# huzi96/NVFPCC

Hardware: AMD Instinct MI355X
Metric: leaf-blocks/sec NVF train step (32^3, chanstr=8,16,8,8) (higher is better)
Workload: dtype f32; 1 GPU; train_step: decoder mini-batch update, NVFPCC.py:149-223 (fwd mode=train q=1, 3 focal losses + rate terms, bwd, fused Adam); full=False, primed_steps=31, batch_per_gpu=16, global_batch=16, blocks_resident=917, ch=3, chanstr=8,16,8,8, parallelism=dp1

## Files before the change

### include/nvf_hip.h

```cpp
#ifndef NVF_HIP_H
#define NVF_HIP_H

#include <stddef.h>
#include <stdint.h>

#ifdef __cplusplus
extern "C" {
#endif

#define NVF_OK 0
#define NVF_EINVAL (-1)
#define NVF_EWORKSPACE (-2)

#define NVF_ACT_NONE 0
#define NVF_ACT_RELU 1
#define NVF_ACT_SIGMOID 2

int nvf_version(void);

typedef struct NvfStepCtx NvfStepCtx;
size_t nvf_step_ctx_bytes(void);
int nvf_step_ctx_init(NvfStepCtx* ctx);
int nvf_step_ctx_set_direct(NvfStepCtx* ctx, int on);
int nvf_step_ctx_set_wgrad_forms(NvfStepCtx* ctx, int conv2_zsplit, int conv1_wino);
// ... 261 lines not shown
                 int nterm, float thh_acc, float thh_sse, float* out, void* workspace, size_t workspace_bytes,
                 NvfStepCtx* ctx, void* stream);

int nvf_sigmoid_bwd(const float* dp, const float* p, float* dlogit, int64_t n, void* stream);

int nvf_relu_bwd(const float* dy, const float* y, float* out, int64_t n, void* stream);

int nvf_squared_error_map(const float* p, const float* dist, float thh, float* out, int batch, int spatial,
                          void* stream);

int nvf_maxpool2(const float* x, float* y, int batch_channels, int d, int h, int w, void* stream);

int nvf_adam_step(float* p, const float* g, float* m, float* v, int64_t n, float lr, float beta1, float beta2,
                  float eps, int step, void* stream);

typedef struct NvfStepTail {
  float* p;
  const float* g;
  float* m;
  float* v;
  int64_t n;
  const float* coef_dev;
  float coef0_host, coef1_host, beta1, beta2, eps;
  int32_t nnb;
  const float* loss_terms;
  const float* lbits;
  const float* nbits;
  const float* inv_npts_dev;
  float inv_npts_host, nbits_scale;
  const float* counts;
  float* acc;
  int64_t* sched_buf;
  const int64_t* sched_rows;
  uint64_t* sched_cursor;
  uint32_t* done;
  int32_t sched_words, reserved;
} NvfStepTail;
int nvf_step_tail(const NvfStepTail* args, void* stream);

int nvf_finals_flush_tail(NvfStepCtx* ctx, const NvfStepTail* tail, const int64_t* ranges, int nranges, void* stream);
int nvf_wgrad_reduce_finals_tail(const float* const* slabs, float* const* dws, const int* nslabs, const int* jtotals,
                                 int n, const float* const* addends, const NvfAdamFuse* adam, NvfStepCtx* ctx,
                                 const NvfStepTail* tail, const int64_t* ranges, int nranges, void* stream);
int nvf_wgrad_reduce_finals(const float* const* slabs, float* const* dws, const int* nslabs, const int* jtotals, int n,
                            const float* const* addends, NvfStepCtx* ctx, void* stream);
int nvf_adam_coefficients(float lr, float beta1, float beta2, int step, float* coef_host);
int nvf_adam_coefficients_n(float lr, float beta1, float beta2, int step0, int n, float* coef_host);

int nvf_gather_rows(const float* src, const int64_t* idx, float* dst, int rows, int width, void* stream);
int nvf_scatter_add_rows(const float* src, const int64_t* idx, float* dst, int rows, int width, void* stream);

int nvf_gather_rows_multi(const float* const* srcs, float* const* dsts, const int* widths, int n,
                          const int64_t* idx, int rows, void* stream);

int nvf_step_head(const void* table_dev, int nlayers, int q, uint64_t seed, uint64_t step, const uint64_t* step_dev,
                  float* const* pack_dsts, const int* pack_kinds, const int* pack_c0s, const int* pack_c1s,
                  const int* pack_layers, const int* pack_bwd, int npack, const float* const* srcs,
                  float* const* dsts, const int* widths, int n, const int64_t* idx, int rows,
                  const NvfRateJob* rate , void* stream);

typedef struct NvfStemHead {
  const float* emb;
  const float* lat_beta_hat;
  const float* lat_gamma_hat;
  const float* sigma;
  const float* mu;
  const float* beta_hat;
  const float* gamma_hat;
  float* h;
  float* lat;
  float* x_rounded;
  float* bits;
  float* a0;
  float* h0;
  float* y1;
  int32_t lat_row, up0_row, conv0_row;
  int32_t mode, ch, c0, c1, reserved;
} NvfStemHead;
int nvf_step_head_stem(const void* table_dev, int nlayers, int q, uint64_t seed, uint64_t step,
                       const uint64_t* step_dev, float* const* pack_dsts, const int* pack_kinds, const int* pack_c0s,
                       const int* pack_c1s, const int* pack_layers, const int* pack_bwd, int npack,
                       const float* const* srcs, float* const* dsts, const int* widths, int n, const int64_t* idx,
                       int rows, const NvfRateJob* rate , const NvfStemHead* stem, void* stream);

int nvf_uniform(float* out, int64_t n, uint64_t seed, uint64_t stream_id, void* stream);

int nvf_threshold_count(const float* p, float thh, int32_t* counts, int batch, int voxels, void* stream);
int nvf_threshold_compact(const float* p, float thh, const int32_t* offsets, const int32_t* origins,
                          int32_t* coords, int batch, int dim, void* stream);

int nvf_nearest_dist2(const int32_t* pts, const int32_t* blk_off, const int32_t* origins, const int32_t* nb_off,
                      const int32_t* nb_idx, int32_t* d2out, int nblocks, void* stream);

#define NVF_PC_CELLS (128 * 128 * 128)
size_t nvf_pc_workspace_bytes(int n_query, int n_target);
int nvf_pc_nearest(const int32_t* query_sorted, int n_query, const int32_t* target_sorted, const int32_t* cell_start,
                   int n_target, int32_t* nn_idx, int32_t* nn_d2, void* stream);
int nvf_pc_knn_normals(const int32_t* cloud_sorted, const int32_t* cell_start, const int32_t* cloud_xyz, int n, int k,
                       float* normals, int32_t* knn_idx, void* stream);
int nvf_pc_error_sums(const int32_t* query_xyz, int n_query, const int32_t* target_xyz, const int32_t* nn_idx,
                      const float* normals, int normals_of_target, int64_t* sums, double* d2_sum, void* workspace,
                      size_t workspace_bytes, void* stream);

int nvf_occ_hist(const float* p, int batch, int voxels, int shift, int nbits, const uint32_t* prefix,
                 const int32_t* d2, const uint8_t* gt, uint32_t* count, uint64_t* sum_d2, uint32_t* count_gt,
                 uint32_t* bad, void* stream);
int nvf_occ_hist_edges(const float* p, int batch, int voxels, const float* edges, int nedges, const int32_t* d2,
                       const uint8_t* gt, uint32_t* count, uint64_t* sum_d2, uint32_t* count_gt, uint32_t* bad,
                       void* stream);
int nvf_threshold_count_v(const float* p, const float* thh, int32_t* counts, int batch, int voxels, void* stream);
int nvf_threshold_compact_v(const float* p, const float* thh, const int32_t* offsets, const int32_t* origins,
                            int32_t* coords, int batch, int dim, void* stream);

#define NVF_PP_META_INTS 16
#define NVF_PP_OCT_BYTES 37449
int nvf_pp_keys(const int32_t* pts, int npts, int32_t* keys, uint32_t* bitmap6, int32_t* meta, void* stream);
int nvf_pp_tree(const uint32_t* bitmap6, int32_t* origins, uint32_t* rank_tab, uint8_t* octree_bytes, int32_t* nb_off,
                int32_t* meta, void* stream);
int nvf_pp_blocks(const int32_t* sorted_keys, int npts, const uint32_t* rank_tab, int32_t* meta, int32_t* pts,
                  int32_t* blk_off, void* stream);
int nvf_pp_neighbours(const int32_t* origins, const uint32_t* rank_tab, const int32_t* nb_off, int32_t* nb_idx,
                      int nblocks, void* stream);
int nvf_pp_grids(const int32_t* d2, float* dist, float* gt, int64_t n, void* stream);

#define NVF_PP_DEEP_WORK_WORDS 11264
int nvf_pp_keys_deep(const int32_t* pts, int npts, int bits, int64_t* keys, uint32_t* bitmap, int32_t* meta,
                     void* stream);
int nvf_pp_tree_deep(const uint32_t* bitmap, int bits, int npts, int32_t* origins, uint32_t* rank_tab,
                     uint8_t* octree_bytes, int32_t* nb_off, uint32_t* work, int32_t* meta, void* stream);
int nvf_pp_blocks_deep(const int64_t* sorted_keys, int npts, int bits, const uint32_t* rank_tab, int32_t* meta,
                       int32_t* pts, int32_t* blk_off, void* stream);
int nvf_pp_neighbours_deep(const int32_t* origins, int bits, const uint32_t* rank_tab, const int32_t* nb_off,
                           int32_t* nb_idx, int nblocks, void* stream);

#ifdef __cplusplus
}
#endif
#endif
```

### nvfpcc_amd/_lib.py

```python
import ctypes as C
import os

_HERE = os.path.dirname(os.path.abspath(__file__))
LIB_PATH = os.environ.get("NVF_LIB", os.path.join(_HERE, "libnvf_hip.so"))

P = C.c_void_p
I = C.c_int
F = C.c_float
L = C.c_int64
U = C.c_uint64
Z = C.c_size_t

PROTOTYPES = {
    "nvf_version": (I, []),
    "nvf_step_ctx_bytes": (Z, []),
    "nvf_step_ctx_init": (I, [P]),
    "nvf_step_ctx_set_direct": (I, [P, I]),
    "nvf_step_ctx_set_wgrad_forms": (I, [P, I, I]),
    "nvf_pack_conv_weight": (I, [P, I, I, I, P, P, P]),
    "nvf_pack_convT_weight": (I, [P, I, I, I, P, P, P]),
    "nvf_effective_params": (I, [P, P, P, P, I, P, P, P, I, I, U, U, P]),
    "nvf_layer_desc_size": (Z, []),
    "nvf_prepare_weights": (I, [P, I, I, U, U, P, P]),
    "nvf_conv3d_gather": (I, [P, P, P, P, P, P] + [I] * 14 + [P]),
# ... 8 lines not shown
    "nvf_conv3d_k4_wino_fwd": (I, [P, P, P, P, I, I, I, P]),
    "nvf_wgrad_k4_wino": (I, [P, P, P, P, P, Z, I, I, P]),
    "nvf_pack_wino16_k4_floats": (Z, []),
    "nvf_conv3d_k4_wino16_bwd": (I, [P, P, P, P, I, I, I, P, P, P]),
    "nvf_conv3d_k4_wino16_fwd": (I, [P, P, P, P, I, I, I, P]),
    "nvf_wgrad16_k4_wino_partial": (I, [P, P, P, I, I, I, I, P, P]),
    "nvf_pack_convT_mfma_floats": (Z, [I]),
    "nvf_pack_convT_mfma": (I, [P, I, I, P, P]),
    "nvf_convT3d_k5s2_mfma": (I, [P, P, P, P, I, I, I, I, I, I, P]),
    "nvf_pack_s2k5_mfma_floats": (Z, [I, I]),
    "nvf_pack_s2k5_mfma": (I, [P, I, I, P, P]),
    "nvf_conv3d_s2k5_mfma": (I, [P, P, P, P, P, I, I, I, I, I, I, P]),
    "nvf_pack_convT16_mfma_floats": (Z, [I, I]),
    "nvf_pack_convT16_mfma": (I, [P, I, I, P, P]),
    "nvf_convT3d_k5s2_mfma16": (I, [P, P, P, P, I, I, I, I, I, I, I, P]),
    "nvf_pack_g16_mfma_floats": (Z, [I, I, I]),
    "nvf_pack_g16_mfma": (I, [P, I, I, I, P, P]),
    "nvf_conv3d_g16_mfma": (I, [P, P, P, P, P, P] + [I] * 14 + [P]),
    "nvf_pack_mfma_all": (I, [P, P, P, P, P, I, P]),
    "nvf_heads3_fwd": (I, [P, P, P, P, P, P, I, I, P]),
    "nvf_heads3_bwd_data": (I, [P, P, P, P, P, P, I, P]),
    "nvf_heads3_loss_bwd_data": (I, [P, P, P, P, P, P, P, P, P, P, P, P, P, I, P, Z, P, P]),
    "nvf_heads3_loss_bwd_data_bias": (I, [P, P, P, P, P, P, P, P, P, P, P, P, P, I, P, P, Z, P, P]),
    "nvf_heads3_fwd_loss_bwd_data": (I, [P, P, P, P, I, P, P, P, P, P, P, P, P, P, P, P, P, I, P, P, Z, P, P, P]),
    "nvf_heads3_wgrad_partial": (I, [P, P, P, P, P, I, I, P, P]),
    "nvf_stem_fwd": (I, [P] * 10 + [I, I, I, I, P]),
    "nvf_stem_latent_fwd": (I, [P] * 12 + [I, U, U, P] + [P] * 9 + [I, I, I, I, P]),
    "nvf_stem_bwd_workspace": (Z, [I, I]),
    "nvf_stem_bwd_workspace_for": (Z, [I, I, I, I]),
    "nvf_stem_bwd": (I, [P] * 13 + [Z, I, I, I, I, P]),
    "nvf_stem_bwd_partial": (I, [P, P, P, P, P, P, P, P, P, P, P, P, P, P, Z, I, I, I, I, P, P, P, P]),
    "nvf_wgrad_workspace": (Z, [I] * 7),
    "nvf_wgrad": (I, [P, P, P, P, Z] + [I] * 15 + [P]),
    "nvf_wgrad_partial": (I, [P, P, P, P, Z] + [I] * 14 + [P, P]),
    "nvf_wgrad_reduce_multi": (I, [P, P, P, P, I, P]),
    "nvf_wgrad_mfma3_partial": (I, [P, P, P, I, P, P, P]),
    "nvf_wgrad_up1_conv0_partial": (I, [P, P, P, I, P, P]),
    "nvf_wgrad_trunk5_partial": (I, [P, P, P, I, P, P, P]),
    "nvf_wgrad_trunk5_partial_bias": (I, [P, P, P, P, I, P, P, P]),
    "nvf_wgrad_trunk5_heads_partial": (I, [P, P, P, P, P, P, P, I, I, P, P, P, P]),
    "nvf_wgrad_trunk5_heads_sums_partial": (I, [P, P, P, P, P, P, P, I, P, P, P, P, I, P, Z, P, P, I, P, P, P, P]),
    "nvf_wgrad_reduce_finals_tail": (I, [P, P, P, P, I, P, P, P, P, P, I, P]),
    "nvf_wgrad_reduce_finals": (I, [P, P, P, P, I, P, P, P]),
    "nvf_channel_sum_workspace": (Z, [I]),
    "nvf_channel_sum": (I, [P, P, P, Z, I, I, I, I, P]),
    "nvf_multi_channel_sum_workspace": (Z, [I]),
    "nvf_multi_channel_sum": (I, [P, P, P, P, I, I, P, Z, P, P]),
    "nvf_wgrad_reduce_multi_and_sums": (I, [P, P, P, P, I, P, P, P, P, I, I, P, Z, P, P]),
    "nvf_latent_tail_queue": (I, [P, P, P, P, P, P, P, P, P, P, F, I, U, U, P, P, P, P, P, P, P, P, P, P, I, I, I]),
    "nvf_stem_bwd_queue": (I, [P] * 16 + [Z, P, I, I, I, I, P]),
    "nvf_stem_bwd_pending": (I, [P]),
    "nvf_latent_tail_pending": (I, [P]),
    "nvf_latent_tail_cancel": (None, [P]),
    "nvf_finals_begin": (I, [P]),
    "nvf_finals_flush": (I, [P, P]),
    "nvf_finals_cancel": (None, [P]),
    "nvf_gdn_fwd": (I, [P, P, P, P, I, I, I, I, P]),
    "nvf_gdn_bwd_workspace": (Z, [I]),
    "nvf_gdn_bwd": (I, [P, P, P, P, P, P, P, P, Z, I, I, I, I, P]),
    "nvf_latent_fwd": (I, [P] * 12 + [I, I, I, I, U, U, P, P]),
    "nvf_latent_rate": (I, [P] * 12 + [F, I, I, I, I, U, U, P, P]),
    "nvf_weight_rate": (I, [P, I, P, P, P, P, P, P, P, F, I, P]),
    "nvf_weight_rate_batch_workspace": (Z, []),
    "nvf_weight_rate_batch": (I, [P, P, P, I, P, P, P, P, P, P, F, P, Z, P, P]),
    "nvf_reduce_workspace": (Z, []),
    "nvf_focal_loss": (I, [P, P, P, F, F, P, P, P, F, P, Z, L, I, I, P]),
    "nvf_focal_loss_multi": (I, [P, P, P, P, P, P, P, I, P, I, P, Z, P, P]),
    "nvf_metrics": (I, [P, P, P, F, F, P, P, Z, L, I, P, P]),
    "nvf_metrics_workspace": (Z, []),
    "nvf_metrics3": (I, [P, P, P, P, I, F, F, P, P, Z, P, P]),
    "nvf_sigmoid_bwd": (I, [P, P, P, L, P]),
    "nvf_relu_bwd": (I, [P, P, P, L, P]),
    "nvf_squared_error_map": (I, [P, P, F, P, I, I, P]),
    "nvf_maxpool2": (I, [P, P, I, I, I, I, P]),
    "nvf_adam_step": (I, [P, P, P, P, L, F, F, F, F, I, P]),
    "nvf_step_tail": (I, [P, P]),
    "nvf_adam_coefficients": (I, [F, F, F, I, P]),
    "nvf_adam_coefficients_n": (I, [F, F, F, I, I, P]),
    "nvf_gather_rows": (I, [P, P, P, I, I, P]),
    "nvf_scatter_add_rows": (I, [P, P, P, I, I, P]),
    "nvf_gather_rows_multi": (I, [P, P, P, I, P, I, P]),
    "nvf_step_head": (I, [P, I, I, U, U, P, P, P, P, P, P, P, I, P, P, P, I, P, I, P, P]),
    "nvf_step_head_stem": (I, [P, I, I, U, U, P, P, P, P, P, P, P, I, P, P, P, I, P, I, P, P, P]),
    "nvf_weight_rate_batch_final": (I, [P, P, P, P, P, P]),
    "nvf_wgrad_reduce_multi_and_sums_fused": (I, [P, P, P, P, I, P, P, P, P, P, P, I, I, P, Z, P, P]),
    "nvf_finals_flush_tail": (I, [P, P, P, I, P]),
    "nvf_uniform": (I, [P, L, U, U, P]),
    "nvf_nearest_dist2": (I, [P, P, P, P, P, P, I, P]),
    "nvf_threshold_count": (I, [P, F, P, I, I, P]),
    "nvf_threshold_compact": (I, [P, F, P, P, P, I, I, P]),
    "nvf_pc_workspace_bytes": (Z, [I, I]),
    "nvf_pc_nearest": (I, [P, I, P, P, I, P, P, P]),
    "nvf_pc_knn_normals": (I, [P, P, P, I, I, P, P, P]),
    "nvf_pc_error_sums": (I, [P, I, P, P, P, I, P, P, P, Z, P]),
    "nvf_occ_hist": (I, [P, I, I, I, I, P, P, P, P, P, P, P, P]),
    "nvf_occ_hist_edges": (I, [P, I, I, P, I, P, P, P, P, P, P, P]),
    "nvf_threshold_count_v": (I, [P, P, P, I, I, P]),
    "nvf_threshold_compact_v": (I, [P, P, P, P, P, I, I, P]),
    "nvf_pp_keys": (I, [P, I, P, P, P, P]),
    "nvf_pp_tree": (I, [P, P, P, P, P, P, P]),
    "nvf_pp_blocks": (I, [P, I, P, P, P, P, P]),
    "nvf_pp_neighbours": (I, [P, P, P, P, I, P]),
    "nvf_pp_grids": (I, [P, P, P, L, P]),
    "nvf_pp_keys_deep": (I, [P, I, I, P, P, P, P]),
    "nvf_pp_tree_deep": (I, [P, I, I, P, P, P, P, P, P, P]),
    "nvf_pp_blocks_deep": (I, [P, I, I, P, P, P, P, P]),
    "nvf_pp_neighbours_deep": (I, [P, I, P, P, P, I, P]),
}



class NvfStepTail(C.Structure):
    _fields_ = [("p", P), ("g", P), ("m", P), ("v", P), ("n", L), ("coef_dev", P),
                ("coef0_host", F), ("coef1_host", F), ("beta1", F), ("beta2", F), ("eps", F), ("nnb", C.c_int32),
                ("loss_terms", P), ("lbits", P), ("nbits", P), ("inv_npts_dev", P),
                ("inv_npts_host", F), ("nbits_scale", F), ("counts", P), ("acc", P),
                ("sched_buf", P), ("sched_rows", P), ("sched_cursor", P), ("done", P),
                ("sched_words", C.c_int32), ("reserved", C.c_int32)]


class NvfRateJob(C.Structure):
    _fields_ = [("kernel", P * 8), ("dk", P * 8), ("n", C.c_int32 * 8), ("nlayers", C.c_int32), ("reserved", C.c_int32),
                ("sigma", P), ("mu", P), ("part", P), ("g", F), ("reserved2", F)]


class NvfStemHead(C.Structure):
    _fields_ = [(n, P) for n in ("emb", "lat_beta_hat", "lat_gamma_hat", "sigma", "mu", "beta_hat", "gamma_hat", "h", "lat",
                                 "x_rounded", "bits", "a0", "h0", "y1")] + \
               [(n, C.c_int32) for n in ("lat_row", "up0_row", "conv0_row", "mode", "ch", "c0", "c1", "reserved")]


class NvfAdamFuse(C.Structure):
    _fields_ = [("g_base", P), ("p_base", P), ("m_base", P), ("v_base", P), ("n", L), ("coef_dev", P),
                ("coef0_host", F), ("coef1_host", F), ("beta1", F), ("beta2", F), ("eps", F), ("reserved", F),
                ("bad_count", P)]


_lib = None


def lib():
    global _lib
    if _lib is None:
        if not os.path.isfile(LIB_PATH):
            raise RuntimeError(
                f"{LIB_PATH} is missing: the HIP extension has not been built "
                "(python -m nvfpcc_amd.build). There is no CPU fallback for the NVF hot path.")
        h = C.CDLL(LIB_PATH)
        for name, (res, args) in PROTOTYPES.items():
            fn = getattr(h, name)
            fn.restype = res
            fn.argtypes = args
        _lib = h
    return _lib


class NvfError(RuntimeError):
    pass


def check(rc, what):
    if rc != 0:
        kind = {-1: "NVF_EINVAL (rejected argument)", -2: "NVF_EWORKSPACE (workspace too small)"}.get(
            rc, f"hipError_t {rc}")
        raise NvfError(f"{what} failed: {kind}")
```

### nvfpcc_amd/csrc/finals.h

```cpp
#pragma once
#include "nvf_common.h"

static const int kLossMaxWG = 1024;

#define NVF_BETA_BOUND 1.0000072759311445e-03f
#define NVF_GAMMA_BOUND 3.814697265625e-06f

__device__ __forceinline__ int adam_fused_elem(const NvfAdamFuse& a, const float* gp, float gi) {
  const long i = gp - a.g_base;
  if (i < 0 || i >= a.n) return 0;
  if (!(fabsf(gi) <= 3.402823466e38f)) return 1;
  const float step_size = a.coef_dev ? a.coef_dev[0] : a.coef0_host, bc2_sqrt = a.coef_dev ? a.coef_dev[1] : a.coef1_host;
  const float mi = a.m_base[i] * a.beta1 + gi * (1.f - a.beta1);
  const float vi = a.v_base[i] * a.beta2 + (gi * gi) * (1.f - a.beta2);
  a.m_base[i] = mi;
  a.v_base[i] = vi;
  const float denom = sqrtf(vi) / bc2_sqrt + a.eps;
  a.p_base[i] = a.p_base[i] - step_size * (mi / denom);
  return 0;
}
__device__ __forceinline__ NvfAdamFuse adam_fuse_of(const NvfStepTail& t) {
  NvfAdamFuse a{};
  a.g_base = t.g; a.p_base = t.p; a.m_base = t.m; a.v_base = t.v; a.n = t.n; a.coef_dev = t.coef_dev;
  a.coef0_host = t.coef0_host; a.coef1_host = t.coef1_host; a.beta1 = t.beta1; a.beta2 = t.beta2; a.eps = t.eps;
  a.bad_count = t.acc ? t.acc + 6 : nullptr;
  return a;
}

struct FocalMulti {
  const float* p[3];
  const float* gt[3];
  const float* dist[3];
  float* dp[3];
  float alpha[3], beta[3];
  long n[3];
  int nwg[3];
};

struct MultiSumDesc {
  const float* x[12];
  float* out[12];
  int32_t c[12], spatial[12], chan_base[12];
  int32_t ntensors, batch, total_channels, nchunk;
};

struct WeightRateBatch {
  const float* kernel[8];
  float* dk[8];
  int32_t n[8];
  int32_t first_wg[9];
  int32_t nlayers, chunk;
};

__device__ __forceinline__ float focal_elem(float pv, float gv, float dv, bool has_dist, float a1, float a0, float beta,
                                            int chain_sigmoid, float& dp, float g = 1.f) {
#pragma clang fp contract(off)
  const bool occ = gv != 0.f;
  const float F = occ ? pv : 1.f - pv;
  const float at = occ ? a1 : a0;
  float w = 1.f;
  if (has_dist) w = dv + (occ ? beta : 0.f);
  const float Fc = F < 1e-9f ? 1e-9f : F;
  const float om = 1.f - Fc;
  const float lg = logf(Fc);
  float d = 0.f;
  if (F >= 1e-9f) d = -at * w * (-2.f * om * lg + om * om / Fc);
  const float dd = g * (occ ? d : -d);
  dp = chain_sigmoid ? dd * ((1.f - pv) * pv) : dd;
  return -1.f * at * (om * om) * w * lg;
}

__device__ __forceinline__ void focal_multi_final_body(const FocalMulti& m, const float* __restrict__ part,
                                                       float* __restrict__ loss, int nterm, int tid) {
  const int t = tid >> 6, lane = tid & 63;
  if (t >= nterm) return;
  float s = 0.f;
  for (int g = lane; g < m.nwg[t]; g += 64) s += part[t * kLossMaxWG + g];
  s = nvf_wave_sum(s);
  if (lane == 0) loss[t] = s;
}

__device__ __forceinline__ int multi_channel_sum_final_body(const MultiSumDesc& d, const float* __restrict__ part,
                                                            int gch, const NvfAdamFuse* adam = nullptr) {
  if (gch >= d.total_channels) return 0;
  int t = 0;
  while (t + 1 < d.ntensors && gch >= d.chan_base[t + 1]) ++t;
  float s = 0.f;
  for (int g = 0; g < d.nchunk; ++g) s += part[(size_t)g * d.total_channels + gch];
  float* o = d.out[t] + (gch - d.chan_base[t]);
  *o = s;
  return adam ? adam_fused_elem(*adam, o, s) : 0;
}

__device__ __forceinline__ int weight_rate_batch_final_body(const WeightRateBatch& b, const float* __restrict__ part,
                                                            const float* __restrict__ sigma, float* __restrict__ bits,
                                                            float* __restrict__ dsigma, float* __restrict__ dmu,
                                                            const float* __restrict__ g_dev, float g_host, int lane,
                                                            const NvfAdamFuse* adam = nullptr) {
  const float g = g_host * (g_dev ? g_dev[0] : 1.f);
  constexpr int SLOTS = 8;
  const int nwg = b.first_wg[b.nlayers];
  float pb[SLOTS], ps[SLOTS], pm[SLOTS];
#pragma unroll
  for (int i = 0; i < SLOTS; ++i) {
    const int wg = lane + 64 * i;
    const bool ok = wg < nwg;
    pb[i] = ok ? part[3 * wg] : 0.f;
    ps[i] = ok ? part[3 * wg + 1] : 0.f;
// ... 67 lines not shown
__device__ __forceinline__ void metrics_final_body(const float* __restrict__ part, float* __restrict__ out,
                                                   const int32_t* nwg, int nterm, int accumulate, int tid) {
  if (tid >= 6 * nterm) return;
  const int t = tid / 6, k = tid - 6 * t;
  float s = 0.f;
  for (int g0 = 0; g0 < nwg[t]; g0 += 16) {
    float v[16];
#pragma unroll
    for (int i = 0; i < 16; ++i) v[i] = g0 + i < nwg[t] ? part[((size_t)t * kLossMaxWG + g0 + i) * 6 + k] : 0.f;
#pragma unroll
    for (int i = 0; i < 16; ++i) s += v[i];
  }
  out[tid] = accumulate ? out[tid] + s : s;
}

struct FinalsArgs {
  FocalMulti f;
  const float* f_part;
  float* f_loss;
  MultiSumDesc s;
  const float* s_part;
  WeightRateBatch r;
  const float* r_part;
  const float* r_sigma;
  float* r_bits;
  float* r_dsigma;
  float* r_dmu;
  const float* r_gdev;
  float r_ghost;
  StemGdnFinal g;
  const float* m_part;
  float* m_out;
  int32_t m_nwg[3], m_nterm, m_accumulate;
  int32_t f_nterm, has_f, has_s, has_r, has_g, has_m;
  const float* hb_part;
  float* hb_out[3];
  int32_t hb_n[3], has_hb;
};

__device__ __forceinline__ int head_bias_final_body(const FinalsArgs& a, int h, int lane, const NvfAdamFuse* adam = nullptr) {
  float s = 0.f;
  for (int g = lane; g < a.hb_n[h]; g += 64) s += a.hb_part[h * kLossMaxWG + g];
  s = nvf_wave_sum(s);
  if (lane != 0) return 0;
  *a.hb_out[h] = s;
  return adam ? adam_fused_elem(*adam, a.hb_out[h], s) : 0;
}

__host__ __device__ inline int finals_sum_blocks(const FinalsArgs& a) {
  const int n = a.has_s ? (a.s.total_channels + 63) / 64 : 0;
  return n > 0 ? n : (a.has_hb ? 1 : 0);
}

__device__ __forceinline__ void finals_plain_body(const FinalsArgs& a, int sum_blocks, int bid) {
  const int tid = threadIdx.x;
  if (a.has_hb && bid == 2 && tid >= 64 && tid < 256) head_bias_final_body(a, (tid >> 6) - 1, tid & 63);
  if (bid == 2 + sum_blocks) {
    if (a.has_m) metrics_final_body(a.m_part, a.m_out, a.m_nwg, a.m_nterm, a.m_accumulate, tid);
  } else if (bid == 0) {
    if (a.has_f) focal_multi_final_body(a.f, a.f_part, a.f_loss, a.f_nterm, tid);
  } else if (bid == 1) {
    if (a.has_r && tid < 64)
      weight_rate_batch_final_body(a.r, a.r_part, a.r_sigma, a.r_bits, a.r_dsigma, a.r_dmu, a.r_gdev, a.r_ghost, tid);
    if (a.has_g && tid >= 64 && tid < 192) stem_gdn_final_body(a.g, tid - 64, 128);
  } else if (a.has_s && tid < 64) {
    multi_channel_sum_final_body(a.s, a.s_part, (bid - 2) * 64 + tid);
  }
}

struct TailRanges { long lo[16], hi[16]; int n; };

__device__ __forceinline__ void finals_tail_arrive(const NvfStepTail& t, unsigned long long cur, int nblocks) {
  if (!t.sched_rows) return;
  const int tid = threadIdx.x;
  __shared__ int last;
  int64_t next_word = 0;
  if (tid < t.sched_words) next_word = t.sched_rows[cur * (unsigned long long)t.sched_words + tid];
  if (tid == 0) last = atomicAdd(t.done, 1u) == (unsigned)nblocks - 1;
  __syncthreads();
  if (!last) return;
  if (tid < t.sched_words) t.sched_buf[tid] = next_word;
  for (int w = tid + blockDim.x; w < t.sched_words; w += blockDim.x)
    t.sched_buf[w] = t.sched_rows[cur * (unsigned long long)t.sched_words + w];
  if (tid == 0) { t.sched_cursor[0] = cur + 1; t.done[0] = 0u; }
}

__device__ __forceinline__ void finals_tail_body(const FinalsArgs& a, int sum_blocks, const NvfStepTail& t,
                                                 const TailRanges& rg, int bid, int nblocks) {
  const int tid = threadIdx.x, wave = tid >> 6, lane = tid & 63;
  const NvfAdamFuse ad = adam_fuse_of(t);
  const unsigned long long cur = t.sched_rows ? t.sched_cursor[0] : 0ull;
  int bad = 0;
  if (bid == 0) {
    if (a.has_f) focal_multi_final_body(a.f, a.f_part, a.f_loss, a.f_nterm, tid);
    if (a.has_r && wave == 3)
      bad += weight_rate_batch_final_body(a.r, a.r_part, a.r_sigma, a.r_bits, a.r_dsigma, a.r_dmu, a.r_gdev, a.r_ghost,
                                          lane, &ad);
    if (a.has_m) metrics_final_body(a.m_part, a.m_out, a.m_nwg, a.m_nterm, a.m_accumulate, tid);
  } else if (bid == 1) {
    if (a.has_g && tid < 256) bad += stem_gdn_final_body(a.g, tid, 256, &ad);
  } else if (bid < 2 + sum_blocks) {
    if (a.has_s && tid < 64) bad += multi_channel_sum_final_body(a.s, a.s_part, (bid - 2) * 64 + tid, &ad);
    if (a.has_hb && bid == 2 && wave >= 1 && wave <= 3) bad += head_bias_final_body(a, wave - 1, lane, &ad);
  } else {
    for (int r = 0; r < rg.n; ++r)
      for (long i = rg.lo[r] + tid; i < rg.hi[r]; i += blockDim.x) bad += adam_fused_elem(ad, t.g + i, t.g[i]);
  }
  if (t.acc) {
    const unsigned long long any = __ballot(bad != 0);
    float c = (float)bad;
    c = nvf_wave_sum(c);
    if (any && lane == 0) atomicAdd(t.acc + 6, c);
  }
  __syncthreads();
  if (bid == 0 && tid == 0 && t.acc) {
    int bad_terms = 0;
    for (int k = 0; k < 3; ++k) {
      const float x = t.loss_terms[k];
      t.acc[k] += x;
      bad_terms += !(fabsf(x) <= 3.402823466e38f);
    }
    const float bl = t.lbits[0] * (t.inv_npts_dev ? t.inv_npts_dev[0] : t.inv_npts_host);
    float nb = 0.f;
    for (int l = 0; l < t.nnb; ++l) nb += t.nbits[l];
    nb *= t.nbits_scale;
    t.acc[3] += bl;
    t.acc[4] += nb;
    bad_terms += !(fabsf(bl) <= 3.402823466e38f) + !(fabsf(nb) <= 3.402823466e38f);
    t.acc[5] += (float)bad_terms;
    t.acc[7] += 1.f;
    if (t.counts) {
      for (int k = 0; k < 3; ++k) {
        t.acc[8 + 2 * k] += t.counts[6 * k] / t.counts[6 * k + 1];
        t.acc[9 + 2 * k] += t.counts[6 * k + 2] / t.counts[6 * k + 3];
      }
      t.acc[14] += t.counts[4];
      t.acc[15] += t.counts[5];
    }
  }
  finals_tail_arrive(t, cur, nblocks);
}

struct NvfStepCtx;
bool nvf_finals_push_focal(NvfStepCtx* ctx, const FocalMulti& m, const float* part, float* loss, int nterm);
int nvf_finals_run_stem_gdn(NvfStepCtx* ctx, const StemGdnFinal& f, void* stream);
int nvf_finals_run_focal(NvfStepCtx* ctx, const FocalMulti& m, const float* part, float* loss, int nterm, void* stream);
bool nvf_finals_push_sums(NvfStepCtx* ctx, const MultiSumDesc& d, const float* part);
int nvf_finals_run_head_bias(NvfStepCtx* ctx, const float* part, float* const* outs, const int* n, void* stream);
bool nvf_finals_push_metrics(NvfStepCtx* ctx, const float* part, float* out, const int* nwg, int nterm, int accumulate);
bool nvf_finals_push_rate(NvfStepCtx* ctx, const WeightRateBatch& b, const float* part, const float* sigma, float* bits,
                          float* dsigma, float* dmu, const float* g_dev, float g_host);
```

### nvfpcc_amd/csrc/pointwise.hip

```cpp
#include "nvf_common.h"
#include "step_ctx.h"
#include "pack_mfma.h"
#include "latent_tail.h"
#include "stem_fwd.h"

#define NVF_GRID(n, bs) ((unsigned)(((n) + (bs)-1) / (bs)))

extern "C" int nvf_version(void) { return 100; }

__global__ void finalize_partials(const float* __restrict__ part, float* __restrict__ out, int nrow, int ncol,
                                  int accumulate) {
  int j = blockIdx.x * blockDim.x + threadIdx.x;
  if (j >= ncol) return;
  float s = 0.f;
  for (int g = 0; g < nrow; ++g) s += part[(size_t)g * ncol + j];
  out[j] = accumulate ? out[j] + s : s;
}

__global__ void effective_params_kernel(const float* __restrict__ kernel, const float* __restrict__ kernel_init,
                                        const float* __restrict__ u, float* __restrict__ w_eff, int n,
                                        const float* __restrict__ b, const float* __restrict__ b_init,
                                        float* __restrict__ b_eff, int nb, int q, uint64_t seed, uint64_t stream_id) {
  int i = blockIdx.x * blockDim.x + threadIdx.x;
  if (i < n) {
    float k = kernel[i];
    if (q == 1) {
      float uu = u ? u[i] : nvf_uniform01(seed, stream_id, (uint64_t)i);
      k = k + (uu - 0.5f) * 0.0625f;
    } else if (q == 2) {
      k = rintf(k * 16.f) / 16.f;
    }
    w_eff[i] = k + kernel_init[i];
  } else if (i < n + nb) {
    int j = i - n;
    b_eff[j] = b[j] + b_init[j];
  }
}

extern "C" int nvf_effective_params(const float* kernel, const float* kernel_init, const float* u, float* w_eff, int n,
                                    const float* b, const float* b_init, float* b_eff, int nb, int q, uint64_t seed,
                                    uint64_t stream_id, void* stream) {
  if (!kernel || !kernel_init || !w_eff || n <= 0 || nb < 0) return NVF_EINVAL;
  if (nb > 0 && (!b || !b_init || !b_eff)) return NVF_EINVAL;
  effective_params_kernel<<<NVF_GRID(n + nb, 256), 256, 0, nvf_stream(stream)>>>(kernel, kernel_init, u, w_eff, n, b,
                                                                                  b_init, b_eff, nb, q, seed,
                                                                                  stream_id);
  NVF_LAUNCH_CHECK();
  return NVF_OK;
}

struct NvfLayerDesc {
  const float* kernel;
  const float* kernel_init;
  const float* b;
  const float* b_init;
  float* w_fwd;
  float* w_bwd;
  float* b_eff;
  int32_t dim0, dim1, k3;
  int32_t kind;
  int32_t quantised;
  int32_t layer_id;
  int32_t nbias, pad_;
};

__device__ __forceinline__ float effective_weight(const NvfLayerDesc& d, int i, int qq, uint64_t seed, uint64_t sid) {
  float k = d.kernel[i];
  if (qq == 1) k = k + (nvf_uniform01(seed, sid, (uint64_t)i) - 0.5f) * 0.0625f;
  else if (qq == 2) k = rintf(k * 16.f) / 16.f;
  return k + d.kernel_init[i];
}

__device__ __forceinline__ void prepare_weights_body(const NvfLayerDesc* __restrict__ table, int q, uint64_t seed,
                                                     uint64_t step, const uint64_t* __restrict__ step_dev, int layer,
                                                     int bx, int nbx) {
  const NvfLayerDesc d = table[layer];
  const int n = d.dim0 * d.dim1 * d.k3;
  const int qq = d.quantised ? q : 0;
  const uint64_t st = step + (step_dev ? step_dev[0] : 0ull);
  const uint64_t sid = (st << 8) | (uint64_t)d.layer_id;
  for (int i = bx * blockDim.x + threadIdx.x; i < n + d.nbias; i += nbx * blockDim.x) {
    if (i < n) {
      const float w = effective_weight(d, i, qq, seed, sid);
      const int t = i % d.k3, i1 = (i / d.k3) % d.dim1, i0 = i / (d.k3 * d.dim1);
      if (d.kind == 0) {
        if (d.w_fwd) d.w_fwd[(i1 * d.k3 + t) * d.dim0 + i0] = w;
        if (d.w_bwd) d.w_bwd[(i0 * d.k3 + (d.k3 - 1 - t)) * d.dim1 + i1] = w;
      } else {
        if (d.w_fwd) d.w_fwd[(i0 * d.k3 + t) * d.dim1 + i1] = w;
        if (d.w_bwd) d.w_bwd[(i1 * d.k3 + t) * d.dim0 + i0] = w;
      }
    } else {
      const int j = i - n;
      d.b_eff[j] = d.b[j] + d.b_init[j];
    }
  }
}

__global__ void prepare_weights_kernel(const NvfLayerDesc* __restrict__ table, int q, uint64_t seed, uint64_t step,
                                       const uint64_t* __restrict__ step_dev) {
  prepare_weights_body(table, q, seed, step, step_dev, blockIdx.y, blockIdx.x, gridDim.x);
}

extern "C" size_t nvf_layer_desc_size(void) { return sizeof(NvfLayerDesc); }

extern "C" int nvf_prepare_weights(const void* table_dev, int nlayers, int q, uint64_t seed, uint64_t step,
                                   const uint64_t* step_dev, void* stream) {
  if (!table_dev || nlayers <= 0) return NVF_EINVAL;
  prepare_weights_kernel<<<dim3(16, nlayers), 256, 0, nvf_stream(stream)>>>((const NvfLayerDesc*)table_dev, q, seed,
                                                                           step, step_dev);
  NVF_LAUNCH_CHECK();
  return NVF_OK;
}

__global__ void gdn_fwd_kernel(const float* __restrict__ x, const float* __restrict__ beta_hat,
                               const float* __restrict__ gamma_hat, float* __restrict__ y, int batch, int c,
                               int spatial, int inverse) {
  long idx = (long)blockIdx.x * blockDim.x + threadIdx.x;
  long total = (long)batch * c * spatial;
  if (idx >= total) return;
  int s = idx % spatial;
  int ch = (idx / spatial) % c;
  long b = idx / ((long)spatial * c);
  const float* xb = x + b * c * spatial + s;
  float acc = gdn_beta(beta_hat[ch]);
  for (int j = 0; j < c; ++j) {
    float xj = xb[(long)j * spatial];
    acc = fmaf(gdn_gamma(gamma_hat[ch * c + j]), xj * xj, acc);
  }
  float nrm = sqrtf(acc);
  float xv = xb[(long)ch * spatial];
  y[idx] = inverse ? xv * nrm : xv / nrm;
}

extern "C" int nvf_gdn_fwd(const float* x, const float* beta_hat, const float* gamma_hat, float* y, int batch, int c,
                           int spatial, int inverse, void* stream) {
  if (!x || !beta_hat || !gamma_hat || !y || batch <= 0 || c <= 0 || spatial <= 0) return NVF_EINVAL;
  long total = (long)batch * c * spatial;
  gdn_fwd_kernel<<<NVF_GRID(total, 256), 256, 0, nvf_stream(stream)>>>(x, beta_hat, gamma_hat, y, batch, c, spatial,
                                                                       inverse);
  NVF_LAUNCH_CHECK();
  return NVF_OK;
}

static const int kGdnMaxC = 32;
static const int kGdnThreads = 128;
static const int kGdnMaxSlabs = 256;

template <int CG>
__global__ __launch_bounds__(kGdnThreads * CG) void gdn_bwd_kernel(const float* __restrict__ x,
                                                                   const float* __restrict__ beta_hat,
                                                                   const float* __restrict__ gamma_hat,
                                                                   const float* __restrict__ dy, float* __restrict__ dx,
                                                                   float* __restrict__ slabs, int batch, int c,
                                                                   int spatial, int inverse, int vox_per_wg,
                                                                   float* __restrict__ dbeta_hat,
                                                                   float* __restrict__ dgamma_hat) {
  extern __shared__ float sm[];
  constexpr int T = kGdnThreads, LD = T + 1, NT = T * CG, MAXK = kGdnMaxC / CG;
  float* ts = sm;
  float* xs = sm + c * LD;
  float* gam = xs + c * LD;
  float* bet = gam + c * c;
  const int tid = threadIdx.x, vt = tid % T, cg = tid / T;
  const int ncol = c + c * c;
  const long nvox = (long)batch * spatial;
  const long v_lo = (long)blockIdx.x * vox_per_wg;
  long v_hi = v_lo + vox_per_wg;
  if (v_hi > nvox) v_hi = nvox;
  for (int i = tid; i < c * c; i += NT) gam[i] = gdn_gamma(gamma_hat[i]);
  for (int i = tid; i < c; i += NT) bet[i] = gdn_beta(beta_hat[i]);
  float own[(kGdnMaxC + kGdnMaxC * kGdnMaxC + NT - 1) / NT];
#pragma unroll
  for (int i = 0; i < (int)(sizeof(own) / sizeof(float)); ++i) own[i] = 0.f;

  for (long base = v_lo; base < v_hi; base += T) {
    const long v = base + vt;
// ... 147 lines not shown
                               float* dsigma, float* dmu, const float* g_dev, float g_host, int batch, int c,
                               int spatial, int mode,
                               uint64_t seed, uint64_t step, const uint64_t* step_dev, void* stream) {
  if (!x || !sigma || !mu || batch <= 0 || c <= 0 || spatial <= 0) return NVF_EINVAL;
  if (mode != 0 && mode != 1) return NVF_EINVAL;
  latent_rate_kernel<<<1, 1024, 0, nvf_stream(stream)>>>(x, u, block_ids, sigma, mu, x_rounded, bits, dx, dx_addend,
                                                         dsigma, dmu, g_dev, g_host, batch, c, spatial, mode, seed,
                                                         step, step_dev);
  NVF_LAUNCH_CHECK();
  return NVF_OK;
}

__global__ __launch_bounds__(1024) void latent_fwd_kernel(const float* __restrict__ e, const float* __restrict__ w,
                                                          const float* __restrict__ bw,
                                                          const float* __restrict__ beta_hat,
                                                          const float* __restrict__ gamma_hat,
                                                          const int64_t* __restrict__ block_ids,
                                                          const float* __restrict__ sigma, const float* __restrict__ mu,
                                                          float* __restrict__ h_out, float* __restrict__ lat_out,
                                                          float* __restrict__ x_rounded, float* __restrict__ bits,
                                                          int batch, int c, int spatial, int mode, uint64_t seed,
                                                          uint64_t step_in, const uint64_t* __restrict__ step_dev) {
  __shared__ float s_par[160];
  __shared__ float scratch[kTailRateLds / 3];
  latent_fwd_body(e, w, bw, beta_hat, gamma_hat, block_ids, sigma, mu, h_out, lat_out, x_rounded, bits, batch, c, spatial,
                  mode, seed, step_in, step_dev, s_par, scratch, kTailRateLds / 3);
}

extern "C" int nvf_latent_fwd(const float* e, const float* w_fwd, const float* bias, const float* beta_hat,
                              const float* gamma_hat, const int64_t* block_ids, const float* sigma, const float* mu,
                              float* h, float* lat, float* x_rounded, float* bits, int batch, int c, int spatial,
                              int mode, uint64_t seed, uint64_t step, const uint64_t* step_dev, void* stream) {
  if (!e || !w_fwd || !bias || !beta_hat || !gamma_hat || !sigma || !mu || !h || !lat || !x_rounded || !bits)
    return NVF_EINVAL;
  if (batch <= 0 || c <= 0 || c > 8 || spatial <= 0 || (mode != 0 && mode != 1)) return NVF_EINVAL;
  latent_fwd_kernel<<<1, 1024, 0, nvf_stream(stream)>>>(e, w_fwd, bias, beta_hat, gamma_hat, block_ids, sigma, mu, h,
                                                        lat, x_rounded, bits, batch, c, spatial, mode, seed, step,
                                                        step_dev);
  NVF_LAUNCH_CHECK();
  return NVF_OK;
}

__global__ __launch_bounds__(1024) void weight_rate_kernel(const float* __restrict__ kernel, int n,
                                                           const float* __restrict__ sigma,
                                                           const float* __restrict__ mu, float* __restrict__ bits,
                                                           float* __restrict__ dk, float* __restrict__ dsigma,
                                                           float* __restrict__ dmu, const float* __restrict__ g_dev,
                                                           float g_host, int accumulate) {
  __shared__ float red[16];
  const float g = g_host * (g_dev ? g_dev[0] : 1.f);
  const float gsign = g > 0.f ? 1.f : (g < 0.f ? -1.f : 0.f);
  const float sraw = sigma[0], sabs = fabsf(sraw), m = mu[0];
  float sb = 0.f, ss = 0.f, sm_ = 0.f;
  for (int i = threadIdx.x; i < n; i += blockDim.x) {
    float v = rintf(kernel[i] * 16.f) / 16.f;
    RateTerm r = rate_term(v, m, sabs, 0.03125f, gsign);
    sb += r.bits;
    ss += r.dsig;
    sm_ += r.dmu;
    if (dk) dk[i] = accumulate ? dk[i] + g * r.dv : g * r.dv;
  }
  float tb = nvf_block_sum(sb, red);
  float tsg = nvf_block_sum(ss, red);
  float tm = nvf_block_sum(sm_, red);
  if (threadIdx.x == 0) {
    if (bits) bits[0] = tb;
    float sgn = sraw > 0.f ? 1.f : (sraw < 0.f ? -1.f : 0.f);
    if (dsigma) dsigma[0] = accumulate ? dsigma[0] + g * tsg * sgn : g * tsg * sgn;
    if (dmu) dmu[0] = accumulate ? dmu[0] + g * tm : g * tm;
  }
}

extern "C" int nvf_weight_rate(const float* kernel, int n, const float* sigma, const float* mu, float* bits, float* dk,
                               float* dsigma, float* dmu, const float* g_dev, float g_host, int accumulate,
                               void* stream) {
  if (!kernel || !sigma || !mu || n <= 0) return NVF_EINVAL;
  weight_rate_kernel<<<1, 1024, 0, nvf_stream(stream)>>>(kernel, n, sigma, mu, bits, dk, dsigma, dmu, g_dev, g_host,
                                                         accumulate);
  NVF_LAUNCH_CHECK();
  return NVF_OK;
}


__device__ __forceinline__ void weight_rate_partial_body(const WeightRateBatch& b, const float* __restrict__ sigma,
                                                         const float* __restrict__ mu, float* __restrict__ part, float g,
                                                         int wg, int accumulate, float* red, int nthreads = 0) {
  if (nthreads <= 0) nthreads = blockDim.x;
  const float gsign = g > 0.f ? 1.f : (g < 0.f ? -1.f : 0.f);
  const float sabs = fabsf(sigma[0]), m = mu[0];
  int l = 0;
  while (l + 1 < b.nlayers && wg >= b.first_wg[l + 1]) ++l;
  const int lo = (wg - b.first_wg[l]) * b.chunk;
  const int hi = min(lo + b.chunk, b.n[l]);
  const float* k = b.kernel[l];
  float* dk = b.dk[l];
  float sb = 0.f, ss = 0.f, sm_ = 0.f;
  for (int i = lo + threadIdx.x; i < hi && (int)threadIdx.x < nthreads; i += nthreads) {
    float v = rintf(k[i] * 16.f) / 16.f;
    RateTerm r = rate_term(v, m, sabs, 0.03125f, gsign);
    sb += r.bits;
    ss += r.dsig;
    sm_ += r.dmu;
    if (dk) dk[i] = accumulate ? dk[i] + g * r.dv : g * r.dv;
  }
  float tb = nvf_block_sum(sb, red);
  float tsg = nvf_block_sum(ss, red);
  float tm = nvf_block_sum(sm_, red);
  if (threadIdx.x == 0) {
    part[3 * wg] = tb;
    part[3 * wg + 1] = tsg;
    part[3 * wg + 2] = tm;
  }
}

__global__ __launch_bounds__(256) void weight_rate_batch_kernel(WeightRateBatch b, const float* __restrict__ sigma,
                                                                const float* __restrict__ mu,
                                                                float* __restrict__ part,
                                                                const float* __restrict__ g_dev, float g_host) {
  __shared__ float red[16];
  weight_rate_partial_body(b, sigma, mu, part, g_host * (g_dev ? g_dev[0] : 1.f), blockIdx.x, 1, red);
}

static int weight_rate_batch_desc(const float* const* kernels, float* const* dks, const int* ns, int nlayers,
                                  WeightRateBatch& b) {
  if (!kernels || !ns || nlayers <= 0 || nlayers > 8) return NVF_EINVAL;
  long total = 0;
  for (int i = 0; i < nlayers; ++i) {
    if (!kernels[i] || ns[i] <= 0) return NVF_EINVAL;
    b.kernel[i] = kernels[i];
    b.dk[i] = dks ? dks[i] : nullptr;
    b.n[i] = ns[i];
    total += ns[i];
  }
  b.nlayers = nlayers;
  long chunk = (total + 255) / 256;
  if (chunk < 256) chunk = 256;
  b.chunk = (int)chunk;
  int wg = 0;
  for (int i = 0; i < nlayers; ++i) {
    b.first_wg[i] = wg;
    wg += (int)((ns[i] + chunk - 1) / chunk);
  }
  b.first_wg[nlayers] = wg;
  return wg > 512 ? NVF_EINVAL : NVF_OK;
}

__global__ void weight_rate_batch_final(WeightRateBatch b, const float* __restrict__ part,
                                        const float* __restrict__ sigma, float* __restrict__ bits,
                                        float* __restrict__ dsigma, float* __restrict__ dmu,
                                        const float* __restrict__ g_dev, float g_host) {
  weight_rate_batch_final_body(b, part, sigma, bits, dsigma, dmu, g_dev, g_host, threadIdx.x);
}

extern "C" int nvf_weight_rate_batch_final(const NvfRateJob* job, float* bits, float* dsigma, float* dmu,
                                           NvfStepCtx* ctx, void* stream) {
  if (!job || !bits || !job->sigma || !job->mu || !job->part) return NVF_EINVAL;
  WeightRateBatch b{};
  const int rc = weight_rate_batch_desc(job->kernel, job->dk, job->n, job->nlayers, b);
  if (rc != NVF_OK) return rc;
  if (!nvf_finals_push_rate(ctx, b, job->part, job->sigma, bits, dsigma, dmu, nullptr, job->g))
    weight_rate_batch_final<<<1, 64, 0, nvf_stream(stream)>>>(b, job->part, job->sigma, bits, dsigma, dmu, nullptr, job->g);
  NVF_LAUNCH_CHECK();
  return NVF_OK;
}

extern "C" size_t nvf_weight_rate_batch_workspace(void) { return (size_t)3 * 512 * sizeof(float); }

extern "C" int nvf_weight_rate_batch(const float* const* kernels, float* const* dks, const int* ns, int nlayers,
                                     const float* sigma, const float* mu, float* bits, float* dsigma, float* dmu,
                                     const float* g_dev, float g_host, void* workspace, size_t workspace_bytes,
                                     NvfStepCtx* ctx, void* stream) {
  if (!kernels || !ns || nlayers <= 0 || nlayers > 8 || !sigma || !mu || !bits || !workspace) return NVF_EINVAL;
  if (workspace_bytes < nvf_weight_rate_batch_workspace()) return NVF_EWORKSPACE;
  WeightRateBatch b{};
  const int rc = weight_rate_batch_desc(kernels, dks, ns, nlayers, b);
  if (rc != NVF_OK) return rc;
  const int wg = b.first_wg[nlayers];
  hipStream_t s = nvf_stream(stream);
  weight_rate_batch_kernel<<<wg, 256, 0, s>>>(b, sigma, mu, (float*)workspace, g_dev, g_host);
  if (!nvf_finals_push_rate(ctx, b, (const float*)workspace, sigma, bits, dsigma, dmu, g_dev, g_host))
    weight_rate_batch_final<<<1, 64, 0, s>>>(b, (const float*)workspace, sigma, bits, dsigma, dmu, g_dev, g_host);
// ... 265 lines not shown
  long i = (long)blockIdx.x * blockDim.x + threadIdx.x;
  if (i >= n) return;
  float gi = g[i];
  float mi = m[i] * b1 + gi * (1.f - b1);
  float vi = v[i] * b2 + (gi * gi) * (1.f - b2);
  m[i] = mi;
  v[i] = vi;
  float denom = sqrtf(vi) / bc2_sqrt + eps;
  p[i] = p[i] - step_size * (mi / denom);
}

extern "C" int nvf_adam_step(float* p, const float* g, float* m, float* v, int64_t n, float lr, float beta1,
                             float beta2, float eps, int step, void* stream) {
  if (!p || !g || !m || !v || n <= 0 || step < 1) return NVF_EINVAL;
  double bc1 = 1.0 - pow((double)beta1, step), bc2 = 1.0 - pow((double)beta2, step);
  adam_kernel<<<NVF_GRID(n, 256), 256, 0, nvf_stream(stream)>>>(p, g, m, v, (long)n, (float)(lr / bc1), beta1, beta2,
                                                                eps, (float)sqrt(bc2));
  NVF_LAUNCH_CHECK();
  return NVF_OK;
}

__global__ void step_tail_kernel(NvfStepTail a) {
  const long i = (long)blockIdx.x * blockDim.x + threadIdx.x;
  int bad = 0;
  if (i < a.n) {
    const float step_size = a.coef_dev ? a.coef_dev[0] : a.coef0_host, bc2_sqrt = a.coef_dev ? a.coef_dev[1] : a.coef1_host;
    const float gi = a.g[i];
    bad = !(fabsf(gi) <= 3.402823466e38f);
    if (!bad) {
      const float mi = a.m[i] * a.beta1 + gi * (1.f - a.beta1);
      const float vi = a.v[i] * a.beta2 + (gi * gi) * (1.f - a.beta2);
      a.m[i] = mi;
      a.v[i] = vi;
      const float denom = sqrtf(vi) / bc2_sqrt + a.eps;
      a.p[i] = a.p[i] - step_size * (mi / denom);
    }
  }
  if (a.acc) {
    const unsigned long long any = __ballot(bad);
    if (any && (threadIdx.x & 63) == 0) atomicAdd(a.acc + 6, (float)__popcll(any));
  }
  if (!a.acc && !a.sched_rows) return;
  __shared__ int last;
  bool is_last = gridDim.x == 1;
  if (gridDim.x > 1) {
    __syncthreads();
    if (threadIdx.x == 0) last = atomicAdd(a.done, 1u) == gridDim.x - 1;
    __syncthreads();
    is_last = last != 0;
  }
  if (!is_last) return;
  if (a.acc && threadIdx.x == 0) {
    int bad_terms = 0;
    for (int t = 0; t < 3; ++t) {
      const float x = a.loss_terms[t];
      a.acc[t] += x;
      bad_terms += !(fabsf(x) <= 3.402823466e38f);
    }
    const float bl = a.lbits[0] * (a.inv_npts_dev ? a.inv_npts_dev[0] : a.inv_npts_host);
    float nb = 0.f;
    for (int l = 0; l < a.nnb; ++l) nb += a.nbits[l];
    nb *= a.nbits_scale;
    a.acc[3] += bl;
    a.acc[4] += nb;
    bad_terms += !(fabsf(bl) <= 3.402823466e38f) + !(fabsf(nb) <= 3.402823466e38f);
    a.acc[5] += (float)bad_terms;
    a.acc[7] += 1.f;
    if (a.counts) {
      for (int t = 0; t < 3; ++t) {
        a.acc[8 + 2 * t] += a.counts[6 * t] / a.counts[6 * t + 1];
        a.acc[9 + 2 * t] += a.counts[6 * t + 2] / a.counts[6 * t + 3];
      }
      a.acc[14] += a.counts[4];
      a.acc[15] += a.counts[5];
    }
  }
  if (a.sched_rows) {
    __shared__ unsigned long long cur_s;
    if (threadIdx.x == 0) cur_s = a.sched_cursor[0];
    __syncthreads();
    const unsigned long long c = cur_s;
    const int64_t* row = a.sched_rows + c * (unsigned long long)a.sched_words;
    for (int w = threadIdx.x; w < a.sched_words; w += blockDim.x) a.sched_buf[w] = row[w];
    if (threadIdx.x == 0) a.sched_cursor[0] = c + 1;
  }
  if (threadIdx.x == 0 && gridDim.x > 1) a.done[0] = 0u;
}

extern "C" int nvf_step_tail(const NvfStepTail* args, void* stream) {
  if (!args) return NVF_EINVAL;
  const NvfStepTail a = *args;
  if (!a.p || !a.g || !a.m || !a.v || a.n <= 0) return NVF_EINVAL;
  if (a.acc && (!a.loss_terms || !a.lbits || !a.nbits || a.nnb <= 0 || a.nnb > 16)) return NVF_EINVAL;
  if (a.sched_rows && (!a.sched_buf || !a.sched_cursor || a.sched_words <= 0)) return NVF_EINVAL;
  if ((a.acc || a.sched_rows) && !a.done) return NVF_EINVAL;
  step_tail_kernel<<<NVF_GRID(a.n, 256), 256, 0, nvf_stream(stream)>>>(a);
  NVF_LAUNCH_CHECK();
  return NVF_OK;
}

extern "C" int nvf_adam_coefficients(float lr, float beta1, float beta2, int step, float* coef_host) {
  if (!coef_host || step < 1) return NVF_EINVAL;
  double bc1 = 1.0 - pow((double)beta1, step), bc2 = 1.0 - pow((double)beta2, step);
  coef_host[0] = (float)(lr / bc1);
  coef_host[1] = (float)sqrt(bc2);
  return NVF_OK;
}

extern "C" int nvf_adam_coefficients_n(float lr, float beta1, float beta2, int step0, int n, float* coef_host) {
  if (!coef_host || step0 < 1 || n < 0) return NVF_EINVAL;
  for (int k = 0; k < n; ++k) {
    const int rc = nvf_adam_coefficients(lr, beta1, beta2, step0 + k, coef_host + 2 * k);
    if (rc != NVF_OK) return rc;
  }
  return NVF_OK;
}

__global__ void gather_rows_kernel(const float* __restrict__ src, const int64_t* __restrict__ idx,
                                   float* __restrict__ dst, int rows, int width) {
  long i = (long)blockIdx.x * blockDim.x + threadIdx.x;
  if (i >= (long)rows * width) return;
  int r = i / width, c = i % width;
  dst[i] = src[idx[r] * width + c];
}

__global__ void scatter_add_rows_kernel(const float* __restrict__ src, const int64_t* __restrict__ idx,
                                        float* __restrict__ dst, int rows, int width) {
  long i = (long)blockIdx.x * blockDim.x + threadIdx.x;
  if (i >= (long)rows * width) return;
  int r = i / width, c = i % width;
  dst[idx[r] * width + c] += src[i];
}

extern "C" int nvf_gather_rows(const float* src, const int64_t* idx, float* dst, int rows, int width, void* stream) {
  if (!src || !idx || !dst || rows <= 0 || width <= 0) return NVF_EINVAL;
  gather_rows_kernel<<<NVF_GRID((long)rows * width, 256), 256, 0, nvf_stream(stream)>>>(src, idx, dst, rows, width);
  NVF_LAUNCH_CHECK();
  return NVF_OK;
}

extern "C" int nvf_scatter_add_rows(const float* src, const int64_t* idx, float* dst, int rows, int width,
                                    void* stream) {
  if (!src || !idx || !dst || rows <= 0 || width <= 0) return NVF_EINVAL;
  scatter_add_rows_kernel<<<NVF_GRID((long)rows * width, 256), 256, 0, nvf_stream(stream)>>>(src, idx, dst, rows,
                                                                                            width);
  NVF_LAUNCH_CHECK();
  return NVF_OK;
}

struct GatherMulti {
  const float* src[6];
  float* dst[6];
  int32_t width[6];
  int32_t n;
};

__device__ __forceinline__ void gather_rows_multi_body(const GatherMulti& g, const int64_t* __restrict__ idx, int rows,
                                                       int t, int bx, int nbx) {
  if (t >= g.n) return;
  const int width = g.width[t];
  const long total = (long)rows * width;
  const float* src = g.src[t];
  float* dst = g.dst[t];
  if ((width & 3) == 0) {
    const long total4 = total >> 2;
    const int w4 = width >> 2;
    for (long i = (long)bx * blockDim.x + threadIdx.x; i < total4; i += (long)nbx * blockDim.x) {
// ... 200 lines not shown
  if ((NVF_HS_SKIP & 2) && bid >= nstem) return;
  if (bid < nstem) {
    const uint64_t st = step + (step_dev ? step_dev[0] : 0ull);
    const StemRawW wp{table[sj.lat_row], table[sj.up0_row], table[sj.conv0_row], sj.emb, idx, seed, st, sj.ch, q};
    const StemLatent L{nullptr, nullptr, nullptr, sj.lat_beta_hat, sj.lat_gamma_hat, idx, sj.sigma, sj.mu, sj.h, sj.lat,
                       sj.x_rounded, sj.bits, step_dev, seed, step, sj.mode, rows};
    const int b = bid == 0 ? 0 : (bid - 1) / PARTS, part = bid == 0 ? PARTS : (bid - 1) % PARTS;
    stem_fwd_body<C0, C1, COG, true, true>(nullptr, wp, sj.beta_hat, sj.gamma_hat, sj.a0, sj.h0, sj.y1, sj.ch, L, b, part,
                                           lds);
    return;
  }
  bid -= nstem;
  if (bid < rate.nwg) {
    weight_rate_partial_body(rate.b, rate.sigma, rate.mu, rate.part, rate.g, bid, 0, lds, 256);
    return;
  }
  bid -= rate.nwg;
  if (bid < wpl * nlayers) { prepare_weights_body(table, q, seed, step, step_dev, bid / wpl, bid % wpl, wpl); return; }
  bid -= wpl * nlayers;
  if (bid < wpl * pk.n) {
    const int job = bid / wpl;
    const NvfLayerDesc d = table[pk.layer[job]];
    const int qq = d.quantised ? q : 0, bwd = pk.bwd[job];
    const uint64_t st = step + (step_dev ? step_dev[0] : 0ull);
    const uint64_t sid = (st << 8) | (uint64_t)d.layer_id;
    pack_mfma_body(pk, job, bid % wpl, wpl, [&](int, int si) {
      return effective_weight(d, layout_to_kernel_index(d, bwd, si), qq, seed, sid);
    });
    return;
  }
  bid -= wpl * pk.n;
  gather_rows_multi_body(g, idx, rows, bid / gwg, bid % gwg, gwg);
}

extern "C" int nvf_step_head_stem(const void* table_dev, int nlayers, int q, uint64_t seed, uint64_t step,
                                  const uint64_t* step_dev, float* const* pack_dsts, const int* pack_kinds,
                                  const int* pack_c0s, const int* pack_c1s, const int* pack_layers, const int* pack_bwd,
                                  int npack, const float* const* srcs, float* const* dsts, const int* widths, int n,
                                  const int64_t* idx, int rows, const NvfRateJob* rate_job, const NvfStemHead* stem,
                                  void* stream) {
  if (!table_dev || nlayers <= 0 || !idx || npack < 0 || !stem) return NVF_EINVAL;
  const NvfStemHead sj = *stem;
  const bool narrow = sj.c0 == 8 && sj.c1 == 16, wide = sj.c0 == 16 && sj.c1 == 32;
  if (!(narrow || wide) || sj.ch <= 0 || sj.ch > kStemFwdMaxCh || rows <= 0 || rows > 32) return NVF_EINVAL;
  if (sj.lat_row < 0 || sj.lat_row >= nlayers || sj.up0_row < 0 || sj.up0_row >= nlayers || sj.conv0_row < 0 ||
      sj.conv0_row >= nlayers || (sj.mode != 0 && sj.mode != 1))
    return NVF_EINVAL;
  if (!sj.emb || !sj.lat_beta_hat || !sj.lat_gamma_hat || !sj.sigma || !sj.mu || !sj.beta_hat || !sj.gamma_hat || !sj.h ||
      !sj.lat || !sj.x_rounded || !sj.bits || !sj.a0 || !sj.h0 || !sj.y1)
    return NVF_EINVAL;
  PackJobs pk{};
  if (npack > 0) {
    if (!pack_layers || !pack_bwd) return NVF_EINVAL;
    const int rc = pack_jobs_desc(nullptr, pack_dsts, pack_kinds, pack_c0s, pack_c1s, npack, pk);
    if (rc != NVF_OK) return rc;
    for (int j = 0; j < npack; ++j) {
      if (pack_layers[j] < 0 || pack_layers[j] >= nlayers) return NVF_EINVAL;
      pk.layer[j] = pack_layers[j]; pk.bwd[j] = pack_bwd[j] ? 1 : 0;
    }
  }
  GatherMulti g{};
  long wg = 0;
  const int rc = gather_multi_desc(srcs, dsts, widths, n, rows, g, wg);
  if (rc != NVF_OK) return rc;
  const int tscale = (narrow ? 2 : 4) * nvf_tune_int("NVF_HS_GSCALE", 1);
  wg = (wg + tscale - 1) / tscale;
  const int wpl = nvf_tune_int("NVF_HS_WPL", 32) > 0 ? nvf_tune_int("NVF_HS_WPL", 32) : 32;
  RateInHead rate{};
  if (rate_job) {
    if (!rate_job->sigma || !rate_job->mu || !rate_job->part) return NVF_EINVAL;
    const int rrc = weight_rate_batch_desc(rate_job->kernel, rate_job->dk, rate_job->n, rate_job->nlayers, rate.b);
    if (rrc != NVF_OK) return rrc;
    rate.sigma = rate_job->sigma; rate.mu = rate_job->mu; rate.part = rate_job->part; rate.g = rate_job->g;
    rate.nwg = rate.b.first_wg[rate.b.nlayers];
  }
  const int parts = narrow ? 16 / 4 : 32 / (2 * 2);
  const unsigned grid = 1 + rows * parts + rate.nwg + wpl * nlayers + wpl * npack + (unsigned)(wg * n);
  if (narrow)
    step_head_stem_kernel<8, 16, 4><<<grid, 512, 0, nvf_stream(stream)>>>(
        (const NvfLayerDesc*)table_dev, nlayers, q, seed, step, step_dev, pk, g, idx, rows, (int)wg, wpl, rate, sj);
  else
    step_head_stem_kernel<16, 32, 2><<<grid, 1024, 0, nvf_stream(stream)>>>(
        (const NvfLayerDesc*)table_dev, nlayers, q, seed, step, step_dev, pk, g, idx, rows, (int)wg, wpl, rate, sj);
  NVF_LAUNCH_CHECK();
  return NVF_OK;
}

__global__ void uniform_kernel(float* __restrict__ out, long n, uint64_t seed, uint64_t stream_id) {
  long i = (long)blockIdx.x * blockDim.x + threadIdx.x;
  if (i < n) out[i] = nvf_uniform01(seed, stream_id, (uint64_t)i);
}

extern "C" int nvf_uniform(float* out, int64_t n, uint64_t seed, uint64_t stream_id, void* stream) {
  if (!out || n <= 0) return NVF_EINVAL;
  uniform_kernel<<<NVF_GRID(n, 256), 256, 0, nvf_stream(stream)>>>(out, (long)n, seed, stream_id);
  NVF_LAUNCH_CHECK();
  return NVF_OK;
}

__global__ __launch_bounds__(1024) void threshold_count_kernel(const float* __restrict__ p, float thh,
                                                               int32_t* __restrict__ counts, int voxels) {
  __shared__ float red[16];
  const float* pb = p + (size_t)blockIdx.x * voxels;
  float c = 0.f;
  for (int i = threadIdx.x; i < voxels; i += blockDim.x) c += pb[i] > thh ? 1.f : 0.f;
  float t = nvf_block_sum(c, red);
  if (threadIdx.x == 0) counts[blockIdx.x] = (int32_t)t;
}

extern "C" int nvf_threshold_count(const float* p, float thh, int32_t* counts, int batch, int voxels, void* stream) {
  if (!p || !counts || batch <= 0 || voxels <= 0 || voxels > (1 << 24)) return NVF_EINVAL;
  threshold_count_kernel<<<batch, 1024, 0, nvf_stream(stream)>>>(p, thh, counts, voxels);
  NVF_LAUNCH_CHECK();
  return NVF_OK;
}

__global__ __launch_bounds__(1024) void threshold_compact_kernel(const float* __restrict__ p, float thh,
                                                                 const int32_t* __restrict__ offsets,
                                                                 const int32_t* __restrict__ origins,
                                                                 int32_t* __restrict__ coords, int dim) {
  __shared__ int wave_cnt[16];
  __shared__ int running;
  const int b = blockIdx.x, voxels = dim * dim * dim;
  const float* pb = p + (size_t)b * voxels;
  const int lane = threadIdx.x & 63, wv = threadIdx.x >> 6, nw = blockDim.x >> 6;
  const int oz = origins ? origins[3 * b] : 0, oy = origins ? origins[3 * b + 1] : 0, ox = origins ? origins[3 * b + 2] : 0;
  if (threadIdx.x == 0) running = offsets[b];
  __syncthreads();
  for (int base = 0; base < voxels; base += blockDim.x) {
    const int i = base + threadIdx.x;
    const bool hit = i < voxels && pb[i] > thh;
    const unsigned long long mask = __ballot(hit);
    const int before = __popcll(mask & ((1ull << lane) - 1ull));
    if (lane == 0) wave_cnt[wv] = __popcll(mask);
    __syncthreads();
    int off = running;
    for (int k = 0; k < wv; ++k) off += wave_cnt[k];
    if (hit) {
      const int z = i / (dim * dim), y = (i / dim) % dim, x = i % dim;
      int32_t* o = coords + (size_t)(off + before) * 3;
      o[0] = oz + z;
      o[1] = oy + y;
      o[2] = ox + x;
    }
    __syncthreads();
    if (threadIdx.x == 0) {
      int t = 0;
      for (int k = 0; k < nw; ++k) t += wave_cnt[k];
      running += t;
    }
    __syncthreads();
  }
}

extern "C" int nvf_threshold_compact(const float* p, float thh, const int32_t* offsets, const int32_t* origins,
                                     int32_t* coords, int batch, int dim, void* stream) {
  if (!p || !offsets || !coords || batch <= 0 || dim <= 0 || dim > 256) return NVF_EINVAL;
  threshold_compact_kernel<<<batch, 1024, 0, nvf_stream(stream)>>>(p, thh, offsets, origins, coords, dim);
  NVF_LAUNCH_CHECK();
  return NVF_OK;
}
```

### nvfpcc_amd/csrc/wgrad.hip

```cpp
#include "nvf_common.h"
#include <cstdio>
#include <cstdlib>
#include "step_ctx.h"
#include "heads_wgrad_mfma.h"

static const int kMaxSlabs = 512;
static const int kSumChunks = 128;
struct MultiSumDesc;
__global__ void multi_channel_sum_final(MultiSumDesc d, const float* __restrict__ part);
extern "C" size_t nvf_multi_channel_sum_workspace(int total_channels);
__global__ void wgrad_reduce(const float* __restrict__ slabs, float* __restrict__ dw, int nslab, int jtotal,
                             int accumulate);

struct WgDims {
  int batch, bc;
  int dp, hp, wp;
  int dq, hq, wq;
  int pad;
  int tiles_x, tiles_y, tiles_z;
  int items, items_per_wg;
  int out_mode, jtotal;
  float* bias_slab;
};

__global__ void wgrad_naive(const float* __restrict__ p, const float* __restrict__ q, float* __restrict__ dw, int a_ch,
                            int k, int stride, WgDims d, int accumulate) {
  int k3 = k * k * k;
  int j = blockIdx.x * (blockDim.x >> 6) + (threadIdx.x >> 6);
  const int lane = threadIdx.x & 63;
  if (j >= a_ch * d.bc * k3) return;
  int kk = j % k3, b = (j / k3) % d.bc, a = j / (k3 * d.bc);
  int kz = kk / (k * k), ky = (kk / k) % k, kx = kk % k;
  const long plane = (long)d.hp * d.wp, vol = (long)d.dp * plane, total = (long)d.batch * vol;
  float acc = 0.f;
  for (long e = lane; e < total; e += 64) {
    const int n = (int)(e / vol);
    const long r = e - (long)n * vol;
    const int iz = (int)(r / plane), iy = (int)((r - (long)iz * plane) / d.wp), ix = (int)(r % d.wp);
    const int qz = iz * stride - d.pad + kz, qy = iy * stride - d.pad + ky, qx = ix * stride - d.pad + kx;
    if (qz < 0 || qz >= d.dq || qy < 0 || qy >= d.hq || qx < 0 || qx >= d.wq) continue;
    const float pv = p[((size_t)n * a_ch + a) * vol + r];
    const float qv = q[(((size_t)n * d.bc + b) * d.dq + qz) * d.hq * d.wq + qy * d.wq + qx];
    acc = fmaf(pv, qv, acc);
  }
  acc = nvf_wave_sum(acc);
  if (lane != 0) return;
  int o = d.out_mode == 0 ? j : (b * a_ch + a) * k3 + (k3 - 1 - kk);
  dw[o] = accumulate ? dw[o] + acc : acc;
}

template <int A_, int KS_, int S_, int NB_, int TX_, int TY_, int TZ_, int IXU_ = 0>
struct WCfg {
  static constexpr int A = A_, KS = KS_, S = S_, NB = NB_, TX = TX_, TY = TY_, TZ = TZ_;
  static constexpr int K3 = KS * KS * KS;
  static constexpr int IXU = IXU_ > 0 ? IXU_ : (A_ <= 8 ? 2 : 1);
  static constexpr int WPB = (K3 + 63) / 64;
  static constexpr int NT = NB * WPB * 64;
  static constexpr int QX = (TX - 1) * S + KS, QY = (TY - 1) * S + KS, QZ = (TZ - 1) * S + KS;
  static constexpr int mod32(int v, int r) { return v + ((r - v % 32) + 32) % 32; }
  static constexpr int QRS = mod32(QX, KS % 32);
  static constexpr int QPS = mod32(QY * QRS, (KS * KS) % 32);
  static constexpr int QCS = QZ * QPS;
  static constexpr int PT = A * TZ * TY * TX;
  static constexpr int POFF = (NB * QCS + 3) / 4 * 4;
  static constexpr int LDSF = POFF + PT;
  static_assert(TX % 4 == 0, "p rows are read four at a time");
  static_assert(NT <= 1024, "workgroup size");
  static_assert(LDSF * 4 <= 160 * 1024, "LDS");
};

template <class C>
__device__ __forceinline__ void wgrad_tiled_body(const float* __restrict__ p, const float* __restrict__ q,
                                                 float* __restrict__ slabs, const WgDims& d, int bx, int by, float* lds) {
  constexpr int A = C::A, KS = C::KS, S = C::S, NB = C::NB, TX = C::TX, TY = C::TY, TZ = C::TZ, K3 = C::K3;
  constexpr int QX = C::QX, QY = C::QY, QZ = C::QZ, QRS = C::QRS, QPS = C::QPS, QCS = C::QCS, NT = C::NT;
  const int tid = threadIdx.x, wave = tid >> 6, lane = tid & 63;
  const int bb = wave / C::WPB;
  const int kk = (wave % C::WPB) * 64 + lane;
  const bool valid = kk < K3;
  const int kz = kk / (KS * KS), ky = (kk / KS) % KS, kx = kk % KS;
  const int b0 = by * NB;
  const int lane_off = valid ? bb * QCS + kz * QPS + ky * QRS + kx : 0;
  float acc[A];
#pragma unroll
  for (int a = 0; a < A; ++a) acc[a] = 0.f;

  const int tiles = d.tiles_x * d.tiles_y * d.tiles_z;
// ... 1077 lines not shown
    const bool cube_t5 = a == 8 && b == 8 && k == 5 && stride == 2 && pad == 0 && out_mode == 0 && dp == 16 && hp == 16 &&
                         wp == 16 && dq == 35 && hq == 35 && wq == 35;
    if (rc == 1 && variant == 0 && cube_t5) rc = launch_wgrad_s2k5<TWCfg<2, 2>>(p, q, dw, slabs, d, accumulate, s, defer_nslab);
    if (rc == 1 && variant == 7 && cube_t5) rc = launch_wgrad_s2k5<TWCfg<1, 4>>(p, q, dw, slabs, d, accumulate, s, defer_nslab);
    NVF_W(9, 8, 4, 1, 32, 8, 32, 8, 2, 0)
    NVF_W(9, 8, 4, 1, 16, 8, 16, 8, 2, 0)
    NVF_W(0, 8, 5, 2, 16, 4, 16, 4, 2, 0)
    NVF_W(9, 8, 5, 2, 16, 4, 16, 4, 2, 0)
    NVF_W(0, 16, 5, 2, 8, 4, 8, 4, 2, 0)
    NVF_W(0, 8, 5, 2, 4, 4, 4, 4, 4, 0)
    NVF_W(0, 16, 4, 1, 32, 8, 32, 4, 2, 0)
    NVF_W(0, 16, 4, 1, 16, 8, 16, 8, 2, 0)
    NVF_W(0, 16, 5, 2, 16, 2, 16, 4, 2, 0)
    NVF_W(0, 32, 5, 2, 8, 4, 8, 4, 2, 0)
    NVF_W(0, 16, 5, 2, 4, 4, 4, 4, 4, 0)
    NVF_W(40, 16, 4, 1, 32, 16, 32, 8, 2, 0)
    NVF_W(41, 16, 4, 1, 32, 8, 32, 4, 2, 0)
    NVF_W(42, 16, 4, 1, 32, 8, 32, 8, 4, 0)
    NVF_W(43, 16, 4, 1, 32, 4, 32, 8, 2, 0)
    NVF_W(40, 16, 5, 2, 16, 8, 16, 4, 2, 0)
    NVF_W(41, 16, 5, 2, 16, 4, 16, 8, 2, 0)
    NVF_W(42, 16, 5, 2, 16, 4, 16, 4, 4, 0)
    NVF_W(43, 16, 5, 2, 16, 2, 16, 4, 2, 0)
    NVF_W(0, 8, 3, 1, 32, 1, 32, 8, 4, 0)
    NVF_W(0, 8, 3, 1, 16, 1, 16, 8, 4, 0)
    NVF_W(0, 16, 3, 1, 8, 1, 8, 8, 8, 0)
    NVF_W(0, 16, 3, 1, 32, 1, 32, 8, 4, 0)
    NVF_W(0, 16, 3, 1, 16, 1, 16, 8, 4, 0)
    NVF_W(0, 32, 3, 1, 8, 1, 8, 8, 8, 0)
    NVF_W(0, 1, 3, 1, 32, 8, 32, 8, 4, 8)
    NVF_W(0, 1, 3, 1, 16, 8, 16, 8, 4, 4)
    NVF_W(0, 1, 3, 1, 8, 8, 8, 8, 8, 2)
    NVF_W(2, 1, 3, 1, 32, 8, 32, 8, 2, 8)
    NVF_W(3, 1, 3, 1, 32, 4, 32, 8, 4, 8)
    NVF_W(2, 8, 4, 1, 32, 8, 32, 8, 2, 1)
    NVF_W(3, 8, 4, 1, 32, 8, 32, 8, 2, 8)
    NVF_W(4, 8, 4, 1, 32, 8, 32, 4, 2, 2)
    NVF_W(5, 8, 4, 1, 32, 4, 32, 8, 4, 2)
    NVF_W(6, 8, 4, 1, 32, 8, 32, 8, 4, 2)
    NVF_W(2, 8, 3, 1, 32, 1, 32, 8, 4, 1)
    NVF_W(3, 8, 3, 1, 32, 1, 32, 4, 2, 2)
    NVF_W(2, 8, 5, 2, 16, 4, 16, 4, 2, 1)
    NVF_W(3, 8, 5, 2, 16, 8, 16, 4, 2, 2)
    NVF_W(4, 8, 5, 2, 16, 4, 16, 2, 2, 2)
#undef NVF_W
  }
  if (rc == 1) {
    wgrad_naive<<<(d.jtotal + 3) / 4, 256, 0, s>>>(p, q, dw, a, k, stride, d, accumulate);
    if (defer_nslab) *defer_nslab = 0;
    rc = NVF_OK;
  }
  NVF_LAUNCH_CHECK();
  return rc;
}

extern "C" int nvf_wgrad_up1_conv0_partial(const float* const* ps, const float* const* qs, float* const* slabs,
                                           int batch, int* nslabs, void* stream) {
  if (!ps || !qs || !slabs || !nslabs || batch <= 0) return NVF_EINVAL;
  using C0 = WCfg<16, 5, 2, 4, 8, 4, 2, 0>; using C1 = WCfg<8, 5, 2, 4, 4, 4, 4, 0>;
  WgTiled2 m{};
  for (int j = 0; j < 2; ++j)
    if (!ps[j] || !qs[j] || !slabs[j]) return NVF_EINVAL;
  fill_up1_conv0<C0, C1>(m, ps, qs, slabs, batch, nslabs);
  wgrad_tiled2_kernel<C0, C1><<<m.nx[0] * m.ny[0] + m.nx[1] * m.ny[1], C0::NT, 0, nvf_stream(stream)>>>(m);
  NVF_LAUNCH_CHECK();
  return NVF_OK;
}

extern "C" int nvf_wgrad(const float* p, const float* q, float* dw, void* workspace, size_t workspace_bytes, int batch,
                         int a, int b, int k, int stride, int pad, int dp, int hp, int wp, int dq, int hq, int wq,
                         int out_mode, int accumulate, int variant, void* stream) {
  return wgrad_dispatch(p, q, dw, workspace, workspace_bytes, batch, a, b, k, stride, pad, dp, hp, wp, dq, hq, wq,
                        out_mode, accumulate, variant, stream, nullptr);
}

extern "C" int nvf_wgrad_partial(const float* p, const float* q, float* dw, void* workspace, size_t workspace_bytes,
                                 int batch, int a, int b, int k, int stride, int pad, int dp, int hp, int wp, int dq,
                                 int hq, int wq, int out_mode, int variant, int* nslab, void* stream) {
  if (!nslab) return NVF_EINVAL;
  return wgrad_dispatch(p, q, dw, workspace, workspace_bytes, batch, a, b, k, stride, pad, dp, hp, wp, dq, hq, wq,
                        out_mode, 0, variant, stream, nslab);
}

struct WgReduceMulti {
  const float* slabs[16];
  float* dw[16];
  const float* add[16];
  int32_t nslab[16], jtotal[16], blk_base[17];
  int32_t n, fuse;
  NvfAdamFuse adam;
};

__device__ __forceinline__ void wgrad_reduce_multi_body(const WgReduceMulti& d, int bid, float (*part)[64]) {
  int t = 0;
  while (t + 1 < d.n && bid >= d.blk_base[t + 1]) ++t;
  const float* slabs = d.slabs[t];
  const int nslab = d.nslab[t], jtotal = d.jtotal[t];
  const int jl = threadIdx.x & 63, sl = threadIdx.x >> 6;
  const int j = (bid - d.blk_base[t]) * 64 + jl;
  float s0 = 0.f, s1 = 0.f, s2 = 0.f, s3 = 0.f;
  if (j < jtotal) {
    for (int g0 = sl; g0 < nslab; g0 += 256) {
      float v[16];
#pragma unroll
      for (int i = 0; i < 16; ++i) v[i] = g0 + 16 * i < nslab ? slabs[(size_t)(g0 + 16 * i) * jtotal + j] : 0.f;
#pragma unroll
      for (int i = 0; i < 16; i += 4) { s0 += v[i]; s1 += v[i + 1]; s2 += v[i + 2]; s3 += v[i + 3]; }
    }
  }
  const float s = (s0 + s1) + (s2 + s3);
  part[sl][jl] = s;
  __syncthreads();
  if (sl == 0) {
    int bad = 0;
    if (j < jtotal) {
      float v = part[0][jl];
#pragma unroll
      for (int k = 1; k < 16; ++k) v += part[k][jl];
      if (d.add[t]) v += d.add[t][j];
      d.dw[t][j] = v;
      if (d.fuse) bad = adam_fused_elem(d.adam, d.dw[t] + j, v);
    }
    if (d.fuse && d.adam.bad_count) {
      const unsigned long long any = __ballot(bad);
      if (any && jl == 0) atomicAdd(d.adam.bad_count, (float)__popcll(any));
    }
  }
}

__global__ __launch_bounds__(1024) void wgrad_reduce_multi(WgReduceMulti d) {
  __shared__ float part[16][64];
  wgrad_reduce_multi_body(d, blockIdx.x, part);
}

extern "C" int nvf_wgrad_reduce_multi(const float* const* slabs, float* const* dws, const int* nslabs,
                                      const int* jtotals, int n, void* stream) {
  if (!slabs || !dws || !nslabs || !jtotals || n <= 0 || n > 16) return NVF_EINVAL;
  WgReduceMulti d{};
  int base = 0, m = 0;
  for (int i = 0; i < n; ++i) {
    if (nslabs[i] == 0) continue;
    if (!slabs[i] || !dws[i] || nslabs[i] < 0 || jtotals[i] <= 0) return NVF_EINVAL;
    d.slabs[m] = slabs[i]; d.dw[m] = dws[i]; d.nslab[m] = nslabs[i]; d.jtotal[m] = jtotals[i];
    d.blk_base[m] = base;
    base += (jtotals[i] + 63) / 64;
    ++m;
  }
  d.blk_base[m] = base;
  d.n = m;
  if (m == 0) return NVF_OK;
  wgrad_reduce_multi<<<base, 1024, 0, nvf_stream(stream)>>>(d);
  NVF_LAUNCH_CHECK();
  return NVF_OK;
}


__global__ __launch_bounds__(256) void channel_sum_partial(const float* __restrict__ x, float* __restrict__ part,
                                                           int batch, int c, int spatial, int chunk) {
  __shared__ float red[16];
  const int ch = blockIdx.x, g = blockIdx.y;
  const long total = (long)batch * spatial;
  const long lo = (long)g * chunk;
  long hi = lo + chunk;
  if (hi > total) hi = total;
  float s = 0.f;
  for (long e = lo + threadIdx.x; e < hi; e += blockDim.x) {
    const long n = e / spatial, sp = e % spatial;
    s += x[((size_t)n * c + ch) * spatial + sp];
  }
  s = nvf_block_sum(s, red);
  if (threadIdx.x == 0) part[(size_t)g * c + ch] = s;
}

__global__ void channel_sum_final(const float* __restrict__ part, float* __restrict__ out, int c, int nchunk,
                                  int accumulate) {
  const int ch = blockIdx.x * blockDim.x + threadIdx.x;
  if (ch >= c) return;
  float s = 0.f;
  for (int g = 0; g < nchunk; ++g) s += part[(size_t)g * c + ch];
  out[ch] = accumulate ? out[ch] + s : s;
}

extern "C" size_t nvf_channel_sum_workspace(int c) { return (size_t)kSumChunks * c * sizeof(float); }

extern "C" int nvf_channel_sum(const float* x, float* out, void* workspace, size_t workspace_bytes, int batch, int c,
                               int spatial, int accumulate, void* stream) {
  if (!x || !out || !workspace || batch <= 0 || c <= 0 || spatial <= 0) return NVF_EINVAL;
  if (workspace_bytes < nvf_channel_sum_workspace(c)) return NVF_EWORKSPACE;
  const long total = (long)batch * spatial;
  long chunk = (total + kSumChunks - 1) / kSumChunks;
  if (chunk < 1024) chunk = 1024;
  const int nchunk = (int)((total + chunk - 1) / chunk);
  hipStream_t s = nvf_stream(stream);
  channel_sum_partial<<<dim3(c, nchunk), 256, 0, s>>>(x, (float*)workspace, batch, c, spatial, (int)chunk);
  channel_sum_final<<<(c + 63) / 64, 64, 0, s>>>((const float*)workspace, out, c, nchunk, accumulate);
  NVF_LAUNCH_CHECK();
  return NVF_OK;
}


__global__ __launch_bounds__(NVF_SUM_T) void multi_channel_sum_partial(MultiSumDesc d, float* __restrict__ part) {
  __shared__ float red[16];
  multi_channel_sum_partial_body<NVF_SUM_T>(d, part, blockIdx.x, blockIdx.y, red);
}

__global__ __launch_bounds__(1024) void wgrad_reduce_and_sums(WgReduceMulti r, int r_blocks, MultiSumDesc m,
                                                              float* __restrict__ part) {
  __shared__ float sm[16][64];
  const int bid = blockIdx.x;
  if (bid < r_blocks) { wgrad_reduce_multi_body(r, bid, sm); return; }
  const int q = bid - r_blocks;
// ... 224 lines not shown
```

### nvfpcc_amd/engine.py

```python
import functools
import os
from typing import NamedTuple

import numpy as np
import torch

from . import ops
from ._lib import lib, check
from .network import NoiseState

R, S, NONE = ops.ACT_RELU, ops.ACT_SIGMOID, ops.ACT_NONE
_WINO = os.environ.get("NVF_WINO", "1") != "0"


def _wino_bwd_ppc(g_out):
    if g_out.shape[0] <= 64:
        return 0
    return 18 if g_out.shape[-1] == 32 else 10


_HEAD_BIAS_IN_LOSS = True
_SUMS_IN_TRUNK5 = True
_STEM_IN_TRUNK5 = True
_STEM_IN_HEAD = True
_HEADS_IN_TRUNK5 = True


class StepPlan(NamedTuple):
    want_w: bool
    want_emb: bool
    stem_fwd: str
    latent_fwd_fused: bool
    heads: str
    head_bias_in_loss: bool
    heads_in_trunk5: bool
    trunk5: bool
    conv0_wgrad_in_stem: bool
    stem_bwd: str
    tail_queued: bool
    sums_in_trunk5: bool
    fused_optimiser: bool


@functools.lru_cache(maxsize=None)
def plan_step(narrow, wide, winograd, fused_stem, fused_latent_stem, heads3, ch, batch, want_w, want_emb, fuse, hook,
              naive, head_bias_in_loss, sums_in_trunk5, stem_in_trunk5, stem_in_head, heads_in_trunk5,
              step_head=False, defer_heads=False):
    tuned = naive == 0
    small = batch <= 32
    stem_fwd = ("head" if step_head and stem_in_head and fused_stem and fused_latent_stem and small and tuned else
                "latent" if ch <= 8 and tuned and fused_stem and fused_latent_stem else
                "fused" if fused_stem else "layers")
    fused_loss = heads3 and small and tuned
    heads = (("deferred" if defer_heads and want_w else "fused_loss") if fused_loss else
             "heads3" if heads3 else "layers")
    trunk5 = want_w and narrow and tuned
    in_trunk5 = trunk5 and heads3 and heads_in_trunk5
    tail = want_w and not want_emb and ch <= 8 and tuned
    stem_bwd = ("queued" if stem_in_trunk5 and tail and in_trunk5 and fused_stem and small else
                "layers" if not fused_stem else "partial" if want_w else "plain")
    return StepPlan(want_w=want_w, want_emb=want_emb, stem_fwd=stem_fwd, latent_fwd_fused=ch <= 8 and tuned, heads=heads,
                    head_bias_in_loss=want_w and head_bias_in_loss and fused_loss, heads_in_trunk5=in_trunk5,
                    trunk5=trunk5, conv0_wgrad_in_stem=want_w and fused_stem and not trunk5, stem_bwd=stem_bwd,
                    tail_queued=tail, sums_in_trunk5=in_trunk5 and sums_in_trunk5, fused_optimiser=fuse and not hook)


TRUNK = ("up0", "conv0", "up1", "conv1", "up2", "conv2", "conv2_cls")
HEADS = ("conv1_cls", "conv0_cls")
MFMA_BWD = {"conv1": (2, 64), "conv2": (0, 64)}

_DESC = np.dtype([("kernel", "<u8"), ("kernel_init", "<u8"), ("b", "<u8"), ("b_init", "<u8"), ("w_fwd", "<u8"),
                  ("w_bwd", "<u8"), ("b_eff", "<u8"), ("dim0", "<i4"), ("dim1", "<i4"), ("k3", "<i4"),
                  ("kind", "<i4"), ("quantised", "<i4"), ("layer_id", "<i4"), ("nbias", "<i4"), ("pad", "<i4")])


class _Layer:
    __slots__ = ("name", "mod", "kind", "k", "w_fwd", "w_bwd", "b_eff", "gk", "gb", "cin", "cout", "pad", "wp_f",
                 "wp_b", "wp_t", "wp_tr", "wp_s", "wp_gf", "wp_gb", "wp_t16", "wp_w", "wp_wf", "bwd_pair", "bwd_max_batch")


class TrainEngine:
    def __init__(self, net, gt_all, dist_all, n_points_total, lmbda, w1, w2, lr, wemb, emb=None, seed=0, winograd=None):
        assert lib().nvf_layer_desc_size() == _DESC.itemsize
        self.winograd = _WINO if winograd is None else bool(winograd)
        self.net = net
        self.dev = gt_all.device
        self.gt, self.dist = gt_all.contiguous(), dist_all.contiguous()
        self.N_leaf = self.gt.shape[0]
        self.n_points_total = float(n_points_total)
        self.lmbda, self.w1, self.w2 = float(lmbda), float(w1), float(w2)
        self.lr, self.lr_emb = float(lr), float(lr) * float(wemb)
        self.seed = int(seed)
        self.noise_step = 0
        self.rate_grad_scale = 1.0
        self.grad_hook = None
        self.opt_step = 0
        self.emb_step = 0
        self.ch = net.entropy_coder.sigma.shape[1]
        self.channels = net.reconstructor.channels
        self.gt16 = ops.maxpool2(self.gt)
        self.gt8 = ops.maxpool2(self.gt16)
        self.counts = self.gt.sum(dim=(1, 2, 3, 4)).double().cpu().numpy()
        self.emb = (torch.ones(self.N_leaf, self.ch, 2, 2, 2, device=self.dev) if emb is None
                    else emb.detach().to(self.dev).float().contiguous().clone())
        self.emb_m = torch.zeros_like(self.emb)
        self.emb_v = torch.zeros_like(self.emb)
        chans = tuple(net.reconstructor.channels)
        self.narrow = chans == (8, 16, 8, 8)
        self.wide = chans == (16, 32, 16, 16)
        self.generic = not (self.narrow or self.wide)
        self._flatten_parameters()
        self._build_layers()
        self.last = {}
        self._step_dev = None
        self.fused_stem = (self.narrow or self.wide) and net.entropy_coder.sigma.shape[1] <= 8
        self.fused_latent_stem = True
        self._g_lat_dev = None
        self._wg = None
        self.ctx = ops.StepCtx()
        self.ctx.set_direct(not self.winograd)
        self.epoch_acc = None
        self._tail_done = torch.zeros(2, dtype=torch.int32, device=self.dev)
        self._coef_live = torch.zeros(2, device=self.dev)
        self._rate = None
        self._rate_ready = False
        self._rate_retired = []
        self._graphs_captured = 0
        self.tail_done = False
        self._tail_ranges = {}
        self.collective_mode = None
        self.heads3 = self.narrow or self.wide

    def _flatten_parameters(self):
        named = list(self.net.named_parameters())
        total = sum(p.numel() for _, p in named)
        self.flat_p = torch.empty(total, device=self.dev)
        self.flat_gx = torch.zeros(total + 32, device=self.dev)
        self.flat_g = self.flat_gx[:total]
        self.step_counts = self.flat_gx[total:total + 18]
        self.flat_m = torch.zeros(total, device=self.dev)
        self.flat_v = torch.zeros(total, device=self.dev)
        self.slices = {}
        off = 0
        for name, p in named:
            n = p.numel()
            self.flat_p[off:off + n].copy_(p.detach().reshape(-1))
            p.data = self.flat_p[off:off + n].view(p.shape)
            p.grad = self.flat_g[off:off + n].view(p.shape)
            self.slices[name] = (off, n)
            off += n

    def _g(self, name):
        off, n = self.slices[name]
        return self.flat_g[off:off + n]

    def _build_layers(self):
        rec = self.net.reconstructor
        mods = [("latent", self.net.latent_gen.h_analysis_2, "latent_gen.h_analysis_2")]
        mods += [(n, getattr(rec, n), "reconstructor." + n) for n in TRUNK + HEADS]
        self.layers = {}
        table = np.zeros(len(mods), _DESC)
        for i, (name, m, prefix) in enumerate(mods):
            L = _Layer()
            L.name, L.mod = name, m
            L.kind = 1 if m.kernel.shape[2] == 5 else 0
            L.k = m.kernel.shape[2]
            n = m.kernel.numel()
            L.w_fwd = torch.empty(n, device=self.dev)
            L.w_bwd = torch.empty(n, device=self.dev)
            L.b_eff = torch.empty(m.b.numel(), device=self.dev)
            L.gk, L.gb = self._g(prefix + ".kernel").view(m.kernel.shape), self._g(prefix + ".b")
            L.cin, L.cout, L.pad = m.in_channels, m.out_channels, m.padding
            L.wp_f = L.wp_b = L.wp_t = L.wp_tr = L.wp_s = L.wp_gf = L.wp_gb = L.wp_t16 = L.wp_w = L.wp_wf = None
            L.bwd_pair, L.bwd_max_batch = 2, 0
            if self.narrow and L.k == 5 and L.cin % 4 == 0 and L.cout == 8 and L.pad == 0 and name in ("up1", "up2"):
                L.wp_t = torch.empty(int(lib().nvf_pack_convT_mfma_floats(L.cin)), device=self.dev)
                if self.winograd:
                    L.wp_tr = torch.empty((L.cin // 4) * 65 * 64, device=self.dev)
                if L.cin in (8, 16):
                    L.wp_s = torch.empty(int(lib().nvf_pack_s2k5_mfma_floats(L.cout, L.cin)), device=self.dev)
            if self.narrow and L.k == 4 and L.cin % 4 == 0 and L.cout == 8 and L.cin == 8 and L.pad == 0:
                L.wp_f = torch.empty(int(lib().nvf_pack_mfma_k4_floats(L.cin, 0)), device=self.dev)
                if name in MFMA_BWD:
                    L.bwd_pair, L.bwd_max_batch = MFMA_BWD[name]
                    L.wp_b = torch.empty(int(lib().nvf_pack_mfma_k4_floats(L.cout, L.bwd_pair)), device=self.dev)
                if self.winograd and name in ("conv2", "conv1"):
                    L.wp_w = torch.empty(int(lib().nvf_pack_wino_k4_floats()), device=self.dev)
                    L.wp_wf = torch.empty(int(lib().nvf_pack_wino_k4_floats()), device=self.dev)
            if self.wide and L.k == 4 and L.cin == 16 and L.cout == 16 and L.pad == 0 and name in ("conv1", "conv2"):
                L.wp_gf = torch.empty(int(lib().nvf_pack_g16_mfma_floats(16, 16, 4)), device=self.dev)
                L.wp_gb = torch.empty(int(lib().nvf_pack_g16_mfma_floats(16, 16, 4)), device=self.dev)
                if self.winograd:
                    L.wp_w = torch.empty(int(lib().nvf_pack_wino16_k4_floats()), device=self.dev)
                    if name == "conv2":
                        L.wp_wf = torch.empty(int(lib().nvf_pack_wino16_k4_floats()), device=self.dev)
            if self.wide and L.k == 5 and L.cout == 16 and L.cin in (16, 32) and L.pad == 0 and name in ("up1", "up2"):
                L.wp_gb = torch.empty(int(lib().nvf_pack_g16_mfma_floats(16, L.cin, 5)), device=self.dev)
            if self.wide and L.k == 5 and (name, L.cin, L.cout, L.pad) in (("up1", 32, 16, 0), ("up2", 16, 16, 0),
                                                                      ("conv0", 16, 32, 2), ("up0", 8, 16, 2)):
                L.wp_t16 = torch.empty(int(lib().nvf_pack_convT16_mfma_floats(L.cin, L.cout)), device=self.dev)
            if self.wide and name == "up0" and L.cin == 8 and L.cout == 16 and L.pad == 2:
                L.wp_gb = torch.empty(int(lib().nvf_pack_g16_mfma_floats(16, 8, 5)), device=self.dev)
            if self.wide and name == "conv0" and L.cin == 16 and L.cout == 32 and L.pad == 2:
                L.wp_gb = torch.empty(int(lib().nvf_pack_g16_mfma_floats(32, 16, 5)), device=self.dev)
            self.layers[name] = L
            t = table[i]
            t["kernel"], t["kernel_init"] = m.kernel.data_ptr(), m.kernel_init.data_ptr()
            t["b"], t["b_init"] = m.b.data_ptr(), m.b_init.data_ptr()
            t["w_fwd"], t["w_bwd"], t["b_eff"] = L.w_fwd.data_ptr(), L.w_bwd.data_ptr(), L.b_eff.data_ptr()
            t["dim0"], t["dim1"], t["k3"] = m.kernel.shape[0], m.kernel.shape[1], L.k ** 3
            t["kind"] = L.kind
            t["quantised"] = 1 if name in TRUNK else 0
            t["layer_id"] = m.layer_id
            t["nbias"] = m.b.numel()
        row = {name: i for i, (name, _, _) in enumerate(mods)}
        self._rows = row
        wk, wc = (41, 16) if self.wide else (40, 8)
        packs = (("wp_f", "w_fwd", lambda L: (0, L.cin, 8)),
                 ("wp_b", "w_bwd", lambda L: (L.bwd_pair, L.cout, 8)),
                 ("wp_w", "w_bwd", lambda L: (wk, L.cout, wc)),
                 ("wp_wf", "w_fwd", lambda L: (wk, L.cin, wc)),
                 ("wp_t", "w_fwd", lambda L: (10, L.cin, 8)),
                 ("wp_tr", "w_fwd", lambda L: (12, L.cin, 8)),
                 ("wp_s", "w_bwd", lambda L: (20, L.cout, L.cin)),
                 ("wp_gf", "w_fwd", lambda L: (30, L.cin, L.cout)),
                 ("wp_gb", "w_bwd", lambda L: (30 if L.k == 4 else 31, L.cout, L.cin)),
                 ("wp_t16", "w_fwd", lambda L: (11, L.cin, L.cout)))
        jobs, meta = [], []
        for slot, src, form in packs:
            for nm, L in self.layers.items():
                if getattr(L, slot) is not None:
                    jobs.append((getattr(L, src), getattr(L, slot)) + form(L))
                    meta.append((row[nm], int(src == "w_bwd")))
        assert len(jobs) <= 16
        self._mfma_jobs = jobs
        self._mfma_job_layers = meta
        self._table_host = table
        self.table = torch.from_numpy(table.view(np.uint8).copy()).to(self.dev)
        self.nlayers = len(mods)

    def _rate_job(self):
        key = (self.rate_grad_scale, self.lmbda, self.w2, self.n_points_total)
        if self._rate is not None and self._rate[2] != key:
            if self._graphs_captured:
                raise RuntimeError("weight-rate coefficients changed after a step graph was captured "
                                   "(attach data parallelism / set lambda before building GraphedTrainStep)")
            self._rate_retired.append(self._rate)
        if self._rate is None or self._rate[2] != key:
            lm = self.net.reconstructor.likelihood_model
            ks = [self.layers[n].mod.kernel for n in TRUNK]
            dk = torch.zeros(sum(k.numel() for k in ks), device=self.dev)
            dks, off = [], 0
            for k in ks:
                dks.append(dk[off:off + k.numel()])
                off += k.numel()
            part = torch.zeros(3 * 512, device=self.dev)
            g = self.lmbda * self.w2 / self.n_points_total * self.rate_grad_scale
            job = ops.rate_job(ks, dks, lm.sigma, lm.mu, part, g)
            add = {self.layers[n].gk.data_ptr(): d for n, d in zip(TRUNK, dks)}
            self._rate = (job, add, key, dk, part)
        return self._rate

    def _plan(self, batch, want_w=False, want_emb=False, fuse=False, step_head=False, defer_heads=False):
        return plan_step(self.narrow, self.wide, self.winograd, self.fused_stem, self.fused_latent_stem, self.heads3,
                         self.ch, batch, want_w, want_emb, fuse, self.grad_hook is not None, ops._NAIVE,
                         _HEAD_BIAS_IN_LOSS, _SUMS_IN_TRUNK5, _STEM_IN_TRUNK5, _STEM_IN_HEAD, _HEADS_IN_TRUNK5,
                         step_head, defer_heads)

    def _noise(self):
        sd = self._step_dev
        return (0 if sd is not None else self.noise_step), sd

    def _ec(self):
        ec = self.net.entropy_coder
        return ec.sigma.reshape(-1), ec.mu.reshape(-1)

    def batch_and_prepare(self, idx_dev, q, with_rate=False, stem_mode=None):
        import ctypes
        srcs = [self.gt, self.dist, self.gt16, self.gt8, self.emb]
        n, rows = len(srcs), idx_dev.numel()
        dsts = [torch.empty((rows,) + tuple(s.shape[1:]), device=s.device) for s in srcs]
        step, sd = self._noise()
        jobs, meta = self._mfma_jobs, self._mfma_job_layers
        npk = len(jobs)
        iarr = lambda xs: (ctypes.c_int * max(len(xs), 1))(*xs)
        args = (self.table.data_ptr(), self.nlayers, int(q), self.seed, step, None if sd is None else sd.data_ptr(),
                (ctypes.c_void_p * max(npk, 1))(*[j[1].data_ptr() for j in jobs]), iarr([j[2] for j in jobs]),
                iarr([j[3] for j in jobs]), iarr([j[4] for j in jobs]), iarr([m[0] for m in meta]),
                iarr([m[1] for m in meta]), npk, (ctypes.c_void_p * n)(*[s.data_ptr() for s in srcs]),
                (ctypes.c_void_p * n)(*[d.data_ptr() for d in dsts]), (ctypes.c_int * n)(*[s[0].numel() for s in srcs]), n,
                idx_dev.data_ptr(), rows, ctypes.byref(self._rate_job()[0]) if with_rate else None)
        o = None
        if self._plan(rows, step_head=stem_mode is not None).stem_fwd == "head":
            from ._lib import NvfStemHead
            net = self.net
            g2, ec, ig = net.latent_gen.gdn_2, net.entropy_coder, net.reconstructor.activation
            dev, ch = self.dev, self.ch
            c0, c1 = self.channels[0], self.channels[1]
            o = {"h": torch.empty(rows, ch, 2, 2, 2, device=dev), "lat": torch.empty(rows, ch, 2, 2, 2, device=dev),
                 "x0": torch.empty(rows, ch, 2, 2, 2, device=dev), "lbits": torch.empty(1, device=dev),
                 "a0": torch.empty(rows, c0, 4, 4, 4, device=dev), "h0": torch.empty(rows, c0, 4, 4, 4, device=dev),
                 "y1": torch.empty(rows, c1, 8, 8, 8, device=dev)}
            sj = NvfStemHead()
            sj.emb, sj.lat_beta_hat, sj.lat_gamma_hat = self.emb.data_ptr(), g2.beta.data_ptr(), g2.gamma.data_ptr()
            sj.sigma, sj.mu = ec.sigma.data_ptr(), ec.mu.data_ptr()
            sj.beta_hat, sj.gamma_hat = ig.beta.data_ptr(), ig.gamma.data_ptr()
            sj.h, sj.lat, sj.x_rounded, sj.bits = (o[k].data_ptr() for k in ("h", "lat", "x0", "lbits"))
            sj.a0, sj.h0, sj.y1 = (o[k].data_ptr() for k in ("a0", "h0", "y1"))
            sj.lat_row, sj.up0_row, sj.conv0_row = self._rows["latent"], self._rows["up0"], self._rows["conv0"]
            sj.mode, sj.ch, sj.c0, sj.c1 = (0 if stem_mode == "train" else 1), ch, c0, c1
            check(lib().nvf_step_head_stem(*args, ctypes.byref(sj), torch.cuda.current_stream().cuda_stream),
                  "nvf_step_head_stem")
        else:
            check(lib().nvf_step_head(*args, torch.cuda.current_stream().cuda_stream), "nvf_step_head")
        self._rate_ready = bool(with_rate)
        return dsts if stem_mode is None else dsts + [o]

    def prepare_weights(self, q):
        step, sd = self._noise()
        check(lib().nvf_prepare_weights(self.table.data_ptr(), self.nlayers, int(q), self.seed, step,
                                        None if sd is None else sd.data_ptr(),
                                        torch.cuda.current_stream().cuda_stream), "nvf_prepare_weights")
        if self._mfma_jobs:
            ops.pack_mfma_all(self._mfma_jobs)

    def _convT(self, L, x, act, train=False):
        if L.wp_t16 is not None:
            return ops.convT3d_k5s2_mfma16(x, L.wp_t16, L.b_eff, act, cout=L.cout, pad=L.pad)
        if L.wp_t is not None:
            if train and L.wp_tr is not None:
                return ops.convT3d_k5s2_mfma(x, L.wp_tr, L.b_eff, act, variant=15)
            return ops.convT3d_k5s2_mfma(x, L.wp_t, L.b_eff, act, variant=5)
        return ops.convT3d_k5s2_fwd(x, L.w_fwd, L.b_eff, L.cout, L.pad, act)

    def _conv(self, L, x, act, train=False):
        if train and L.wp_wf is not None and act == R and (self.wide or x.shape[-1] == 35 or x.shape[0] > 64):
            if self.wide:
                return ops.conv3d_k4_wino16_fwd(x, L.wp_wf, L.b_eff)
            if x.shape[-1] == 19:
                return ops.conv3d_k4_wino_fwd(x, L.wp_wf, L.b_eff, ppc=8)
            return ops.conv3d_k4_wino_fwd(x, L.wp_wf, L.b_eff, ppc=16 if x.shape[0] > 64 else 0)
        if L.wp_gf is not None:
            osz = tuple(s - 3 for s in x.shape[2:])
            return ops.conv3d_g16_mfma(x, L.wp_gf, L.b_eff, L.cout, 4, 1, 0, osz, act)
        if L.wp_f is not None:
            var = 5 if (x.shape[-1] == 19 and x.shape[0] >= 64) else None
            return ops.conv3d_k4_mfma(x, L.wp_f, L.b_eff, 0, 0, act, variant=var)
        osz = tuple(s + 2 * L.pad - L.k + 1 for s in x.shape[2:])
        return ops.conv3d_gather(x, L.w_fwd, L.b_eff, L.cout, L.k, 1, L.pad, osz, act)

    def forward(self, e, mode, block_ids, defer_heads=False, stem=None):
        net, Ls = self.net, self.layers
        a = {"e": e}
        plan = self._plan(e.shape[0], want_w=defer_heads, step_head=stem is not None, defer_heads=defer_heads)
        g2 = net.latent_gen.gdn_2
        ig = net.reconstructor.activation
        step, sd = self._noise()
        noise = dict(block_ids=block_ids, seed=self.seed, step=step, step_dev=sd)
        if plan.stem_fwd == "head":
            a.update(stem)
        elif plan.stem_fwd == "latent":
            (a["h"], a["lat"], a["x0"], a["lbits"], a["a0"], a["h0"], a["y1"]) = ops.stem_latent_fwd(
                e, Ls["latent"].w_fwd, Ls["latent"].b_eff, g2.beta, g2.gamma, *self._ec(), mode, Ls["up0"].w_fwd,
                Ls["up0"].b_eff, ig.beta, ig.gamma, Ls["conv0"].w_fwd, Ls["conv0"].b_eff, **noise)
        elif plan.latent_fwd_fused:
            a["h"], a["lat"], a["x0"], a["lbits"] = ops.latent_fwd(
                e, Ls["latent"].w_fwd, Ls["latent"].b_eff, g2.beta, g2.gamma, *self._ec(), mode, **noise)
        else:
            a["h"] = self._conv(Ls["latent"], e, NONE)
            a["lat"] = ops.gdn_fwd(a["h"], g2.beta, g2.gamma, False)
            a["x0"], a["lbits"], _, _, _ = ops.latent_rate(a["lat"], *self._ec(), mode, **noise)
        if plan.stem_fwd == "fused":
            a["a0"], a["h0"], a["y1"] = ops.stem_fwd(a["x0"], Ls["up0"].w_fwd, Ls["up0"].b_eff, ig.beta, ig.gamma,
                                                     Ls["conv0"].w_fwd, Ls["conv0"].b_eff)
        elif plan.stem_fwd == "layers":
            a["a0"] = self._convT(Ls["up0"], a["x0"], NONE)
            a["h0"] = ops.gdn_fwd(a["a0"], ig.beta, ig.gamma, True)
            a["y1"] = self._convT(Ls["conv0"], a["h0"], R)
        if plan.heads == "layers":
            a["p0"] = self._conv(Ls["conv0_cls"], a["y1"], S)
        a["y2"] = self._convT(Ls["up1"], a["y1"], R, train=(mode == "train"))
        a["y3"] = self._conv(Ls["conv1"], a["y2"], R, train=(mode == "train"))
        if plan.heads == "layers":
            a["p1"] = self._conv(Ls["conv1_cls"], a["y3"], S)
        a["y4"] = self._convT(Ls["up2"], a["y3"], R, train=(mode == "train"))
        a["y5"] = self._conv(Ls["conv2"], a["y4"], R, train=(mode == "train"))
        if plan.heads == "deferred":
            a["p0"] = a["p1"] = a["p2"] = None
        elif plan.heads != "layers":
            hl = [Ls["conv0_cls"], Ls["conv1_cls"], Ls["conv2_cls"]]
            a["p0"], a["p1"], a["p2"] = ops.heads3_fwd([a["y1"], a["y3"], a["y5"]], [L.w_fwd for L in hl],
                                                       [L.b_eff for L in hl])
        else:
            a["p2"] = self._conv(Ls["conv2_cls"], a["y5"], S)
        return a

    def _wgrad_conv(self, L, g_out, x_in, sums):
        if (self.wide and self.winograd and L.k == 4 and L.cin == 16 and L.cout == 16 and L.pad == 0
                and g_out.shape[-1] in (32, 16)):
            base = self._wg.reserve(256 * 16384 * 4)
            n = ops.wgrad16_k4_wino_partial(g_out, x_in, base, zsplit=0 if g_out.shape[-1] == 32 else 8)
            self._wg.add_job(base, L.gk, n, 16384)
        else:
            self._wg.add(g_out, x_in, L.k, 1, L.pad, 0, L.gk)
        sums.append((g_out, L.gb))

    def _wgrad_convT(self, L, g_out, x_in, sums):
        self._wg.add(x_in, g_out, 5, 2, L.pad, 0, L.gk)
        sums.append((g_out, L.gb))

    def _dx_conv(self, L, g_out, x_in, mask=None, addend=None, bias_out=None, sums=None):
        slabs = False
        if self.wide and L.wp_w is not None and mask is not None and addend is None and g_out.shape[-1] in (32, 16):
            dx = ops.conv3d_k4_wino16_bwd(g_out, L.wp_w, mask)
        elif L.wp_gb is not None:
            dx = ops.conv3d_g16_mfma(g_out, L.wp_gb, None, L.cin, 4, 1, 3, tuple(x_in.shape[2:]), addend=addend,
                                     mask=mask)
        elif L.wp_w is not None and mask is not None and addend is None and g_out.shape[-1] in (32, 16):
            if bias_out is not None and g_out.shape[0] <= 64:
                base = self._wg.reserve(16384 * 8 * 4)
                dx, nparts = ops.conv3d_k4_wino_bwd(g_out, L.wp_w, mask, bias_part=base)
                self._wg.add_job(base, bias_out, nparts, 8)
                slabs = True
            else:
                dx = ops.conv3d_k4_wino_bwd(g_out, L.wp_w, mask, ppc=_wino_bwd_ppc(g_out))
        elif L.wp_b is not None and g_out.shape[0] <= L.bwd_max_batch:
            if bias_out is not None and mask is not None and addend is None:
                base = self._wg.reserve(4096 * 8 * 4)
                dx, nparts = ops.conv3d_k4_mfma(g_out, L.wp_b, None, 3, L.bwd_pair, NONE, mask=mask, bias_part=base)
                self._wg.add_job(base, bias_out, nparts, 8)
                slabs = True
            else:
                dx = ops.conv3d_k4_mfma(g_out, L.wp_b, None, 3, L.bwd_pair, NONE, addend=addend, mask=mask)
        else:
            dx = ops.conv3d_gather(g_out, L.w_bwd, None, L.cin, L.k, 1, L.k - 1 - L.pad, tuple(x_in.shape[2:]),
                                   addend=addend, mask=mask)
        if bias_out is not None and not slabs:
            sums.append((dx, bias_out))
        return dx

    def _dx_convT(self, L, g_out, x_in, mask=None, addend=None):
        if L.wp_gb is not None:
            return ops.conv3d_g16_mfma(g_out, L.wp_gb, None, L.cin, 5, 2, L.pad, tuple(x_in.shape[2:]), addend=addend,
                                       mask=mask)
        if L.wp_s is not None:
            if L.cin == 16:
                var = 2 if g_out.shape[0] > 64 else (7 if self.winograd else None)
            else:
                var = 6 if g_out.shape[0] <= 64 else 5
            return ops.conv3d_s2k5_mfma(g_out, L.wp_s, L.cin, addend=addend, mask=mask, variant=var)
        return ops.conv3d_gather(g_out, L.w_bwd, None, L.cin, 5, 2, L.pad, tuple(x_in.shape[2:]), addend=addend,
                                 mask=mask)

    def backward(self, *args, **kw):
        try:
            return self._backward(*args, **kw)
        except BaseException:
            self.ctx.cancel()
            raise

    def _backward(self, a, gt, dist, gt16, gt8, n_pts, mode, block_ids, want_w, want_emb, fuse=None):
        deferred = a.get("p2") is None
        plan = self._plan(a["e"].shape[0], want_w, want_emb, fuse is not None, defer_heads=deferred)
        if deferred and plan.heads != "deferred":
            raise ValueError("forward(defer_heads=True) must be followed by a backward pass with weight gradients "
                             "(want_w=True): the heads' forward runs in that pass's loss launch")
        if self._wg is None:
            self._wg = ops.WgradBatch(self.dev, nbytes=(256 if self.wide else 128) << 20, ctx=self.ctx)
        loss = torch.empty(4, device=self.dev)
        nbits = torch.empty(7, device=self.dev)
        if want_w:
            self.ctx.begin()
        sums = []
        t0, t1, g5, heads_job = self._bwd_loss_heads(plan, a, gt, dist, gt16, gt8, loss, sums)
        g4, g3, g2, g1 = self._bwd_trunk(plan, a, t0, t1, g5, sums)
        da0, dx0, stem_jobs = self._bwd_stem(plan, a, g1, sums)
        de, tail = self._bwd_latent(plan, a, dx0, n_pts, mode, block_ids, sums)
        sums_done = False
        if plan.trunk5:
            Ls = self.layers
            sums_done = plan.sums_in_trunk5 and self._rate_ready
            self._wg.add_trunk5([g5, a["y3"], g3, a["y1"], a["h0"]], [a["y4"], g4, a["y2"], g2, g1],
                                [Ls["conv2"].gk, Ls["up2"].gk, Ls["conv1"].gk, Ls["up1"].gk, Ls["conv0"].gk],
                                bias_outs=(Ls["conv2"].gb, Ls["conv1"].gb), heads=heads_job,
                                sums=([t for t, _ in sums], [o for _, o in sums]) if sums_done else None,
                                coef=((fuse["coef_dev"], self._coef_live)
                                      if (fuse is not None and fuse.get("coef_dev") is not None) else None),
                                stem_jobs=stem_jobs)
        last = {"loss_terms": loss, "latent_bits": a["lbits"], "net_bits": nbits, "n_pts": n_pts}
        self._bwd_finish(plan, sums, sums_done, last, fuse)
        self.last = last
        return de

    def _bwd_loss_heads(self, plan, a, gt, dist, gt16, gt8, loss, sums):
        Ls = self.layers
        want_w = plan.want_w
        ctx = self.ctx if want_w else None
        hl = [Ls["conv0_cls"], Ls["conv1_cls"], Ls["conv2_cls"]]

        def step_metrics():
            if self.epoch_acc is not None and want_w:
                ops.metrics3([a["p2"], a["p0"], a["p1"]], [gt, gt8, gt16], [dist, None, None], 0.5, 0.6,
                             out=self.step_counts, ctx=ctx)
        bias_outs = [L.gb for L in hl] if plan.head_bias_in_loss else None
        terms = ([gt8, gt16, gt], [None, None, dist], [0.85, 0.85, 0.9], [0.0, 0.0, 1.0], [1, 2, 0], loss, [L.w_bwd for L in hl])
        if plan.heads == "deferred":
            (a["p0"], a["p1"], a["p2"]), (dl0, dl1, dl2), (t0, t1, g5) = ops.heads3_fwd_loss_bwd_data(
                [a["y1"], a["y3"], a["y5"]], [L.w_fwd for L in hl], [L.b_eff for L in hl], *terms, [None, None, a["y5"]],
                self.ctx, bias_outs=bias_outs)
            step_metrics()
        elif plan.heads == "fused_loss":
            step_metrics()
            (dl0, dl1, dl2), (t0, t1, g5) = ops.heads3_loss_bwd_data(
                [a["p0"], a["p1"], a["p2"]], *terms, [L.cin for L in hl], [None, None, a["y5"]], ctx=ctx, bias_outs=bias_outs)
        else:
            dl2, dl0, dl1 = ops.focal_loss_multi([(a["p2"], gt, dist, 0.9, 1.0), (a["p0"], gt8, None, 0.85, 0.0),
                                                  (a["p1"], gt16, None, 0.85, 0.0)], loss, ctx=ctx)
            step_metrics()
        if plan.heads == "layers":
            t1 = self._dx_conv(Ls["conv1_cls"], dl1, a["y3"])
            t0 = self._dx_conv(Ls["conv0_cls"], dl0, a["y1"])
            if want_w:
                self._wgrad_conv(Ls["conv2_cls"], dl2, a["y5"], sums)
                self._wgrad_conv(Ls["conv1_cls"], dl1, a["y3"], sums)
                self._wgrad_conv(Ls["conv0_cls"], dl0, a["y1"], sums)
            g5 = self._dx_conv(Ls["conv2_cls"], dl2, a["y5"], mask=a["y5"])
            return t0, t1, g5, None
        if plan.heads == "heads3":
            t0, t1, g5 = ops.heads3_bwd_data([dl0, dl1, dl2], [L.w_bwd for L in hl], [L.cin for L in hl],
                                             [None, None, a["y5"]])
        heads_job = None
        if want_w:
            heads_job = ([dl0, dl1, dl2], [a["y1"], a["y3"], a["y5"]], [L.gk for L in hl])
            if not plan.heads_in_trunk5:
                self._wg.add_heads3(*heads_job)
                heads_job = None
            if not plan.head_bias_in_loss:
                sums += [(dl2, hl[2].gb), (dl1, hl[1].gb), (dl0, hl[0].gb)]
        return t0, t1, g5, heads_job

    def _bwd_trunk(self, plan, a, t0, t1, g5, sums):
        Ls = self.layers
        each = plan.want_w and not plan.trunk5
        if each:
            self._wgrad_conv(Ls["conv2"], g5, a["y4"], sums)
        g4 = self._dx_conv(Ls["conv2"], g5, a["y4"], mask=a["y4"], bias_out=Ls["up2"].gb if plan.trunk5 else None, sums=sums)
        if each:
            self._wgrad_convT(Ls["up2"], g4, a["y3"], sums)
        g3 = self._dx_convT(Ls["up2"], g4, a["y3"], mask=a["y3"], addend=t1)
        if each:
            self._wgrad_conv(Ls["conv1"], g3, a["y2"], sums)
        g2 = self._dx_conv(Ls["conv1"], g3, a["y2"], mask=a["y2"], bias_out=Ls["up1"].gb if plan.trunk5 else None, sums=sums)
        if each:
            self._wgrad_convT(Ls["up1"], g2, a["y1"], sums)
        g1 = self._dx_convT(Ls["up1"], g2, a["y1"], mask=a["y1"], addend=t0)
        if plan.trunk5 or plan.conv0_wgrad_in_stem:
            sums.append((g1, Ls["conv0"].gb))
        elif plan.want_w:
            self._wgrad_convT(Ls["conv0"], g1, a["h0"], sums)
        return g4, g3, g2, g1

    def _gdn_grads(self, prefix, mod, want_w):
        if not want_w:
            return None, None
        return self._g(prefix + ".beta"), self._g(prefix + ".gamma").view(mod.gamma.shape)

    def _bwd_stem(self, plan, a, g1, sums):
        Ls = self.layers
        ig = self.net.reconstructor.activation
        dbeta, dgamma = self._gdn_grads("reconstructor.activation", ig, plan.want_w)
        if plan.stem_bwd == "queued":
            return ops.stem_bwd_queue(g1, a["x0"], a["a0"], Ls["conv0"].w_bwd, Ls["up0"].w_bwd, ig.beta, ig.gamma, dbeta,
                                      dgamma, Ls["up0"].gk, Ls["up0"].gb, self.ctx)
        if plan.stem_bwd == "partial":
            wg0 = plan.conv0_wgrad_in_stem
            da0, dx0 = ops.stem_bwd_partial(g1, a["x0"], a["a0"], Ls["conv0"].w_bwd, Ls["up0"].w_bwd, ig.beta,
                                            ig.gamma, dbeta, dgamma, Ls["up0"].gk, self._wg, ctx=self.ctx,
                                            h0=a["h0"] if wg0 else None, dw_conv0=Ls["conv0"].gk if wg0 else None)
            sums.append((da0, Ls["up0"].gb))
        elif plan.stem_bwd == "plain":
            da0, dx0 = ops.stem_bwd(g1, a["x0"], a["a0"], Ls["conv0"].w_bwd, Ls["up0"].w_bwd, ig.beta, ig.gamma)
        else:
            dh0 = self._dx_convT(Ls["conv0"], g1, a["h0"])
            da0, _, _ = ops.gdn_bwd(a["a0"], ig.beta, ig.gamma, dh0, True, dbeta, dgamma)
            if plan.want_w:
                self._wgrad_convT(Ls["up0"], da0, a["x0"], sums)
            dx0 = self._dx_convT(Ls["up0"], da0, a["x0"])
        return da0, dx0, None

    def _bwd_latent(self, plan, a, dx0, n_pts, mode, block_ids, sums):
        Ls = self.layers
        want_w = plan.want_w
        step, sd = self._noise()
        g_lat = self.lmbda * self.w1 / n_pts if self._g_lat_dev is None else 1.0
        g2m = self.net.latent_gen.gdn_2
        dsigma, dmu = (self._g("entropy_coder.sigma"), self._g("entropy_coder.mu")) if want_w else (None, None)
        dbeta, dgamma = self._gdn_grads("latent_gen.gdn_2", g2m, want_w)
        if plan.tail_queued:
            dlat, dh = torch.empty_like(a["lat"]), torch.empty_like(a["h"])
            ops.latent_tail_queue(self.ctx, a["lat"], *self._ec(), mode, block_ids, dx0, dlat, dsigma, dmu,
                                  self._g_lat_dev, g_lat, self.seed, step, sd, a["h"], g2m.beta, g2m.gamma, dh, dbeta,
                                  dgamma, a["e"], Ls["latent"].gk, Ls["latent"].gb)
            return None, (dlat, dh)
        _, _, dlat, _, _ = ops.latent_rate(a["lat"], *self._ec(), mode, block_ids=block_ids, want_grad=True, g_host=g_lat,
                                           g_dev=self._g_lat_dev, seed=self.seed, step=step, step_dev=sd,
                                           dx_addend=dx0, dsigma_out=dsigma, dmu_out=dmu)
        dh, _, _ = ops.gdn_bwd(a["h"], g2m.beta, g2m.gamma, dlat, False, dbeta, dgamma)
        if want_w:
            self._wgrad_conv(Ls["latent"], dh, a["e"], sums)
        return (self._dx_conv(Ls["latent"], dh, a["e"]) if plan.want_emb else None), None

    def _bwd_finish(self, plan, sums, sums_done, last, fuse):
        Ls, nbits = self.layers, last["net_bits"]
        lm = self.net.reconstructor.likelihood_model
        kernels = [Ls[n].mod.kernel for n in TRUNK]
        rate_head, self._rate_ready = self._rate_ready and plan.want_w, False
        self.tail_done = False
        if not plan.want_w:
            ops.weight_rate_batch(kernels, None, lm.sigma, lm.mu, nbits)
            return
        gs, gm = self._g("reconstructor.likelihood_model.sigma"), self._g("reconstructor.likelihood_model.mu")
        addends = fused = None
        if rate_head:
            job, addends = self._rate_job()[:2]
            live = {out for out, _ in self._wg.live_outputs()}
            if not all(Ls[n].gk.data_ptr() in live for n in TRUNK) or len(self._wg.jobs) > 16:
                rate_head, addends = False, None
        if plan.fused_optimiser and rate_head:
            fused = tail, adam, ranges = self._fused_tail(plan, fuse, sums, last, gs, gm)
            self.tail_done = True
        one_launch = sums_done and rate_head
        if not one_launch:
            todo = [] if sums_done else sums
            self._wg.finish_with_sums([t for t, _ in todo], [o for _, o in todo], addends=addends,
                                      adam=adam if fused else None)
        if rate_head:
            ops.weight_rate_final(job, nbits, gs, gm, ctx=self.ctx)
        else:
            g_net = self.lmbda * self.w2 / self.n_points_total
            ops.weight_rate_batch(kernels, [Ls[n].gk for n in TRUNK], lm.sigma, lm.mu, nbits, gs, gm,
                                  g_host=g_net * self.rate_grad_scale, ctx=self.ctx)
        if one_launch and fused:
            if fuse.get("coef_dev") is not None:
                adam.coef_dev = self._coef_live.data_ptr()
            self._wg.finish_and_flush_tail(addends, adam, tail, ranges)
        elif one_launch:
            self._wg.finish_and_flush(addends)
        elif fused:
            self.ctx.flush_tail(tail, ranges)
        else:
            self.ctx.flush()

    def _tail_kw(self, last):
        stats = self.epoch_acc is not None
        return dict(p=self.flat_p, g=self.flat_g, m=self.flat_m, v=self.flat_v,
                    loss_terms=last["loss_terms"] if stats else None, lbits=last["latent_bits"] if stats else None,
                    nbits=last["net_bits"] if stats else None, nbits_scale=1.0 / self.n_points_total,
                    counts=self.step_counts if stats else None, acc=self.epoch_acc, done=self._tail_done)

    def _fused_tail(self, plan, tail, sums, last, gs, gm):
        t = ops.step_tail_args(**tail, **self._tail_kw(last))
        outs = [o for _, o in sums] + [gs, gm]
        if plan.head_bias_in_loss:
            outs += [self.layers[n].gb for n in ("conv0_cls", "conv1_cls", "conv2_cls")]
        if plan.stem_bwd in ("queued", "partial"):
            outs += [self._g("reconstructor.activation.beta"), self._g("reconstructor.activation.gamma")]
        base = self.flat_g.data_ptr()
        cover = [((ptr - base) // 4, (ptr - base) // 4 + cnt)
                 for ptr, cnt in self._wg.live_outputs() + [(o.data_ptr(), o.numel()) for o in outs]]
        n = self.flat_g.numel()
        key = tuple(sorted(c for c in cover if 0 <= c[0] < n))
        ranges = self._tail_ranges.get(key)
        if ranges is None:
            ranges, pos = [], 0
            for lo, hi in key:
                if lo < pos:
                    raise RuntimeError("fused tail: two launches write the same gradient elements")
                if lo > pos:
                    ranges.append((pos, lo))
                pos = hi
            if pos < n:
                ranges.append((pos, n))
            if len(ranges) > 16:
                raise RuntimeError("fused tail: more than 16 uncovered gradient ranges")
            self._tail_ranges[key] = ranges
        return t, ops.adam_fuse_args(t), ranges

    def _batch(self, idx_dev):
        return ops.gather_rows_multi([self.gt, self.dist, self.gt16, self.gt8, self.emb], idx_dev)

    def enable_epoch_stats(self):
        if self.epoch_acc is None:
            self.epoch_acc = torch.zeros(16, device=self.dev)

    def read_epoch_stats(self, reset=True, reduce=None, world=1):
        acc = self.epoch_acc.clone()
        if reduce is not None:
            reduce(acc)
        acc = acc.double().cpu().numpy()
        if reduce is not None and world > 1:
            acc[4] /= world
            acc[7:16] /= world
        if reset:
            self.epoch_acc.zero_()
        if acc[5] > 0:
            raise ValueError("Problem in loss: %d non-finite objective terms this epoch" % int(acc[5]))
        if acc[6] > 0:
            raise ValueError("Problem with grad: %d non-finite gradient entries this epoch" % int(acc[6]))
        return acc

    def train_log_fields(self, acc, nsteps, peak=1023):
        cnt = float(nsteps)
        ls, bl, bn = acc[0:3] / cnt, acc[3] / cnt, acc[4] / cnt
        with np.errstate(divide="ignore", invalid="ignore"):
            mse1 = np.float64(acc[14]) / np.float64(acc[15])
            psnr1 = 20 * np.log10(peak / np.sqrt(mse1 / 3))
        loss = ls.sum() + self.lmbda * (bl * self.w1 + bn * self.w2)
        return [loss, 0.0, 0.0, acc[8] / cnt, acc[9] / cnt, ls[1], ls[2], acc[10] / cnt, acc[11] / cnt,
                acc[12] / cnt, acc[13] / cnt, bl + bn, bl, bn, mse1, psnr1]

    def _tail(self, n_pts):
        if self.grad_hook is not None:
            self.grad_hook(self.flat_gx)
        self.opt_step += 1
        ops.step_tail(coef_host=ops.adam_coefficients(self.lr, self.opt_step), inv_npts_host=1.0 / n_pts,
                      **self._tail_kw(self.last))

    def _idle_backward(self):
        net, Ls = self.net, self.layers
        self.flat_gx.zero_()
        lm = net.reconstructor.likelihood_model
        nbits = torch.empty(7, device=self.dev)
        g_net = self.lmbda * self.w2 / self.n_points_total
        ops.weight_rate_batch([Ls[n].mod.kernel for n in TRUNK], [Ls[n].gk for n in TRUNK], lm.sigma, lm.mu, nbits,
                              self._g("reconstructor.likelihood_model.sigma"),
                              self._g("reconstructor.likelihood_model.mu"), g_host=g_net * self.rate_grad_scale)
        self.last = {"loss_terms": torch.zeros(4, device=self.dev), "latent_bits": torch.zeros(1, device=self.dev),
                     "net_bits": nbits, "n_pts": 1.0}

    def train_step(self, idx_host, q, idx_dev=None, update=True, n_pts=None):
        idx_host = np.asarray(idx_host, np.int64)
        self.noise_step += 1
        a = None
        if idx_host.shape[0] == 0:
# ... 9 lines not shown
            tail = None
            if update and self.grad_hook is None:
                tail = dict(coef_host=ops.adam_coefficients(self.lr, self.opt_step + 1), inv_npts_host=1.0 / n_pts)
            self.backward(a, gt, dist, gt16, gt8, n_pts, "train", idx_dev, want_w=True, want_emb=False, fuse=tail)
            if tail is not None and self.tail_done:
                self.opt_step += 1
                update = False
        if update:
            self._tail(n_pts)
        elif self.grad_hook is not None:
            self.grad_hook(self.flat_gx)
        return a

    def latent_step(self, q, lo=0, hi=None, update=True):
        hi = self.N_leaf if hi is None else hi
        self.noise_step += 1
        ids = torch.arange(lo, hi, device=self.dev)
        n_pts = float(self.counts.sum())
        self.prepare_weights(q)
        e = self.emb[lo:hi]
        a = self.forward(e, "train", ids)
        de = self.backward(a, self.gt[lo:hi], self.dist[lo:hi], self.gt16[lo:hi], self.gt8[lo:hi], n_pts, "train",
                           ids, want_w=False, want_emb=True)
        if update:
            self.emb_step += 1
            ops.adam_step(self.emb[lo:hi].view(-1), de.view(-1), self.emb_m[lo:hi].view(-1),
                          self.emb_v[lo:hi].view(-1), self.lr_emb, self.emb_step)
        return a, de

    def eval_forward(self, lo=0, hi=None, q=2):
        hi = self.N_leaf if hi is None else hi
        ids = torch.arange(lo, hi, device=self.dev)
        self.prepare_weights(q)
        return self.forward(self.emb[lo:hi], "eval", ids)

    def eval_sums(self, lo=0, hi=None, q=2):
        hi = self.N_leaf if hi is None else hi
        out = torch.zeros(22, device=self.dev)
        if hi <= lo:
            return out
        a = self.eval_forward(lo, hi, q)
        loss = torch.empty(4, device=self.dev)
        gt, dist, gt16, gt8 = self.gt[lo:hi], self.dist[lo:hi], self.gt16[lo:hi], self.gt8[lo:hi]
        ops.focal_loss_multi([(a["p2"], gt, dist, 0.9, 1.0), (a["p0"], gt8, None, 0.85, 0.0),
                              (a["p1"], gt16, None, 0.85, 0.0)], loss)
        c = ops.metrics3([a["p2"], a["p0"], a["p1"]], [gt, gt8, gt16], [dist, None, None], 0.5, 0.6)
        out[0:3] = loss[0:3]
        out[3:21] = c[0:18]
        out[21] = a["lbits"].reshape(-1)[0]
        return out

    def weight_bits(self):
        nbits = torch.empty(7, device=self.dev)
        lm = self.net.reconstructor.likelihood_model
        ops.weight_rate_batch([self.layers[n].mod.kernel for n in TRUNK], None, lm.sigma, lm.mu, nbits)
        return float(nbits.sum().item())

    def loss_value(self):
        t = self.last
        terms = t["loss_terms"].cpu().numpy()
        b_latent = t["latent_bits"].item() / t["n_pts"]
        b_net = t["net_bits"].sum().item() / self.n_points_total
        return float(terms[0] + terms[1] + terms[2] + self.lmbda * (b_latent * self.w1 + b_net * self.w2))


class GraphedTrainStep:

    CAP = 4096
    UNROLL = (16, 8, 4, 2)

    def __init__(self, eng, batch, q, ring=2, collective=None, unroll=None):
        self.eng, self.batch, self.q = eng, batch, q
        un = self.UNROLL if unroll is None else ((unroll,) if isinstance(unroll, int) else tuple(unroll))
        self.unrolls = tuple(u for u in sorted({max(int(v), 1) for v in un}, reverse=True) if u > 1)
        self.unroll = self.unrolls[0] if self.unrolls else 1
        dev = eng.dev
        if collective is None:
            collective = getattr(eng, "collective_mode", None) or os.environ.get("NVF_GRAPH_COLLECTIVE", "host")
        self.collective = collective if eng.grad_hook is not None else "none"
        nw = self.nw = batch + 3
        self.sched = torch.zeros(nw + 2 + (self.CAP + 1) * nw, dtype=torch.int64, device=dev)
        self.buf = self.sched[:nw]
        self.cursor, self.rows = self.sched[nw:nw + 1], self.sched[nw + 2:]
        self.pins = [torch.zeros(self.sched.numel(), dtype=torch.int64).pin_memory() for _ in range(max(int(ring), 1))]
        self.pin_np = [p.numpy() for p in self.pins]
        self.pin_events = [None] * len(self.pins)
        self.pin_gen = [0] * len(self.pins)
        self.loads = 0
        self.pending = []
        self.idx = self.buf[:batch]
        self.step = self.buf[batch:batch + 1]
        rate = self.buf[batch + 1:batch + 2].view(torch.float32)
        self.g_lat, self.inv_npts = rate[0:1], rate[1:2]
        self.coef = self.buf[batch + 2:batch + 3].view(torch.float32)
        eng._step_dev, eng._g_lat_dev = self.step, self.g_lat
        first = torch.zeros(nw, dtype=torch.int64)
        first[:batch] = torch.arange(batch) % eng.N_leaf
        first[batch + 1:batch + 2].view(torch.float32)[:] = 1.0
        self.buf.copy_(first)
        side = torch.cuda.Stream()
        side.wait_stream(torch.cuda.current_stream())
        acc = eng.epoch_acc
        try:
            with torch.cuda.stream(side):
                for _ in range(2):
                    self._body(tail=False)
            torch.cuda.current_stream().wait_stream(side)
            torch.cuda.synchronize()
            if self.collective == "graph":
                try:
                    self._capture(True)
                except Exception as e:
                    import warnings
                    warnings.warn(f"all-reduce could not be captured into the step graph ({e}); launching it from "
                                  f"the host behind the graph instead")
                    torch.cuda.synchronize()
                    self.collective = eng.collective_mode = "host"
                    self._capture(False)
            else:
                self._capture(self.collective != "host")
        finally:
            eng._step_dev, eng._g_lat_dev = None, None

    def _capture(self, tail):
        self.graph = torch.cuda.CUDAGraph()
        with torch.cuda.graph(self.graph):
            self._body(tail=tail)
        self.eng._graphs_captured += 1
        self.out1, self.last1 = self.out, self.last
        self.graphs_u = {}
        for u in (self.unrolls if tail else ()):
            g = torch.cuda.CUDAGraph()
            with torch.cuda.graph(g):
                for _ in range(u):
                    self._body(tail=tail)
            self.graphs_u[u] = (g, self.out, self.last)
        self.graph_u = self.graphs_u[self.unroll][0] if self.graphs_u else None

    def _body(self, tail):
        eng = self.eng
        gt, dist, gt16, gt8, e, stem = eng.batch_and_prepare(self.idx, self.q, with_rate=True, stem_mode="train")
        a = eng.forward(e, "train", self.idx, defer_heads=True, stem=stem)
        spec = None
        if tail and eng.grad_hook is None:
            spec = dict(coef_dev=self.coef, inv_npts_dev=self.inv_npts, sched=(self.buf, self.rows, self.cursor, self.nw))
        eng.backward(a, gt, dist, gt16, gt8, 1.0, "train", self.idx, want_w=True, want_emb=False, fuse=spec)
        self.out = a
        self.last = dict(eng.last)
        if tail and not (spec is not None and eng.tail_done):
            self._tail()

    def _tail(self):
        eng = self.eng
        if eng.grad_hook is not None:
            eng.grad_hook(eng.flat_gx)
        ops.step_tail(coef_dev=self.coef, inv_npts_dev=self.inv_npts, sched=(self.buf, self.rows, self.cursor, self.nw),
                      **eng._tail_kw(self.last))

    def stage_schedule(self, steps):
        eng, B, nw = self.eng, self.batch, self.nw
        def is2d(x):
            if isinstance(x, np.ndarray) or torch.is_tensor(x):
                return x.ndim == 2
            return (isinstance(x, (list, tuple)) and len(x) > 0 and
                    all(isinstance(r, (list, tuple, np.ndarray)) and np.ndim(r) == 1 for r in x))
        arrays = len(steps) == 2 and is2d(steps[0])
        if arrays and torch.is_tensor(steps[0]):
            steps = (steps[0].cpu().numpy(), steps[1].cpu().numpy() if torch.is_tensor(steps[1]) else steps[1])
        if arrays:
            ids_all, npts = np.asarray(steps[0], np.int64), np.asarray(steps[1], np.float64)
        else:
            ids_all = np.stack([np.asarray(ids, np.int64).reshape(-1) for ids, _ in steps]) if len(steps) else np.zeros((0, B), np.int64)
            npts = np.array([float(eng.counts[ids_all[k]].sum()) if p is None else float(p)
                             for k, (_, p) in enumerate(steps)], np.float64)
        n = ids_all.shape[0]
        if not (0 < n <= self.CAP):
            raise ValueError("load_schedule: 1..%d steps" % self.CAP)
        if ids_all.shape != (n, B) or npts.shape != (n,):
            raise ValueError("load_schedule: ids must be [n, %d] and n_pts [n]; got %s, %s" % (B, ids_all.shape, npts.shape))
        slot = self.loads % len(self.pins)
        self.loads += 1
        if self.pin_events[slot] is not None:
            self.pin_events[slot].synchronize()
        host = self.pin_np[slot]
        rows = host[nw + 2:nw + 2 + (n + 1) * nw].reshape(n + 1, nw)
        f32 = rows.view(np.float32)
        rows[:n, :B] = ids_all
        rows[:n, B] = eng.noise_step + 1 + np.arange(n)
        f32[:n, 2 * (B + 1)] = (eng.lmbda * eng.w1 / npts).astype(np.float32)
        f32[:n, 2 * (B + 1) + 1] = (1.0 / npts).astype(np.float32)
        f32[:n, 2 * (B + 2):2 * (B + 2) + 2] = ops.adam_coefficients_n(eng.lr, eng.opt_step + 1, n)
        rows[n] = rows[n - 1]
        host[:nw] = rows[0]
        host[nw], host[nw + 1] = 1, 0
        self.pin_gen[slot] += 1
        m = nw + 2 + (n + 1) * nw
        return {"_staged": True, "slot": slot, "gen": self.pin_gen[slot], "n": n, "npts": npts.tolist(), "words": m,
                "src": self.pins[slot][:m], "dst": self.sched[:m],
                "state": (eng.noise_step, eng.opt_step, eng.lr, eng.lmbda, eng.w1)}

    def load_schedule(self, steps):
        eng = self.eng
        if self.pending:
            raise ValueError("load_schedule: only after every loaded step has been replayed")
        h = steps if (isinstance(steps, dict) and steps.get("_staged")) else self.stage_schedule(steps)
        if h["state"] != (eng.noise_step, eng.opt_step, eng.lr, eng.lmbda, eng.w1):
            raise ValueError("load_schedule: the staged schedule was made for other step counters / coefficients")
        slot, m = h["slot"], h["words"]
        if h.get("gen") != self.pin_gen[slot]:
            raise ValueError("load_schedule: stale handle -- its staging slot has been filled again since (ring=%d)"
                             % len(self.pins))
        self.pending.extend(h["npts"])
        h["dst"].copy_(h["src"], non_blocking=True)
        ev = self.pin_events[slot]
        if ev is None:
            ev = self.pin_events[slot] = torch.cuda.Event()
        ev.record()

    def replay(self):
        eng = self.eng
        n_pts = self.pending.pop(0)
        eng.noise_step += 1
        eng.opt_step += 1
        self.graph.replay()
        self.out, self.last = self.out1, self.last1
        eng.last = dict(self.last)
        eng.last["n_pts"] = n_pts
        if self.collective == "host":
            self._tail()
        return self.out

    def replay_all(self):
        eng = self.eng
        n, sizes = len(self.pending), []
        for U in self.unrolls:
            if U in self.graphs_u:
                while n >= U:
                    sizes.append(U)
                    n -= U
        sizes += [1] * n
        for U in reversed(sizes):
            if U == 1:
                self.replay()
                continue
            g, out, last = self.graphs_u[U]
            n_pts = self.pending[U - 1]
            del self.pending[:U]
            eng.noise_step += U
            eng.opt_step += U
            g.replay()
            self.out, self.last = out, last
            eng.last = dict(self.last)
            eng.last["n_pts"] = n_pts
        return self.out

    def prime(self, rounds=1):
        B, N = self.batch, self.eng.N_leaf
        sizes = [u for u in self.unrolls if u in self.graphs_u] + [1]
        n = 0
        for _ in range(max(int(rounds), 1)):
            for u in sizes:
                self.load_schedule([((np.arange(B) + k * B) % N, None) for k in range(u)])
                self.replay_all()
                n += u
        torch.cuda.synchronize()
        return n

    def __call__(self, idx_host, n_pts=None):
        self.load_schedule([(idx_host, n_pts)])
        return self.replay()


class EpochDriver:

    def __init__(self, eng, batch, rank=0, world=1, use_graph=True):
        from . import dist as nd
        self.eng, self.batch, self.rank, self.world, self.use_graph = eng, int(batch), rank, world, use_graph
# ... 39 lines not shown
```

### nvfpcc_amd/ops.py

```python
import torch

from ._lib import lib, check

ACT_NONE, ACT_RELU, ACT_SIGMOID = 0, 1, 2
_NAIVE = 0


def set_naive(flag):
    global _NAIVE
    _NAIVE = int(bool(flag))


def set_variant(v):
    global _NAIVE
    _NAIVE = int(v)


def _ptr(t):
    return None if t is None else t.data_ptr()


def _stream():
    return torch.cuda.current_stream().cuda_stream

# ... 654 lines not shown
    def add_up1_conv0(self, ps, qs, outs):
        _f32(*ps, *qs, *outs)
        self._grouped("nvf_wgrad_up1_conv0_partial", lambda bases, nsl: lib().nvf_wgrad_up1_conv0_partial(
            _parr(ps), _parr(qs), bases, ps[0].shape[0], nsl, _stream()), outs, (16000, 16000), 512)

    def add_trunk5(self, ps, qs, outs, bias_outs=None, heads=None, sums=None, coef=None, stem_jobs=None):
        import ctypes
        _f32(*ps, *qs, *outs)
        B = ps[0].shape[0]
        self.sums_done = False
        jt = (4096, 8000, 4096, 16000, 16000) + ((8, 8) if bias_outs is not None else ())
        sizes = [512 * j * 4 for j in jt]
        if heads is not None:
            hd, hx, ho = heads
            _f32(*hd, *hx, *ho)
            hcs = [x.shape[1] for x in hx]
            sizes += [_HEADS_SLABS * c * 27 * 4 for c in hcs]
        bases = self._alloc(sizes)
        nsl = (ctypes.c_int * 5)()
        hn = (ctypes.c_int * 3)()
        if heads is not None and sums is not None:
            st, so = sums
            _f32(*st, *so)
            total = sum(t.shape[1] for t in st)
            ws = workspace(lib().nvf_multi_channel_sum_workspace(total), st[0].device, "mchsum", self.ctx)
            check(lib().nvf_wgrad_trunk5_heads_sums_partial(
                _parr(ps), _parr(qs), (ctypes.c_void_p * 5)(*bases[:5]), (ctypes.c_void_p * 3)(bases[5], None, bases[6]),
                _parr(hd), _parr(hx), (ctypes.c_void_p * 3)(*bases[7:10]), _HEADS_SLABS, _parr(st), _parr(so),
                _iarr([t.shape[1] for t in st]), _iarr([t[0, 0].numel() for t in st]), len(st), _ptr(ws), ws.numel(),
                _ptr(coef[0]) if coef else None, _ptr(coef[1]) if coef else None, B,
                nsl, hn, _ctx(self.ctx), _stream()), "nvf_wgrad_trunk5_heads_sums_partial")
            self.sums_done = True
        elif heads is not None:
            check(lib().nvf_wgrad_trunk5_heads_partial(
                _parr(ps), _parr(qs), (ctypes.c_void_p * 5)(*bases[:5]), (ctypes.c_void_p * 3)(bases[5], None, bases[6]),
                _parr(hd), _parr(hx), (ctypes.c_void_p * 3)(*bases[7:10]), _HEADS_SLABS, B, nsl, hn, _ctx(self.ctx),
                _stream()), "nvf_wgrad_trunk5_heads_partial")
        elif bias_outs is None:
            check(lib().nvf_wgrad_trunk5_partial(_parr(ps), _parr(qs), (ctypes.c_void_p * 5)(*bases[:5]), B, nsl,
                                                 _ctx(self.ctx), _stream()), "nvf_wgrad_trunk5_partial")
        else:
            _f32(*bias_outs)
            check(lib().nvf_wgrad_trunk5_partial_bias(_parr(ps), _parr(qs), (ctypes.c_void_p * 5)(*bases[:5]),
                                                      (ctypes.c_void_p * 3)(bases[5], None, bases[6]), B, nsl,
                                                      _ctx(self.ctx), _stream()), "nvf_wgrad_trunk5_partial_bias")
        self._check_slabs("add_trunk5", nsl, (512,) * 5)
        if heads is not None:
            self._check_slabs("add_trunk5 (heads)", hn, (_HEADS_SLABS,) * 3)
        self.jobs += stem_jobs or []
        if heads is not None:
            self.jobs += [(bases[7 + h], ho[h].data_ptr(), hn[h], hcs[h] * 27) for h in range(3)]
        self.jobs += [(bases[h], outs[h].data_ptr(), nsl[h], jt[h]) for h in range(5)]
        if bias_outs is not None:
            self.jobs.append((bases[5], bias_outs[0].data_ptr(), nsl[0], 8))
            self.jobs.append((bases[6], bias_outs[1].data_ptr(), nsl[2], 8))

    def add_heads3(self, dls, xs, outs, max_slabs=_HEADS_SLABS):
        _f32(*dls, *xs, *outs)
        cs = [x.shape[1] for x in xs]
        self._grouped("nvf_heads3_wgrad_partial", lambda bases, nsl: lib().nvf_heads3_wgrad_partial(
            _parr(dls), _parr(xs), bases, _iarr(cs), _iarr([x.shape[-1] for x in xs]), xs[0].shape[0], max_slabs, nsl,
            _stream()), outs, [c * 27 for c in cs], max_slabs)

    def finish_with_sums(self, tensors, outs, addends=None, adam=None):
        import ctypes
        if not self.jobs or len(self.jobs) > 16 or not tensors:
            if addends or adam is not None:
                raise RuntimeError("finish_with_sums: addends / fused Adam need the one-launch reduction")
            self.finish()
            if tensors:
                multi_channel_sum(tensors, outs, ctx=self.ctx)
            return
        jobs = self._take_jobs()
        _f32(*tensors)
        _f32(*outs)
        total = sum(t.shape[1] for t in tensors)
        ws = workspace(lib().nvf_multi_channel_sum_workspace(total), tensors[0].device, "mchsum", self.ctx)
        check(lib().nvf_wgrad_reduce_multi_and_sums_fused(
            *self._job_arrays(jobs, addends), None if adam is None else ctypes.byref(adam),
            _parr(tensors), _parr(outs), _iarr([t.shape[1] for t in tensors]), _iarr([t[0, 0].numel() for t in tensors]),
            len(tensors), tensors[0].shape[0], _ptr(ws), ws.numel(), _ctx(self.ctx), _stream()),
            "nvf_wgrad_reduce_multi_and_sums_fused")

    def finish_and_flush_tail(self, addends, adam, tail, ranges):
        import ctypes
        if not (0 < len(self.jobs) <= 16) or self.ctx is None:
            raise RuntimeError("finish_and_flush_tail: 1..16 reduction jobs and a step context are required")
        jobs = self._take_jobs()
        flat = [int(v) for r in ranges for v in r]
        arr = (ctypes.c_int64 * max(len(flat), 1))(*flat)
        check(lib().nvf_wgrad_reduce_finals_tail(*self._job_arrays(jobs, addends), ctypes.byref(adam), _ctx(self.ctx),
                                                 ctypes.byref(tail), arr, len(ranges), _stream()),
              "nvf_wgrad_reduce_finals_tail")

    def finish_and_flush(self, addends):
        if not (0 < len(self.jobs) <= 16) or self.ctx is None:
            raise RuntimeError("finish_and_flush: 1..16 reduction jobs and a step context are required")
        jobs = self._take_jobs()
        check(lib().nvf_wgrad_reduce_finals(*self._job_arrays(jobs, addends), _ctx(self.ctx), _stream()),
              "nvf_wgrad_reduce_finals")

    def finish(self):
        jobs = self._take_jobs()
        for i in range(0, len(jobs), 16):
            bases, outs, nslabs, sizes, n, _ = self._job_arrays(jobs[i:i + 16])
            check(lib().nvf_wgrad_reduce_multi(bases, outs, nslabs, sizes, n, _stream()), "nvf_wgrad_reduce_multi")


def channel_sum(x, out=None, accumulate=False):
    _f32(x)
    B, c = x.shape[0], x.shape[1]
    spatial = x[0, 0].numel()
    o = out if out is not None else torch.empty(c, device=x.device)
    ws = workspace(lib().nvf_channel_sum_workspace(c), x.device, "chsum")
    check(lib().nvf_channel_sum(_ptr(x), _ptr(o), _ptr(ws), ws.numel(), B, c, spatial, int(accumulate), _stream()),
          "nvf_channel_sum")
    return o


def multi_channel_sum(tensors, outs, ctx=None):
    import ctypes
    _f32(*tensors)
    _f32(*outs)
    n = len(tensors)
    B = tensors[0].shape[0]
    xs = (ctypes.c_void_p * n)(*[t.data_ptr() for t in tensors])
    os_ = (ctypes.c_void_p * n)(*[t.data_ptr() for t in outs])
    cs = (ctypes.c_int * n)(*[t.shape[1] for t in tensors])
    sp = (ctypes.c_int * n)(*[t[0, 0].numel() for t in tensors])
    total = sum(t.shape[1] for t in tensors)
    ws = workspace(lib().nvf_multi_channel_sum_workspace(total), tensors[0].device, "mchsum", ctx)
    check(lib().nvf_multi_channel_sum(xs, os_, cs, sp, n, B, _ptr(ws), ws.numel(), _ctx(ctx), _stream()),
          "nvf_multi_channel_sum")


def gdn_fwd(x, beta_hat, gamma_hat, inverse):
    _f32(x, beta_hat, gamma_hat)
    B, c = x.shape[0], x.shape[1]
    y = torch.empty_like(x)
    check(lib().nvf_gdn_fwd(_ptr(x), _ptr(beta_hat), _ptr(gamma_hat), _ptr(y), B, c, x[0, 0].numel(), int(inverse),
                            _stream()), "nvf_gdn_fwd")
    return y


def gdn_bwd(x, beta_hat, gamma_hat, dy, inverse, dbeta_out=None, dgamma_out=None):
    _f32(x, beta_hat, gamma_hat, dy, dbeta_out, dgamma_out)
    B, c = x.shape[0], x.shape[1]
    dx = torch.empty_like(x)
    dbeta = dbeta_out if dbeta_out is not None else torch.empty_like(beta_hat)
    dgamma = dgamma_out if dgamma_out is not None else torch.empty_like(gamma_hat)
    ws = workspace(lib().nvf_gdn_bwd_workspace(c), x.device, "gdn")
    check(lib().nvf_gdn_bwd(_ptr(x), _ptr(beta_hat), _ptr(gamma_hat), _ptr(dy), _ptr(dx), _ptr(dbeta), _ptr(dgamma),
                            _ptr(ws), ws.numel(), B, c, x[0, 0].numel(), int(inverse), _stream()), "nvf_gdn_bwd")
    return dx, dbeta, dgamma


def latent_fwd(e, w_fwd, bias, beta_hat, gamma_hat, sigma, mu, mode, block_ids=None, seed=0, step=0, step_dev=None):
    _f32(e, w_fwd, bias, beta_hat, gamma_hat, sigma, mu)
    _chk(block_ids)
    B, c = e.shape[0], e.shape[1]
    h, lat, xr = torch.empty_like(e), torch.empty_like(e), torch.empty_like(e)
    bits = torch.empty(1, device=e.device)
    check(lib().nvf_latent_fwd(_ptr(e), _ptr(w_fwd), _ptr(bias), _ptr(beta_hat), _ptr(gamma_hat), _ptr(block_ids),
                               _ptr(sigma), _ptr(mu), _ptr(h), _ptr(lat), _ptr(xr), _ptr(bits), B, c, e[0, 0].numel(),
                               0 if mode == "train" else 1, int(seed), int(step), _ptr(step_dev), _stream()),
          "nvf_latent_fwd")
    return h, lat, xr, bits


def latent_rate(x, sigma, mu, mode, u=None, block_ids=None, want_grad=False, g_dev=None, g_host=1.0, seed=0,
                step=0, dx_addend=None, dsigma_out=None, dmu_out=None, step_dev=None):
    _f32(x, sigma, mu, u, g_dev, dx_addend)
    _chk(block_ids)
    B, c = x.shape[0], x.shape[1]
    xr = torch.empty_like(x)
    bits = torch.empty(1, device=x.device)
# ... 97 lines not shown
          "nvf_metrics3")
    return o


def sigmoid_bwd(dp, p):
    _f32(dp, p)
    out = torch.empty_like(p)
    check(lib().nvf_sigmoid_bwd(_ptr(dp), _ptr(p), _ptr(out), p.numel(), _stream()), "nvf_sigmoid_bwd")
    return out


def relu_bwd(dy, y):
    _f32(dy, y)
    out = torch.empty_like(y)
    check(lib().nvf_relu_bwd(_ptr(dy), _ptr(y), _ptr(out), y.numel(), _stream()), "nvf_relu_bwd")
    return out


def squared_error_map(p, dist, thh):
    _f32(p, dist)
    B = p.shape[0]
    spatial = p[0].numel()
    out = torch.empty((B, 2) + tuple(p.shape[2:]), device=p.device)
    check(lib().nvf_squared_error_map(_ptr(p), _ptr(dist), float(thh), _ptr(out), B, spatial, _stream()),
          "nvf_squared_error_map")
    return out


def maxpool2(x):
    _f32(x)
    B, c, d, h, w = x.shape
    y = torch.empty((B, c, d // 2, h // 2, w // 2), device=x.device)
    check(lib().nvf_maxpool2(_ptr(x), _ptr(y), B * c, d, h, w, _stream()), "nvf_maxpool2")
    return y


def adam_step(p, g, m, v, lr, step, beta1=0.9, beta2=0.999, eps=1e-8):
    _f32(p, g, m, v)
    check(lib().nvf_adam_step(_ptr(p), _ptr(g), _ptr(m), _ptr(v), p.numel(), float(lr), float(beta1), float(beta2),
                              float(eps), int(step), _stream()), "nvf_adam_step")


def adam_coefficients(lr, step, beta1=0.9, beta2=0.999):
    import ctypes
    c = (ctypes.c_float * 2)()
    check(lib().nvf_adam_coefficients(float(lr), float(beta1), float(beta2), int(step), c), "nvf_adam_coefficients")
    return float(c[0]), float(c[1])


def adam_coefficients_n(lr, step0, n, beta1=0.9, beta2=0.999):
    import numpy as np
    out = np.empty((n, 2), np.float32)
    check(lib().nvf_adam_coefficients_n(float(lr), float(beta1), float(beta2), int(step0), int(n),
                                        out.ctypes.data), "nvf_adam_coefficients_n")
    return out


def step_tail(p, g, m, v, coef_dev=None, coef_host=(0.0, 0.0), loss_terms=None, lbits=None, nbits=None,
              inv_npts_dev=None, inv_npts_host=1.0, nbits_scale=1.0, counts=None, acc=None, done=None, sched=None,
              beta1=0.9, beta2=0.999, eps=1e-8):
    import ctypes
    a = step_tail_args(p, g, m, v, coef_dev, coef_host, loss_terms, lbits, nbits, inv_npts_dev, inv_npts_host,
                       nbits_scale, counts, acc, done, sched, beta1, beta2, eps)
    check(lib().nvf_step_tail(ctypes.byref(a), _stream()), "nvf_step_tail")


def step_tail_args(p, g, m, v, coef_dev=None, coef_host=(0.0, 0.0), loss_terms=None, lbits=None, nbits=None,
                   inv_npts_dev=None, inv_npts_host=1.0, nbits_scale=1.0, counts=None, acc=None, done=None, sched=None,
                   beta1=0.9, beta2=0.999, eps=1e-8):
    from ._lib import NvfStepTail
    _f32(p, g, m, v, coef_dev, loss_terms, lbits, nbits, inv_npts_dev, counts, acc)
    a = NvfStepTail()
    a.p, a.g, a.m, a.v, a.n = _ptr(p), _ptr(g), _ptr(m), _ptr(v), p.numel()
    a.coef_dev, a.coef0_host, a.coef1_host = _ptr(coef_dev), float(coef_host[0]), float(coef_host[1])
    a.beta1, a.beta2, a.eps = float(beta1), float(beta2), float(eps)
    a.nnb = 0 if nbits is None else nbits.numel()
    a.loss_terms, a.lbits, a.nbits = _ptr(loss_terms), _ptr(lbits), _ptr(nbits)
    a.inv_npts_dev, a.inv_npts_host, a.nbits_scale = _ptr(inv_npts_dev), float(inv_npts_host), float(nbits_scale)
    a.counts, a.acc = _ptr(counts), _ptr(acc)
    if done is not None:
        _chk(done)
        a.done = done.data_ptr()
    if sched is not None:
        buf, rows, cursor, words = sched
        _chk(buf, rows, cursor)
        a.sched_buf, a.sched_rows, a.sched_cursor, a.sched_words = buf.data_ptr(), rows.data_ptr(), cursor.data_ptr(), int(words)
    return a


def adam_fuse_args(tail):
    from ._lib import NvfAdamFuse
    a = NvfAdamFuse()
    a.g_base, a.p_base, a.m_base, a.v_base, a.n = tail.g, tail.p, tail.m, tail.v, tail.n
    a.coef_dev, a.coef0_host, a.coef1_host = tail.coef_dev, tail.coef0_host, tail.coef1_host
    a.beta1, a.beta2, a.eps = tail.beta1, tail.beta2, tail.eps
    a.bad_count = (tail.acc + 6 * 4) if tail.acc else None
    return a


def rate_job(kernels, dks, sigma, mu, part, g):
    from ._lib import NvfRateJob
    _f32(*kernels, *[d for d in dks if d is not None], sigma, mu, part)
    j = NvfRateJob()
    for i, k in enumerate(kernels):
        j.kernel[i], j.n[i] = k.data_ptr(), k.numel()
        j.dk[i] = None if dks[i] is None else dks[i].data_ptr()
    j.nlayers = len(kernels)
    j.sigma, j.mu, j.part, j.g = sigma.data_ptr(), mu.data_ptr(), part.data_ptr(), float(g)
    return j


def weight_rate_final(job, bits, dsigma=None, dmu=None, ctx=None):
    import ctypes
    _f32(bits, dsigma, dmu)
    check(lib().nvf_weight_rate_batch_final(ctypes.byref(job), _ptr(bits), _ptr(dsigma), _ptr(dmu), _ctx(ctx), _stream()),
          "nvf_weight_rate_batch_final")


def gather_rows(src, idx):
    _f32(src)
    _chk(idx)
    if idx.dtype != torch.int64:
        raise RuntimeError("row indices must be int64")
    width = src[0].numel()
    dst = torch.empty((idx.numel(),) + tuple(src.shape[1:]), device=src.device)
    check(lib().nvf_gather_rows(_ptr(src), _ptr(idx), _ptr(dst), idx.numel(), width, _stream()), "nvf_gather_rows")
    return dst


def gather_rows_multi(srcs, idx):
    import ctypes
    _f32(*srcs)
    _chk(idx)
    n, rows = len(srcs), idx.numel()
    dsts = [torch.empty((rows,) + tuple(s.shape[1:]), device=s.device) for s in srcs]
    sp = (ctypes.c_void_p * n)(*[s.data_ptr() for s in srcs])
    dp = (ctypes.c_void_p * n)(*[d.data_ptr() for d in dsts])
    wd = (ctypes.c_int * n)(*[s[0].numel() for s in srcs])
    check(lib().nvf_gather_rows_multi(sp, dp, wd, n, _ptr(idx), rows, _stream()), "nvf_gather_rows_multi")
    return dsts


def scatter_add_rows(src, idx, dst):
    _f32(src, dst)
    _chk(idx)
    check(lib().nvf_scatter_add_rows(_ptr(src), _ptr(idx), _ptr(dst), idx.numel(), src[0].numel(), _stream()),
          "nvf_scatter_add_rows")
    return dst


def uniform(shape, device, seed, stream_id):
    out = torch.empty(shape, device=device)
    check(lib().nvf_uniform(_ptr(out), out.numel(), int(seed), int(stream_id), _stream()), "nvf_uniform")
    return out


def threshold_points(p, thh, origins=None):
    _f32(p)
    B, dim = p.shape[0], p.shape[-1]
    per_block = isinstance(thh, torch.Tensor)
    if per_block:
        _f32(thh)
        if thh.shape != (B,):
            raise RuntimeError(f"per-block thresholds must have shape ({B},), got {tuple(thh.shape)}")
    counts = torch.empty(B, dtype=torch.int32, device=p.device)
    if per_block:
        check(lib().nvf_threshold_count_v(_ptr(p), _ptr(thh), _ptr(counts), B, dim ** 3, _stream()),
              "nvf_threshold_count_v")
# ... 54 lines not shown
```

Baseline: 54020 blocks/s.

## Fuse step tail with next step's head into one seam kernel via flag sync

Adds a step_seam kernel that, inside an unrolled CUDA graph, merges the previous step's wgrad reduce, finals and fused-Adam tail with the next step's head work (stem forward, weight preparation, packing, rate partials and row gathers) in one launch. Cross-block dependencies are handled with agent-scope atomic counters and spin-waits. The gather blocks run without waiting, and the head blocks start once all tail groups have signalled. The aim is to remove a kernel boundary and the idle gap between steps. In exchange it adds spin-wait costs, atomic parameter stores, a duplicated schedule cursor, and a risk of deadlock if not every block is resident at once.

After: 53220 blocks/s. 0.985x the previous value.

```diff
diff --git a/include/nvf_hip.h b/include/nvf_hip.h
--- a/include/nvf_hip.h
+++ b/include/nvf_hip.h
@@ -367,6 +367,14 @@
                        const int* pack_c1s, const int* pack_layers, const int* pack_bwd, int npack,
                        const float* const* srcs, float* const* dsts, const int* widths, int n, const int64_t* idx,
                        int rows, const NvfRateJob* rate , const NvfStemHead* stem, void* stream);
+size_t nvf_step_seam_flags_bytes(void);
+int nvf_step_seam(const float* const* slabs, float* const* dws, const int* nslabs, const int* jtotals, int n,
+                  const float* const* addends, const NvfAdamFuse* adam, NvfStepCtx* ctx, const NvfStepTail* tail,
+                  const int64_t* ranges, int nranges, uint32_t* flags, int seam_index, int refuse, const void* table_dev,
+                  int nlayers, int q, uint64_t seed, uint64_t step, const uint64_t* step_dev, float* const* pack_dsts,
+                  const int* pack_kinds, const int* pack_c0s, const int* pack_c1s, const int* pack_layers,
+                  const int* pack_bwd, int npack, const float* const* srcs, float* const* dsts, const int* widths, int ng,
+                  const int64_t* idx, int rows, const NvfRateJob* rate_job, const NvfStemHead* stem, void* stream);
 
 int nvf_uniform(float* out, int64_t n, uint64_t seed, uint64_t stream_id, void* stream);
 
diff --git a/nvfpcc_amd/_lib.py b/nvfpcc_amd/_lib.py
--- a/nvfpcc_amd/_lib.py
+++ b/nvfpcc_amd/_lib.py
@@ -114,6 +114,9 @@
     "nvf_gather_rows_multi": (I, [P, P, P, I, P, I, P]),
     "nvf_step_head": (I, [P, I, I, U, U, P, P, P, P, P, P, P, I, P, P, P, I, P, I, P, P]),
     "nvf_step_head_stem": (I, [P, I, I, U, U, P, P, P, P, P, P, P, I, P, P, P, I, P, I, P, P, P]),
+    "nvf_step_seam": (I, [P, P, P, P, I, P, P, P, P, P, I, P, I, I,
+                          P, I, I, U, U, P, P, P, P, P, P, P, I, P, P, P, I, P, I, P, P, P]),
+    "nvf_step_seam_flags_bytes": (Z, []),
     "nvf_weight_rate_batch_final": (I, [P, P, P, P, P, P]),
     "nvf_wgrad_reduce_multi_and_sums_fused": (I, [P, P, P, P, I, P, P, P, P, P, P, I, I, P, Z, P, P]),
     "nvf_finals_flush_tail": (I, [P, P, P, I, P]),
diff --git a/nvfpcc_amd/csrc/finals.h b/nvfpcc_amd/csrc/finals.h
--- a/nvfpcc_amd/csrc/finals.h
+++ b/nvfpcc_amd/csrc/finals.h
@@ -16,7 +16,9 @@
   a.m_base[i] = mi;
   a.v_base[i] = vi;
   const float denom = sqrtf(vi) / bc2_sqrt + a.eps;
-  a.p_base[i] = a.p_base[i] - step_size * (mi / denom);
+  const float pn = a.p_base[i] - step_size * (mi / denom);
+  if (a.reserved != 0.f) __hip_atomic_store(a.p_base + i, pn, __ATOMIC_RELAXED, __HIP_MEMORY_SCOPE_AGENT);
+  else a.p_base[i] = pn;
   return 0;
 }
 __device__ __forceinline__ NvfAdamFuse adam_fuse_of(const NvfStepTail& t) {
@@ -24,6 +26,7 @@
   a.g_base = t.g; a.p_base = t.p; a.m_base = t.m; a.v_base = t.v; a.n = t.n; a.coef_dev = t.coef_dev;
   a.coef0_host = t.coef0_host; a.coef1_host = t.coef1_host; a.beta1 = t.beta1; a.beta2 = t.beta2; a.eps = t.eps;
   a.bad_count = t.acc ? t.acc + 6 : nullptr;
+  a.reserved = (t.reserved & 2) ? 1.f : 0.f;
   return a;
 }
 
@@ -257,7 +260,11 @@
   if (tid < t.sched_words) t.sched_buf[tid] = next_word;
   for (int w = tid + blockDim.x; w < t.sched_words; w += blockDim.x)
     t.sched_buf[w] = t.sched_rows[cur * (unsigned long long)t.sched_words + w];
-  if (tid == 0) { t.sched_cursor[0] = cur + 1; t.done[0] = 0u; }
+  if (tid == 0) {
+    t.sched_cursor[0] = cur + 1;
+    if ((t.reserved & 3) == 1) t.sched_cursor[1] = cur + 1;
+    t.done[0] = 0u;
+  }
 }
 
 __device__ __forceinline__ void finals_tail_body(const FinalsArgs& a, int sum_blocks, const NvfStepTail& t,
diff --git a/nvfpcc_amd/csrc/pointwise.hip b/nvfpcc_amd/csrc/pointwise.hip
--- a/nvfpcc_amd/csrc/pointwise.hip
+++ b/nvfpcc_amd/csrc/pointwise.hip
@@ -3,6 +3,7 @@
 #include "pack_mfma.h"
 #include "latent_tail.h"
 #include "stem_fwd.h"
+#include "wgrad_reduce.h"
 
 #define NVF_GRID(n, bs) ((unsigned)(((n) + (bs)-1) / (bs)))
 
@@ -64,13 +65,15 @@
   int32_t nbias, pad_;
 };
 
+template <bool DEV = false>
 __device__ __forceinline__ float effective_weight(const NvfLayerDesc& d, int i, int qq, uint64_t seed, uint64_t sid) {
-  float k = d.kernel[i];
+  float k = DEV ? nvf_load_dev(d.kernel + i) : d.kernel[i];
   if (qq == 1) k = k + (nvf_uniform01(seed, sid, (uint64_t)i) - 0.5f) * 0.0625f;
   else if (qq == 2) k = rintf(k * 16.f) / 16.f;
   return k + d.kernel_init[i];
 }
 
+template <bool DEV = false>
 __device__ __forceinline__ void prepare_weights_body(const NvfLayerDesc* __restrict__ table, int q, uint64_t seed,
                                                      uint64_t step, const uint64_t* __restrict__ step_dev, int layer,
                                                      int bx, int nbx) {
@@ -81,7 +84,7 @@
   const uint64_t sid = (st << 8) | (uint64_t)d.layer_id;
   for (int i = bx * blockDim.x + threadIdx.x; i < n + d.nbias; i += nbx * blockDim.x) {
     if (i < n) {
-      const float w = effective_weight(d, i, qq, seed, sid);
+      const float w = effective_weight<DEV>(d, i, qq, seed, sid);
       const int t = i % d.k3, i1 = (i / d.k3) % d.dim1, i0 = i / (d.k3 * d.dim1);
       if (d.kind == 0) {
         if (d.w_fwd) d.w_fwd[(i1 * d.k3 + t) * d.dim0 + i0] = w;
@@ -92,7 +95,7 @@
       }
     } else {
       const int j = i - n;
-      d.b_eff[j] = d.b[j] + d.b_init[j];
+      d.b_eff[j] = (DEV ? nvf_load_dev(d.b + j) : d.b[j]) + d.b_init[j];
     }
   }
 }
@@ -406,12 +409,13 @@
 }
 
 
+template <bool DEV = false>
 __device__ __forceinline__ void weight_rate_partial_body(const WeightRateBatch& b, const float* __restrict__ sigma,
                                                          const float* __restrict__ mu, float* __restrict__ part, float g,
                                                          int wg, int accumulate, float* red, int nthreads = 0) {
   if (nthreads <= 0) nthreads = blockDim.x;
   const float gsign = g > 0.f ? 1.f : (g < 0.f ? -1.f : 0.f);
-  const float sabs = fabsf(sigma[0]), m = mu[0];
+  const float sabs = fabsf(DEV ? nvf_load_dev(sigma) : sigma[0]), m = DEV ? nvf_load_dev(mu) : mu[0];
   int l = 0;
   while (l + 1 < b.nlayers && wg >= b.first_wg[l + 1]) ++l;
   const int lo = (wg - b.first_wg[l]) * b.chunk;
@@ -420,7 +424,7 @@
   float* dk = b.dk[l];
   float sb = 0.f, ss = 0.f, sm_ = 0.f;
   for (int i = lo + threadIdx.x; i < hi && (int)threadIdx.x < nthreads; i += nthreads) {
-    float v = rintf(k[i] * 16.f) / 16.f;
+    float v = rintf((DEV ? nvf_load_dev(k + i) : k[i]) * 16.f) / 16.f;
     RateTerm r = rate_term(v, m, sabs, 0.03125f, gsign);
     sb += r.bits;
     ss += r.dsig;
@@ -852,7 +856,10 @@
     const unsigned long long c = cur_s;
     const int64_t* row = a.sched_rows + c * (unsigned long long)a.sched_words;
     for (int w = threadIdx.x; w < a.sched_words; w += blockDim.x) a.sched_buf[w] = row[w];
-    if (threadIdx.x == 0) a.sched_cursor[0] = c + 1;
+    if (threadIdx.x == 0) {
+      a.sched_cursor[0] = c + 1;
+      if (a.reserved & 1) a.sched_cursor[1] = c + 1;
+    }
   }
   if (threadIdx.x == 0 && gridDim.x > 1) a.done[0] = 0u;
 }
@@ -1219,6 +1226,214 @@
   else
     step_head_stem_kernel<16, 32, 2><<<grid, 1024, 0, nvf_stream(stream)>>>(
         (const NvfLayerDesc*)table_dev, nlayers, q, seed, step, step_dev, pk, g, idx, rows, (int)wg, wpl, rate, sj);
+  NVF_LAUNCH_CHECK();
+  return NVF_OK;
+}
+
+constexpr int kSeamLine = 64;
+constexpr int kSeamFinals = 16, kSeamMaster = 17, kSeamShard0 = 18, kSeamTop = 26, kSeamLines = 27;
+
+__device__ __forceinline__ unsigned seam_add(unsigned* c) {
+  return __hip_atomic_fetch_add(c, 1u, __ATOMIC_RELAXED, __HIP_MEMORY_SCOPE_AGENT);
+}
+__device__ __forceinline__ void seam_signal(unsigned* flags, int line, unsigned target) {
+  asm volatile("s_waitcnt vmcnt(0)" ::: "memory");
+  __syncthreads();
+  if (threadIdx.x == 0 && seam_add(flags + line * kSeamLine) == target - 1) seam_add(flags + kSeamMaster * kSeamLine);
+}
+template <bool ACQUIRE>
+__device__ __forceinline__ void seam_wait(unsigned* flags, unsigned ngroups) {
+  if (threadIdx.x == 0) {
+    while (__hip_atomic_load(flags + kSeamMaster * kSeamLine, __ATOMIC_RELAXED, __HIP_MEMORY_SCOPE_AGENT) < ngroups)
+      __builtin_amdgcn_s_sleep(32);
+    if (ACQUIRE) {
+      __builtin_amdgcn_fence(__ATOMIC_ACQUIRE, "agent");
+      asm volatile("s_waitcnt vmcnt(0)" ::: "memory");
+    }
+  }
+  __syncthreads();
+}
+__device__ __forceinline__ void seam_leave(unsigned* flags, int cid, int nwait) {
+  if (threadIdx.x != 0) return;
+  const int shard = cid & 7, nshard = nwait < 8 ? nwait : 8;
+  const unsigned mine = (unsigned)(nwait / 8 + (shard < nwait % 8 ? 1 : 0));
+  if (seam_add(flags + (kSeamShard0 + shard) * kSeamLine) != mine - 1) return;
+  if (seam_add(flags + kSeamTop * kSeamLine) != (unsigned)nshard - 1) return;
+  for (int l = 0; l < kSeamLines; ++l)
+    __hip_atomic_store(flags + l * kSeamLine, 0u, __ATOMIC_RELAXED, __HIP_MEMORY_SCOPE_AGENT);
+}
+
+struct SeamSched {
+  const int64_t* rows;
+  const uint64_t* base;
+  int32_t words, seam_index, idx_word, step_word;
+};
+
+__global__ __launch_bounds__(512, 4) void step_seam_kernel(WgReduceMulti r, int r_blocks, int f_blocks, FinalsArgs a,
+                                                            int sum_blocks, NvfStepTail t, TailRanges rg, unsigned* flags,
+                                                            SeamSched ss, const NvfLayerDesc* __restrict__ table,
+                                                            int nlayers, int q, uint64_t seed, uint64_t step, PackJobs pk,
+                                                            GatherMulti g, int rows, int gwg, int wpl, RateInHead rate,
+                                                            NvfStemHead sj) {
+  constexpr int C0 = 8, C1 = 16, COG = 4, PARTS = C1 / (COG * (C0 / 8));
+  __shared__ __attribute__((aligned(16))) float lds[StemFwdLds<C0, C1, COG>::FLOATS];
+  static_assert(StemFwdLds<C0, C1, COG>::FLOATS >= 16 * 64, "the reduction's slices fit");
+  int bid = blockIdx.x;
+  if (bid < f_blocks) {
+    finals_tail_body(a, sum_blocks, t, rg, bid, f_blocks);
+    seam_signal(flags, kSeamFinals, (unsigned)f_blocks);
+    return;
+  }
+  bid -= f_blocks;
+  if (bid < r_blocks) {
+    const int job = wgrad_reduce_multi_body<512>(r, bid, (float(*)[64])lds);
+    seam_signal(flags, job, (unsigned)(r.blk_base[job + 1] - r.blk_base[job]));
+    return;
+  }
+  bid -= r_blocks;
+  const unsigned ngroups = (unsigned)r.n + 1u;
+  const int64_t* row = ss.rows + (ss.base[0] + (uint64_t)ss.seam_index) * (uint64_t)ss.words;
+  const int64_t* idx = row + ss.idx_word;
+  const uint64_t* step_dev = (const uint64_t*)(row + ss.step_word);
+  const int nstem = 1 + rows * PARTS;
+  const int nwait = nstem + rate.nwg + wpl * nlayers + wpl * pk.n;
+  if (bid >= nwait) {
+    bid -= nwait;
+    gather_rows_multi_body(g, idx, rows, bid / gwg, bid % gwg, gwg);
+    return;
+  }
+  const int cid = bid;
+  if (bid < nstem) {
+    seam_wait<true>(flags, ngroups);
+    const uint64_t st = step + step_dev[0];
+    const StemRawW wp{table[sj.lat_row], table[sj.up0_row], table[sj.conv0_row], sj.emb, idx, seed, st, sj.ch, q};
+    const StemLatent L{nullptr, nullptr, nullptr, sj.lat_beta_hat, sj.lat_gamma_hat, idx, sj.sigma, sj.mu, sj.h, sj.lat,
+                       sj.x_rounded, sj.bits, step_dev, seed, step, sj.mode, rows};
+    const int b = bid == 0 ? 0 : (bid - 1) / PARTS, part = bid == 0 ? PARTS : (bid - 1) % PARTS;
+    stem_fwd_body<C0, C1, COG, true, true>(nullptr, wp, sj.beta_hat, sj.gamma_hat, sj.a0, sj.h0, sj.y1, sj.ch, L, b, part,
+                                           lds);
+    seam_leave(flags, cid, nwait);
+    return;
+  }
+  bid -= nstem;
+  seam_wait<false>(flags, ngroups);
+  if (bid < rate.nwg) {
+    weight_rate_partial_body<true>(rate.b, rate.sigma, rate.mu, rate.part, rate.g, bid, 0, lds, 256);
+  } else if ((bid -= rate.nwg) < wpl * nlayers) {
+    prepare_weights_body<true>(table, q, seed, step, step_dev, bid / wpl, bid % wpl, wpl);
+  } else {
+    bid -= wpl * nlayers;
+    const int job = bid / wpl;
+    const NvfLayerDesc d = table[pk.layer[job]];
+    const int qq = d.quantised ? q : 0, bwd = pk.bwd[job];
+    const uint64_t sid = ((step + step_dev[0]) << 8) | (uint64_t)d.layer_id;
+    pack_mfma_body(pk, job, bid % wpl, wpl, [&](int, int si) {
+      return effective_weight<true>(d, layout_to_kernel_index(d, bwd, si), qq, seed, sid);
+    });
+  }
+  seam_leave(flags, cid, nwait);
+}
+
+extern "C" size_t nvf_step_seam_flags_bytes(void) { return (size_t)kSeamLines * kSeamLine * sizeof(unsigned); }
+
+extern "C" int nvf_step_seam(const float* const* slabs, float* const* dws, const int* nslabs, const int* jtotals, int n,
+                             const float* const* addends, const NvfAdamFuse* adam, NvfStepCtx* ctx,
+                             const NvfStepTail* tail, const int64_t* ranges, int nranges, uint32_t* flags, int seam_index,
+                             int refuse, const void* table_dev, int nlayers, int q, uint64_t seed, uint64_t step,
+                             const uint64_t* step_dev, float* const* pack_dsts, const int* pack_kinds,
+                             const int* pack_c0s, const int* pack_c1s, const int* pack_layers, const int* pack_bwd,
+                             int npack, const float* const* srcs, float* const* dsts, const int* widths, int ng,
+                             const int64_t* idx, int rows, const NvfRateJob* rate_job, const NvfStemHead* stem,
+                             void* stream) {
+  if (refuse) return NVF_EINVAL;
+  if (!slabs || !dws || !nslabs || !jtotals || n <= 0 || n > 16 || !adam || !tail || !nvf_ctx_ok(ctx) || !flags)
+    return NVF_EINVAL;
+  if (nranges < 0 || nranges > 16 || (nranges > 0 && !ranges) || seam_index < 0) return NVF_EINVAL;
+  NvfStepTail t = *tail;
+  if (!t.p || !t.g || !t.m || !t.v || t.n <= 0) return NVF_EINVAL;
+  if (t.acc && (!t.loss_terms || !t.lbits || !t.nbits || t.nnb <= 0 || t.nnb > 16)) return NVF_EINVAL;
+  if (!t.sched_rows || !t.sched_buf || !t.sched_cursor || t.sched_words <= 0 || !t.done || !(t.reserved & 1)) return NVF_EINVAL;
+  if (!adam->g_base || !adam->p_base || !adam->m_base || !adam->v_base || adam->n <= 0) return NVF_EINVAL;
+  if (adam->coef_dev) {
+    const char* c = (const char*)adam->coef_dev;
+    const char* b = (const char*)t.sched_buf;
+    if (c + 2 * sizeof(float) > b && c < b + (size_t)t.sched_words * sizeof(int64_t)) return NVF_EINVAL;
+  }
+  WgReduceMulti r{};
+  int base = 0, m = 0;
+  for (int i = 0; i < n; ++i) {
+    if (nslabs[i] == 0) continue;
+    if (!slabs[i] || !dws[i] || nslabs[i] < 0 || jtotals[i] <= 0) return NVF_EINVAL;
+    r.slabs[m] = slabs[i]; r.dw[m] = dws[i]; r.nslab[m] = nslabs[i]; r.jtotal[m] = jtotals[i];
+    r.add[m] = addends ? addends[i] : nullptr;
+    r.blk_base[m] = base;
+    base += (jtotals[i] + 63) / 64;
+    ++m;
+  }
+  r.blk_base[m] = base;
+  r.n = m;
+  r.fuse = 1;
+  r.adam = *adam;
+  r.adam.reserved = 1.f;
+  t.reserved |= 2;
+  if (m == 0) return NVF_EINVAL;
+  TailRanges rg{};
+  for (int k = 0; k < nranges; ++k) {
+    if (ranges[2 * k] < 0 || ranges[2 * k + 1] > t.n || ranges[2 * k] > ranges[2 * k + 1]) return NVF_EINVAL;
+    rg.lo[k] = (long)ranges[2 * k]; rg.hi[k] = (long)ranges[2 * k + 1];
+  }
+  rg.n = nranges;
+  if (ctx->args.has_f && ctx->args.f_nterm > 3) return NVF_EINVAL;
+  if (!table_dev || nlayers <= 0 || !idx || !step_dev || npack < 0 || !stem) return NVF_EINVAL;
+  const NvfStemHead sj = *stem;
+  if (!(sj.c0 == 8 && sj.c1 == 16) || sj.ch <= 0 || sj.ch > kStemFwdMaxCh || rows <= 0 || rows > 32) return NVF_EINVAL;
+  if (sj.lat_row < 0 || sj.lat_row >= nlayers || sj.up0_row < 0 || sj.up0_row >= nlayers || sj.conv0_row < 0 ||
+      sj.conv0_row >= nlayers || (sj.mode != 0 && sj.mode != 1))
+    return NVF_EINVAL;
+  if (!sj.emb || !sj.lat_beta_hat || !sj.lat_gamma_hat || !sj.sigma || !sj.mu || !sj.beta_hat || !sj.gamma_hat || !sj.h ||
+      !sj.lat || !sj.x_rounded || !sj.bits || !sj.a0 || !sj.h0 || !sj.y1)
+    return NVF_EINVAL;
+  SeamSched ss{};
+  {
+    const int64_t* b0 = t.sched_buf;
+    const int64_t *ip = idx, *sp = (const int64_t*)step_dev;
+    if (ip < b0 || ip + rows > b0 + t.sched_words || sp < b0 || sp >= b0 + t.sched_words) return NVF_EINVAL;
+    ss.rows = t.sched_rows; ss.base = t.sched_cursor + 1; ss.words = t.sched_words; ss.seam_index = seam_index;
+    ss.idx_word = (int32_t)(ip - b0); ss.step_word = (int32_t)(sp - b0);
+  }
+  PackJobs pk{};
+  if (npack > 0) {
+    if (!pack_layers || !pack_bwd) return NVF_EINVAL;
+    const int rc = pack_jobs_desc(nullptr, pack_dsts, pack_kinds, pack_c0s, pack_c1s, npack, pk);
+    if (rc != NVF_OK) return rc;
+    for (int j = 0; j < npack; ++j) {
+      if (pack_layers[j] < 0 || pack_layers[j] >= nlayers) return NVF_EINVAL;
+      pk.layer[j] = pack_layers[j]; pk.bwd[j] = pack_bwd[j] ? 1 : 0;
+    }
+  }
+  GatherMulti g{};
+  long wg = 0;
+  const int rc = gather_multi_desc(srcs, dsts, widths, ng, rows, g, wg);
+  if (rc != NVF_OK) return rc;
+  wg = (wg + 1) / 2;
+  const int wpl = 32;
+  RateInHead rate{};
+  if (rate_job) {
+    if (!rate_job->sigma || !rate_job->mu || !rate_job->part) return NVF_EINVAL;
+    const int rrc = weight_rate_batch_desc(rate_job->kernel, rate_job->dk, rate_job->n, rate_job->nlayers, rate.b);
+    if (rrc != NVF_OK) return rrc;
+    rate.sigma = rate_job->sigma; rate.mu = rate_job->mu; rate.part = rate_job->part; rate.g = rate_job->g;
+    rate.nwg = rate.b.first_wg[rate.b.nlayers];
+  }
+  const FinalsArgs a = ctx->args;
+  ctx->args = FinalsArgs{};
+  ctx->deferring = 0;
+  const int sum_blocks = finals_sum_blocks(a);
+  const int f_blocks = 2 + sum_blocks + 1;
+  const unsigned grid = f_blocks + base + 1 + rows * 4 + rate.nwg + wpl * nlayers + wpl * npack + (unsigned)(wg * ng);
+  step_seam_kernel<<<grid, 512, 0, nvf_stream(stream)>>>(r, base, f_blocks, a, sum_blocks, t, rg, flags, ss,
+                                                         (const NvfLayerDesc*)table_dev, nlayers, q, seed, step, pk, g, rows,
+                                                         (int)wg, wpl, rate, sj);
   NVF_LAUNCH_CHECK();
   return NVF_OK;
 }
diff --git a/nvfpcc_amd/csrc/wgrad.hip b/nvfpcc_amd/csrc/wgrad.hip
--- a/nvfpcc_amd/csrc/wgrad.hip
+++ b/nvfpcc_amd/csrc/wgrad.hip
@@ -3,6 +3,7 @@
 #include <cstdlib>
 #include "step_ctx.h"
 #include "heads_wgrad_mfma.h"
+#include "wgrad_reduce.h"
 
 static const int kMaxSlabs = 512;
 static const int kSumChunks = 128;
@@ -1246,51 +1247,6 @@
                         out_mode, 0, variant, stream, nslab);
 }
 
-struct WgReduceMulti {
-  const float* slabs[16];
-  float* dw[16];
-  const float* add[16];
-  int32_t nslab[16], jtotal[16], blk_base[17];
-  int32_t n, fuse;
-  NvfAdamFuse adam;
-};
-
-__device__ __forceinline__ void wgrad_reduce_multi_body(const WgReduceMulti& d, int bid, float (*part)[64]) {
-  int t = 0;
-  while (t + 1 < d.n && bid >= d.blk_base[t + 1]) ++t;
-  const float* slabs = d.slabs[t];
-  const int nslab = d.nslab[t], jtotal = d.jtotal[t];
-  const int jl = threadIdx.x & 63, sl = threadIdx.x >> 6;
-  const int j = (bid - d.blk_base[t]) * 64 + jl;
-  float s0 = 0.f, s1 = 0.f, s2 = 0.f, s3 = 0.f;
-  if (j < jtotal) {
-    for (int g0 = sl; g0 < nslab; g0 += 256) {
-      float v[16];
-#pragma unroll
-      for (int i = 0; i < 16; ++i) v[i] = g0 + 16 * i < nslab ? slabs[(size_t)(g0 + 16 * i) * jtotal + j] : 0.f;
-#pragma unroll
-      for (int i = 0; i < 16; i += 4) { s0 += v[i]; s1 += v[i + 1]; s2 += v[i + 2]; s3 += v[i + 3]; }
-    }
-  }
-  const float s = (s0 + s1) + (s2 + s3);
-  part[sl][jl] = s;
-  __syncthreads();
-  if (sl == 0) {
-    int bad = 0;
-    if (j < jtotal) {
-      float v = part[0][jl];
-#pragma unroll
-      for (int k = 1; k < 16; ++k) v += part[k][jl];
-      if (d.add[t]) v += d.add[t][j];
-      d.dw[t][j] = v;
-      if (d.fuse) bad = adam_fused_elem(d.adam, d.dw[t] + j, v);
-    }
-    if (d.fuse && d.adam.bad_count) {
-      const unsigned long long any = __ballot(bad);
-      if (any && jl == 0) atomicAdd(d.adam.bad_count, (float)__popcll(any));
-    }
-  }
-}
 
 __global__ __launch_bounds__(1024) void wgrad_reduce_multi(WgReduceMulti d) {
   __shared__ float part[16][64];
diff --git a/nvfpcc_amd/csrc/wgrad_reduce.h b/nvfpcc_amd/csrc/wgrad_reduce.h
--- /dev/null
+++ b/nvfpcc_amd/csrc/wgrad_reduce.h
@@ -0,0 +1,62 @@
+#pragma once
+#include "nvf_common.h"
+#include "finals.h"
+
+struct WgReduceMulti {
+  const float* slabs[16];
+  float* dw[16];
+  const float* add[16];
+  int32_t nslab[16], jtotal[16], blk_base[17];
+  int32_t n, fuse;
+  NvfAdamFuse adam;
+};
+
+template <int NT = 1024>
+__device__ __forceinline__ int wgrad_reduce_multi_body(const WgReduceMulti& d, int bid, float (*part)[64]) {
+  static_assert(NT == 1024 || NT == 512 || NT == 256, "16 slices over NT / 64 waves");
+  constexpr int SPT = 1024 / NT, NSL = NT / 64;
+  int t = 0;
+  while (t + 1 < d.n && bid >= d.blk_base[t + 1]) ++t;
+  const float* slabs = d.slabs[t];
+  const int nslab = d.nslab[t], jtotal = d.jtotal[t];
+  const int jl = threadIdx.x & 63, sl0 = threadIdx.x >> 6;
+  const int j = (bid - d.blk_base[t]) * 64 + jl;
+  float s0[SPT], s1[SPT], s2[SPT], s3[SPT];
+#pragma unroll
+  for (int h = 0; h < SPT; ++h) s0[h] = s1[h] = s2[h] = s3[h] = 0.f;
+  if (j < jtotal) {
+    for (int g0 = 0; g0 < nslab; g0 += 256) {
+      float v[SPT][16];
+#pragma unroll
+      for (int h = 0; h < SPT; ++h)
+#pragma unroll
+        for (int i = 0; i < 16; ++i) {
+          const int g = g0 + sl0 + h * NSL + 16 * i;
+          v[h][i] = g < nslab ? slabs[(size_t)g * jtotal + j] : 0.f;
+        }
+#pragma unroll
+      for (int h = 0; h < SPT; ++h)
+#pragma unroll
+        for (int i = 0; i < 16; i += 4) { s0[h] += v[h][i]; s1[h] += v[h][i + 1]; s2[h] += v[h][i + 2]; s3[h] += v[h][i + 3]; }
+    }
+  }
+#pragma unroll
+  for (int h = 0; h < SPT; ++h) part[sl0 + h * NSL][jl] = (s0[h] + s1[h]) + (s2[h] + s3[h]);
+  __syncthreads();
+  if (sl0 == 0) {
+    int bad = 0;
+    if (j < jtotal) {
+      float v = part[0][jl];
+#pragma unroll
+      for (int k = 1; k < 16; ++k) v += part[k][jl];
+      if (d.add[t]) v += d.add[t][j];
+      d.dw[t][j] = v;
+      if (d.fuse) bad = adam_fused_elem(d.adam, d.dw[t] + j, v);
+    }
+    if (d.fuse && d.adam.bad_count) {
+      const unsigned long long any = __ballot(bad);
+      if (any && jl == 0) atomicAdd(d.adam.bad_count, (float)__popcll(any));
+    }
+  }
+  return t;
+}
diff --git a/nvfpcc_amd/engine.py b/nvfpcc_amd/engine.py
--- a/nvfpcc_amd/engine.py
+++ b/nvfpcc_amd/engine.py
@@ -24,6 +24,8 @@
 _STEM_IN_TRUNK5 = True
 _STEM_IN_HEAD = True
 _HEADS_IN_TRUNK5 = True
+_STEP_SEAM = True
+_SEAM_REFUSE = False
 
 
 class StepPlan(NamedTuple):
@@ -40,12 +42,13 @@
     tail_queued: bool
     sums_in_trunk5: bool
     fused_optimiser: bool
+    seam: bool = False
 
 
 @functools.lru_cache(maxsize=None)
 def plan_step(narrow, wide, winograd, fused_stem, fused_latent_stem, heads3, ch, batch, want_w, want_emb, fuse, hook,
               naive, head_bias_in_loss, sums_in_trunk5, stem_in_trunk5, stem_in_head, heads_in_trunk5,
-              step_head=False, defer_heads=False):
+              step_head=False, defer_heads=False, seam=False):
     tuned = naive == 0
     small = batch <= 32
     stem_fwd = ("head" if step_head and stem_in_head and fused_stem and fused_latent_stem and small and tuned else
@@ -59,7 +62,10 @@
     tail = want_w and not want_emb and ch <= 8 and tuned
     stem_bwd = ("queued" if stem_in_trunk5 and tail and in_trunk5 and fused_stem and small else
                 "layers" if not fused_stem else "partial" if want_w else "plain")
-    return StepPlan(want_w=want_w, want_emb=want_emb, stem_fwd=stem_fwd, latent_fwd_fused=ch <= 8 and tuned, heads=heads,
+    fused = fuse and not hook
+    seam = bool(seam and fused and narrow and not wide and in_trunk5 and sums_in_trunk5 and stem_in_head and fused_stem and
+                fused_latent_stem and small and tuned)
+    return StepPlan(seam=seam, want_w=want_w, want_emb=want_emb, stem_fwd=stem_fwd, latent_fwd_fused=ch <= 8 and tuned, heads=heads,
                     head_bias_in_loss=want_w and head_bias_in_loss and fused_loss, heads_in_trunk5=in_trunk5,
                     trunk5=trunk5, conv0_wgrad_in_stem=want_w and fused_stem and not trunk5, stem_bwd=stem_bwd,
                     tail_queued=tail, sums_in_trunk5=in_trunk5 and sums_in_trunk5, fused_optimiser=fuse and not hook)
@@ -127,6 +133,10 @@
         self._rate_retired = []
         self._graphs_captured = 0
         self.tail_done = False
+        self._seam = None
+        self._seam_flags = None
+        self.seam_launches = 0
+        self.seam_refused = 0
         self._tail_ranges = {}
         self.collective_mode = None
         self.heads3 = self.narrow or self.wide
@@ -261,11 +271,11 @@
             self._rate = (job, add, key, dk, part)
         return self._rate
 
-    def _plan(self, batch, want_w=False, want_emb=False, fuse=False, step_head=False, defer_heads=False):
+    def _plan(self, batch, want_w=False, want_emb=False, fuse=False, step_head=False, defer_heads=False, seam=False):
         return plan_step(self.narrow, self.wide, self.winograd, self.fused_stem, self.fused_latent_stem, self.heads3,
                          self.ch, batch, want_w, want_emb, fuse, self.grad_hook is not None, ops._NAIVE,
                          _HEAD_BIAS_IN_LOSS, _SUMS_IN_TRUNK5, _STEM_IN_TRUNK5, _STEM_IN_HEAD, _HEADS_IN_TRUNK5,
-                         step_head, defer_heads)
+                         step_head, defer_heads, seam and _STEP_SEAM)
 
     def _noise(self):
         sd = self._step_dev
@@ -291,6 +301,9 @@
                 (ctypes.c_void_p * n)(*[d.data_ptr() for d in dsts]), (ctypes.c_int * n)(*[s[0].numel() for s in srcs]), n,
                 idx_dev.data_ptr(), rows, ctypes.byref(self._rate_job()[0]) if with_rate else None)
         o = None
+        held, self._seam = self._seam, None
+        if held is not None and self._plan(rows, step_head=stem_mode is not None).stem_fwd != "head":
+            held = self._close_held(held)
         if self._plan(rows, step_head=stem_mode is not None).stem_fwd == "head":
             from ._lib import NvfStemHead
             net = self.net
@@ -309,12 +322,30 @@
             sj.a0, sj.h0, sj.y1 = (o[k].data_ptr() for k in ("a0", "h0", "y1"))
             sj.lat_row, sj.up0_row, sj.conv0_row = self._rows["latent"], self._rows["up0"], self._rows["conv0"]
             sj.mode, sj.ch, sj.c0, sj.c1 = (0 if stem_mode == "train" else 1), ch, c0, c1
-            check(lib().nvf_step_head_stem(*args, ctypes.byref(sj), torch.cuda.current_stream().cuda_stream),
-                  "nvf_step_head_stem")
+            stream = torch.cuda.current_stream().cuda_stream
+            if held is not None:
+                cargs, index = held[0], held[1]
+                rc = lib().nvf_step_seam(*cargs[:-1], self._seam_flags.data_ptr(), index, int(_SEAM_REFUSE), *args,
+                                         ctypes.byref(sj), stream)
+                if rc == -1:
+                    self.seam_refused += 1
+                    self._close_held(held)
+                    held = None
+                else:
+                    check(rc, "nvf_step_seam")
+                    self.seam_launches += 1
+            if held is None:
+                check(lib().nvf_step_head_stem(*args, ctypes.byref(sj), stream), "nvf_step_head_stem")
         else:
             check(lib().nvf_step_head(*args, torch.cuda.current_stream().cuda_stream), "nvf_step_head")
         self._rate_ready = bool(with_rate)
         return dsts if stem_mode is None else dsts + [o]
+
+    def _close_held(self, held):
+        held[0][-1][1].reserved = 0
+        check(lib().nvf_wgrad_reduce_finals_tail(*held[0][:-1], torch.cuda.current_stream().cuda_stream),
+              "nvf_wgrad_reduce_finals_tail")
+        return None
 
     def prepare_weights(self, q):
         step, sd = self._noise()
@@ -461,7 +492,8 @@
 
     def _backward(self, a, gt, dist, gt16, gt8, n_pts, mode, block_ids, want_w, want_emb, fuse=None):
         deferred = a.get("p2") is None
-        plan = self._plan(a["e"].shape[0], want_w, want_emb, fuse is not None, defer_heads=deferred)
+        plan = self._plan(a["e"].shape[0], want_w, want_emb, fuse is not None, defer_heads=deferred,
+                          seam=fuse is not None and fuse.get("seam") is not None)
         if deferred and plan.heads != "deferred":
             raise ValueError("forward(defer_heads=True) must be followed by a backward pass with weight gradients "
                              "(want_w=True): the heads' forward runs in that pass's loss launch")
@@ -490,6 +522,8 @@
         last = {"loss_terms": loss, "latent_bits": a["lbits"], "net_bits": nbits, "n_pts": n_pts}
         self._bwd_finish(plan, sums, sums_done, last, fuse)
         self.last = last
+        if self._seam is not None:
+            self._seam += ((t0, t1, g5, g4, g3, g2, g1, da0, dx0, de, tail, sums, heads_job, stem_jobs, loss, nbits, a),)
         return de
 
     def _bwd_loss_heads(self, plan, a, gt, dist, gt16, gt8, loss, sums):
@@ -643,7 +677,10 @@
         if one_launch and fused:
             if fuse.get("coef_dev") is not None:
                 adam.coef_dev = self._coef_live.data_ptr()
-            self._wg.finish_and_flush_tail(addends, adam, tail, ranges)
+            if plan.seam:
+                self._seam = (self._wg.finish_and_flush_tail(addends, adam, tail, ranges, defer=True), fuse["seam"])
+            else:
+                self._wg.finish_and_flush_tail(addends, adam, tail, ranges)
         elif one_launch:
             self._wg.finish_and_flush(addends)
         elif fused:
@@ -659,7 +696,7 @@
                     counts=self.step_counts if stats else None, acc=self.epoch_acc, done=self._tail_done)
 
     def _fused_tail(self, plan, tail, sums, last, gs, gm):
-        t = ops.step_tail_args(**tail, **self._tail_kw(last))
+        t = ops.step_tail_args(**{k: v for k, v in tail.items() if k != "seam"}, **self._tail_kw(last))
         outs = [o for _, o in sums] + [gs, gm]
         if plan.head_bias_in_loss:
             outs += [self.layers[n].gb for n in ("conv0_cls", "conv1_cls", "conv2_cls")]
@@ -835,6 +872,7 @@
         self.sched = torch.zeros(nw + 2 + (self.CAP + 1) * nw, dtype=torch.int64, device=dev)
         self.buf = self.sched[:nw]
         self.cursor, self.rows = self.sched[nw:nw + 1], self.sched[nw + 2:]
+        self.sched_arg = (self.buf, self.rows, self.cursor, self.nw, True)
         self.pins = [torch.zeros(self.sched.numel(), dtype=torch.int64).pin_memory() for _ in range(max(int(ring), 1))]
         self.pin_np = [p.numpy() for p in self.pins]
         self.pin_events = [None] * len(self.pins)
@@ -851,6 +889,8 @@
         first[:batch] = torch.arange(batch) % eng.N_leaf
         first[batch + 1:batch + 2].view(torch.float32)[:] = 1.0
         self.buf.copy_(first)
+        if eng._seam_flags is None:
+            eng._seam_flags = torch.zeros(lib().nvf_step_seam_flags_bytes() // 4, dtype=torch.int32, device=dev)
         side = torch.cuda.Stream()
         side.wait_stream(torch.cuda.current_stream())
         acc = eng.epoch_acc
@@ -885,18 +925,20 @@
         for u in (self.unrolls if tail else ()):
             g = torch.cuda.CUDAGraph()
             with torch.cuda.graph(g):
-                for _ in range(u):
-                    self._body(tail=tail)
+                for i in range(u):
+                    self._body(tail=tail, seam=i if i < u - 1 else None)
             self.graphs_u[u] = (g, self.out, self.last)
         self.graph_u = self.graphs_u[self.unroll][0] if self.graphs_u else None
 
-    def _body(self, tail):
+    def _body(self, tail, seam=None):
         eng = self.eng
         gt, dist, gt16, gt8, e, stem = eng.batch_and_prepare(self.idx, self.q, with_rate=True, stem_mode="train")
         a = eng.forward(e, "train", self.idx, defer_heads=True, stem=stem)
         spec = None
         if tail and eng.grad_hook is None:
-            spec = dict(coef_dev=self.coef, inv_npts_dev=self.inv_npts, sched=(self.buf, self.rows, self.cursor, self.nw))
+            spec = dict(coef_dev=self.coef, inv_npts_dev=self.inv_npts, sched=self.sched_arg)
+            if seam is not None:
+                spec["seam"] = seam
         eng.backward(a, gt, dist, gt16, gt8, 1.0, "train", self.idx, want_w=True, want_emb=False, fuse=spec)
         self.out = a
         self.last = dict(eng.last)
@@ -907,7 +949,7 @@
         eng = self.eng
         if eng.grad_hook is not None:
             eng.grad_hook(eng.flat_gx)
-        ops.step_tail(coef_dev=self.coef, inv_npts_dev=self.inv_npts, sched=(self.buf, self.rows, self.cursor, self.nw),
+        ops.step_tail(coef_dev=self.coef, inv_npts_dev=self.inv_npts, sched=self.sched_arg,
                       **eng._tail_kw(self.last))
 
     def stage_schedule(self, steps):
@@ -945,7 +987,7 @@
         f32[:n, 2 * (B + 2):2 * (B + 2) + 2] = ops.adam_coefficients_n(eng.lr, eng.opt_step + 1, n)
         rows[n] = rows[n - 1]
         host[:nw] = rows[0]
-        host[nw], host[nw + 1] = 1, 0
+        host[nw], host[nw + 1] = 1, 1
         self.pin_gen[slot] += 1
         m = nw + 2 + (n + 1) * nw
         return {"_staged": True, "slot": slot, "gen": self.pin_gen[slot], "n": n, "npts": npts.tolist(), "words": m,
diff --git a/nvfpcc_amd/ops.py b/nvfpcc_amd/ops.py
--- a/nvfpcc_amd/ops.py
+++ b/nvfpcc_amd/ops.py
@@ -760,16 +760,17 @@
             len(tensors), tensors[0].shape[0], _ptr(ws), ws.numel(), _ctx(self.ctx), _stream()),
             "nvf_wgrad_reduce_multi_and_sums_fused")
 
-    def finish_and_flush_tail(self, addends, adam, tail, ranges):
+    def finish_and_flush_tail(self, addends, adam, tail, ranges, defer=False):
         import ctypes
         if not (0 < len(self.jobs) <= 16) or self.ctx is None:
             raise RuntimeError("finish_and_flush_tail: 1..16 reduction jobs and a step context are required")
         jobs = self._take_jobs()
         flat = [int(v) for r in ranges for v in r]
         arr = (ctypes.c_int64 * max(len(flat), 1))(*flat)
-        check(lib().nvf_wgrad_reduce_finals_tail(*self._job_arrays(jobs, addends), ctypes.byref(adam), _ctx(self.ctx),
-                                                 ctypes.byref(tail), arr, len(ranges), _stream()),
-              "nvf_wgrad_reduce_finals_tail")
+        args = (*self._job_arrays(jobs, addends), ctypes.byref(adam), _ctx(self.ctx), ctypes.byref(tail), arr, len(ranges))
+        if defer:
+            return args + ((adam, tail, addends),)
+        check(lib().nvf_wgrad_reduce_finals_tail(*args, _stream()), "nvf_wgrad_reduce_finals_tail")
 
     def finish_and_flush(self, addends):
         if not (0 < len(self.jobs) <= 16) or self.ctx is None:
@@ -1033,8 +1034,10 @@
         _chk(done)
         a.done = done.data_ptr()
     if sched is not None:
-        buf, rows, cursor, words = sched
+        buf, rows, cursor, words = sched[:4]
         _chk(buf, rows, cursor)
+        if len(sched) > 4 and sched[4]:
+            a.reserved = 1
         a.sched_buf, a.sched_rows, a.sched_cursor, a.sched_words = buf.data_ptr(), rows.data_ptr(), cursor.data_ptr(), int(words)
     return a
 
```
